# ducha-aiki/affnet

Measured on AMD Instinct MI355X. Metric: keypoints/sec (detect+AffNet+OriNet+HardNet) per image, 2000 kp @1024x768, higher is better.
Workload: dtype f32

## Files before the change

### affnet_amd/SparseImgRepresenter.py

```python
import ctypes as C

import torch
import torch.nn as nn

from . import _lib, engine
from ._lib import lib, check, ptr
from .architectures import _HipPatchNet
from .HandCraftedModules import AffineShapeEstimator, OrientationDetector, _HipHandCrafted
from .HardNet import HardTFeatNet
from .pytorch_sift import SIFTNet

_FOLLOW = (SIFTNet, HardTFeatNet)


class ScaleSpaceAffinePatchExtractor(nn.Module):
    def __init__(self, border=16, num_features=500, patch_size=32, mrSize=3.0, nlevels=3, num_Baum_iters=0,
                 init_sigma=1.6, th=None, RespNet=None, OriNet=None, AffNet=None, arith="fp32"):
        super(ScaleSpaceAffinePatchExtractor, self).__init__()
        self.arith = arith
        _lib.arith_code(arith)
        self.mrSize, self.PS, self.b = mrSize, patch_size, border
        self.num, self.nlevels = num_features, nlevels
        self.num_Baum_iters, self.init_sigma = num_Baum_iters, init_sigma
        self.th = th
        if th is not None:
            self.num = -1
        else:
            self.th = 0
        self.RespNet = RespNet
        if not 1 <= nlevels <= 6:
            raise NotImplementedError("nlevels must be 1..6 (levels per octave = nlevels + 2 <= 8)")
        self.OriNet = OriNet if OriNet is not None else OrientationDetector(patch_size=19)
        self.AffNet = AffNet if AffNet is not None else AffineShapeEstimator(patch_size=19)
        self.scale_pyr = self.sigmas = self.pix_dists = None
        self._ctx = None
        self._ctx_key = None
        self._fctx = self._fctx_key = self._pyr_ctx = None
        self.last_ids = None
        self.max_keep = 16384
        self.raw_div = 4
        self.lazy_shape_rows = -1
        self.shape_form = 1

        self.desc_form = 2

    def _context(self, x, allow_batch=False):
        engine.require_cuda(x, "image")
        if x.dim() != 4 or x.size(1) != 1 or x.size(0) < 1 or (x.size(0) != 1 and not allow_batch):
            raise ValueError("expected a (1,1,H,W) image; forward() is batch-size-1 like the reference "
                             "(HandCraftedModules.py:283-284) - use enqueue()/run_batch() for (B,1,H,W) batches")
        pre = int(1.5 * self.num) if self.num_Baum_iters > 0 else self.num
        key = (x.size(0), x.size(2), x.size(3), x.device, pre, self.num, float(self.th), self.mrSize, self.b, self.init_sigma,
               self.nlevels, self.max_keep, self.num_Baum_iters, self.raw_div, self.lazy_shape_rows)
        if self._ctx is not None and self._ctx_key == key and self._ctx.arith != _lib.arith_code(self.arith):
            self._ctx.set_arith(self.arith)
        if self._ctx is None or self._ctx_key != key:
            self._ctx = engine.Context(x.size(2), x.size(3), x.device, self.nlevels, self.init_sigma, self.b, self.mrSize,
                                       float(self.th), self.num, pre, self.max_keep, batch=x.size(0), baum_iters=self.num_Baum_iters, raw_div=self.raw_div,
                                       lazy_shape_rows=self.lazy_shape_rows, arith=self.arith)
            self._ctx_key = key
        if self._ctx.shape_form != int(self.shape_form):
            self._ctx.set_shape_form(self.shape_form)
        if self._ctx.desc_form != int(self.desc_form):
            self._ctx.set_desc_form(self.desc_form)
        return self._ctx

    def _publish_pyramid(self, ctx):
        self._pyr_ctx = ctx
        self.scale_pyr = ctx.pyramid_views()
        self.sigmas = [list(s) for s in ctx.plan.sigmas]
        self.pix_dists = [list(p) for p in ctx.plan.pix_dists]

    def _response_pyramid(self, ctx, img):
        dev = img.device
        st = engine.stream_of(dev)
        check(lib.affnet_pyramid_build(ctx.handle, ptr(img), st), ctx.handle, "affnet_pyramid_build")
        stride = lib.affnet_pyramid_image_stride(ctx.handle)
        base = lib.affnet_pyramid_level_offset(ctx.handle, 0, 0)
        resp = torch.zeros(ctx.batch * stride, dtype=torch.float32, device=dev)
        with torch.no_grad():
            for b in range(ctx.batch):
                pyr = ctx.pyramid_views(b)
                for o, (h, w) in enumerate(ctx.plan.sizes):
                    for l in range(ctx.plan.levels_per_octave):
                        off = b * stride + lib.affnet_pyramid_level_offset(ctx.handle, o, l) - base
                        r = self.RespNet(pyr[o][l], ctx.plan.sigmas[o][l])
                        resp[off:off + h * w].copy_(r.reshape(-1).to(dev, torch.float32))
        return resp

    @staticmethod
    def _native(slot):
        return slot is None or isinstance(slot, (_HipPatchNet, _HipHandCrafted))

    def enqueue(self, x, do_ori=False, desc=None, det_stream=None, input_ready=None):
        ctx = self._context(x, allow_batch=True)
        dev = x.device
        if not (self._native(self.AffNet) and self._native(self.OriNet)):
            raise NotImplementedError("the fused path needs the native AffNetFast / OriNetFast slots (foreign slots: forward())")
        img = x.contiguous().float()
        B, F = x.size(0), ctx.cap_final
        lafs = torch.empty(B, F, 2, 3, dtype=torch.float32, device=dev)
        resp = torch.empty(B, F, dtype=torch.float32, device=dev)
        ids = torch.empty(B, F, 3, dtype=torch.int32, device=dev)
        count = torch.zeros(B, dtype=torch.int32, device=dev)
        dsc = torch.empty(B, F, 128, dtype=torch.float32, device=dev) if desc is not None else None
        nets = self._nets(dev, do_ori, desc)
        follow = isinstance(desc, _FOLLOW)
        if isinstance(desc, HardTFeatNet):
            desc.check_usable()
        fused_dsc = None if follow else dsc
        if self.RespNet is not None:
            rmaps = self._response_pyramid(ctx, img)
            check(lib.affnet_detect_image_responses(ctx.handle, ptr(rmaps), engine.stream_of(dev)), ctx.handle, "affnet_detect_image_responses")
            rc = lib.affnet_describe_detected(ctx.handle, C.byref(nets), int(bool(do_ori)), ptr(lafs), ptr(resp), ptr(ids), ptr(fused_dsc),
                                              ptr(count), engine.stream_of(dev))
            check(rc, ctx.handle, "affnet_describe_detected")
        elif det_stream is None:
            rc = lib.affnet_extract_features(ctx.handle, C.byref(nets), ptr(img), int(bool(do_ori)), ptr(lafs), ptr(resp), ptr(ids),
                                             ptr(fused_dsc), ptr(count), engine.stream_of(dev))
            check(rc, ctx.handle, "affnet_extract_features")
        else:
            cur = torch.cuda.current_stream(dev)
            if input_ready is None:
                det_stream.wait_stream(cur)
            elif input_ready is not False:
                det_stream.wait_event(input_ready)
            if getattr(self, "_busy", None) is not None:
# ... 374 lines not shown
```

### affnet_amd/_lib.py

```python
import ctypes as C
import os

_HERE = os.path.dirname(os.path.abspath(__file__))
LIB_PATH = os.environ.get("AFFNET_HIP_LIB") or os.path.join(_HERE, "libaffnet_hip.so")
PROBES_LIB_PATH = os.path.join(_HERE, "libaffnet_hip_probes.so")

MAX_OCTAVES, MAX_LEVELS, MAX_TAPS = 16, 8, 37
NET_AFFNET, NET_ORINET, NET_HARDNET, NET_AFFNET_FULLCONV = 0, 1, 2, 3
ARITH_FP32_MFMA, ARITH_FP32_SPLIT3, ARITH_FP32_SPLIT2H = 0, 1, 2
ARITH_NAMES = {"fp32": ARITH_FP32_MFMA, "fp32_mfma": ARITH_FP32_MFMA, "fp32_split3": ARITH_FP32_SPLIT3, "split3": ARITH_FP32_SPLIT3,
               "fp32_split2h": ARITH_FP32_SPLIT2H, "split2h": ARITH_FP32_SPLIT2H}


def arith_code(arith):
    if arith is None:
        return ARITH_FP32_MFMA
    if isinstance(arith, str):
        if arith.lower() not in ARITH_NAMES:
            raise ValueError("arith must be one of %s" % sorted(ARITH_NAMES))
        return ARITH_NAMES[arith.lower()]
    if int(arith) not in (ARITH_FP32_MFMA, ARITH_FP32_SPLIT3, ARITH_FP32_SPLIT2H):
        raise ValueError("arith must be AFFNET_ARITH_FP32_MFMA (0), AFFNET_ARITH_FP32_SPLIT3 (1) or AFFNET_ARITH_FP32_SPLIT2H (2)")
    return int(arith)
SHAPE_FORM_DIRECT, SHAPE_FORM_WINOGRAD, SHAPE_FORM_POLYPHASE = 0, 1, 2
DESC_FORM_DIRECT, DESC_FORM_POLYPHASE, DESC_FORM_F43 = 0, 1, 2
OK, ERR_INVALID, ERR_HIP, ERR_CAPACITY, ERR_EMPTY = 0, -1, -2, -3, -4
VERIFY_AFFINE, VERIFY_HOMOGRAPHY, VERIFY_TILE, VERIFY_CHUNK = 0, 1, 128, 128
KNN_MAX_K = 8
IVF_MAX_PROBE = 8
VERIFY_FLAG_PAIR_RANGE = 8


class Config(C.Structure):
    _fields_ = [
        ("height", C.c_int32), ("width", C.c_int32), ("n_octaves", C.c_int32), ("levels_per_octave", C.c_int32),
        ("oct_h", C.c_int32 * MAX_OCTAVES), ("oct_w", C.c_int32 * MAX_OCTAVES),
        ("level_sigma", (C.c_float * MAX_LEVELS) * MAX_OCTAVES),
        ("level_sigma4", (C.c_float * MAX_LEVELS) * MAX_OCTAVES),
        ("level_sigma_px", (C.c_double * MAX_LEVELS) * MAX_OCTAVES),
        ("first_blur_taps", C.c_int32), ("first_blur", C.c_float * (MAX_TAPS * MAX_TAPS)),
        ("level_blur_taps", C.c_int32 * MAX_LEVELS),
        ("level_blur", (C.c_float * (MAX_TAPS * MAX_TAPS)) * MAX_LEVELS),
        ("level_blur0_taps", C.c_int32 * MAX_LEVELS),
        ("level_blur0", (C.c_float * (MAX_TAPS * MAX_TAPS)) * MAX_LEVELS),
        ("lazy_shape_rows", C.c_int32),
        ("onepass", C.c_int32),
        ("mr_size", C.c_float), ("threshold", C.c_float),
        ("num_features", C.c_int32), ("num_prefilter", C.c_int32),
        ("max_raw_per_octave_div", C.c_int32), ("max_keep", C.c_int32), ("batch", C.c_int32), ("baum_iters", C.c_int32),
        ("arith", C.c_int32),
    ]


class Nets(C.Structure):
    _fields_ = [("d_affnet", C.c_void_p), ("d_orinet", C.c_void_p), ("d_hardnet", C.c_void_p),
                ("h_orientation_window", C.c_void_p), ("h_baumberg_window", C.c_void_p)]


_P, _I, _SZ = C.c_void_p, C.c_int, C.c_size_t
SYMBOLS = {
    "affnet_config_fill": (_I, [C.POINTER(Config), _I, _I, _I, C.c_double, _I, C.c_double, C.c_double, _I, _I, _I, _I]),
    "affnet_ctx_create": (_I, [C.POINTER(_P), _I, C.POINTER(Config)]),
    "affnet_ctx_destroy": (None, [_P]),
    "affnet_last_error": (C.c_char_p, [_P]),
    "affnet_version": (C.c_char_p, []),
    "affnet_set_arith": (_I, [_P, _I]),
    "affnet_get_arith": (_I, [_P]),
    "affnet_set_shape_form": (_I, [_P, _I]),
    "affnet_get_shape_form": (_I, [_P]),
    "affnet_set_desc_form": (_I, [_P, _I]),
    "affnet_get_desc_form": (_I, [_P]),
    "affnet_workspace_bytes": (_SZ, [_P]),
    "affnet_bind_workspace": (_I, [_P, _P, _SZ]),
    "affnet_pyramid_level_offset": (C.c_int64, [_P, _I, _I]),
    "affnet_pyramid_image_stride": (C.c_int64, [_P]),
    "affnet_batch": (_I, [_P]),
    "affnet_capacity_prefilter": (_I, [_P]),
    "affnet_capacity_final": (_I, [_P]),
    "affnet_gauss_blur": (_I, [_P, _P, _P, _I, _I, C.POINTER(C.c_float), _I, _P]),
    "affnet_pyramid_build": (_I, [_P, _P, _P]),
    "affnet_hessian_response": (_I, [_P, _P, _P, _I, _I, C.c_float, _P]),
    "affnet_detect": (_I, [_P, _P, _P, _P, _P, _P]),
    "affnet_detect_responses": (_I, [_P, _P, _P, _P, _P, _P, _P]),
    "affnet_laf_grid_sample": (_I, [_P, _P, _I, _I, _P, _I, _I, _P, _P]),
    "affnet_pyr_grid_sample": (_I, [_P, _P, _P, _P, _I, _I, _P, _P]),
    "affnet_cnn32_packed_floats": (_SZ, [_I]),
    "affnet_cnn32_winograd_offset": (C.c_int64, [_I, _I]),
    "affnet_cnn32_pack_weights": (_I, [_I, C.POINTER(_P), C.POINTER(_P), C.POINTER(_P), _P, _P, _P, _P, _P]),
    "affnet_cnn32_forward": (_I, [_P, _I, _P, _P, _P, _I, _P, _P, _P]),
    "affnet_cnn32_forward_pyr": (_I, [_P, _I, _P, _P, _P, _P, _I, _P, _P, _P]),
    "affnet_local_norm": (_I, [_P, _P, _P, _I, _I, _P]),
    "affnet_fullconv_scratch_bytes": (_SZ, [_I, _I]),
    "affnet_fullconv_forward": (_I, [_P, _P, _P, _I, _I, _P, _P, _P]),
    "affnet_nms2d": (_I, [_P, _P, _P, _I, _I, C.c_float, _P]),
    "affnet_shape_filter_select": (_I, [_P, _P, _P, _P, _P, _P, _P, _P, _P, _P, _P]),
    "affnet_apply_rotation": (_I, [_P, _P, _P, _P, _I, _P]),
    "affnet_scale_lafs": (_I, [_P, _P, _P, _P, _I, _I, _I, _I, _P]),
    "affnet_lafs_to_ellipses": (_I, [_P, _P, _P, _I, _P, _P]),
    "affnet_ellipses_to_lafs": (_I, [_P, _P, _P, _I, _P, _P]),
    "affnet_level_select": (_I, [_P, _P, _P, _I, _I, _P, _P, _P]),
    "affnet_handcrafted_forward": (_I, [_P, _I, _P, _I, _P, _P, _P, _P]),
    "affnet_handcrafted_forward_pyr": (_I, [_P, _I, _P, _P, _P, _I, _P, _P, _P]),
    "affnet_sift_host_window": (_I, [_I, C.POINTER(C.c_float)]),
    "affnet_sift_forward": (_I, [_P, _P, _I, _P, C.c_float, _P, _P]),
    "affnet_sift_forward_pyr": (_I, [_P, _P, _P, _P, _I, _P, C.c_float, _P, _P]),
    "affnet_tfeat_packed_floats": (_SZ, []),
    "affnet_tfeat_pack_weights": (_I, [_P, _P, _P, _P, _P, _P, _P]),
    "affnet_tfeat_scratch_floats": (_SZ, [_I]),
    "affnet_tfeat_forward": (_I, [_P, _P, _P, _P, _I, _P, _P, _P]),
    "affnet_tfeat_forward_pyr": (_I, [_P, _P, _P, _P, _P, _I, _P, _P, _P]),
    "affnet_match_scratch_bytes": (_SZ, [_I, _I]),
    "affnet_distance_matrix": (_I, [_P, _P, _I, _P, _I, _I, _P, _P, _P]),
    "affnet_match_snn": (_I, [_P, _P, _I, _P, _I, _I, C.c_float, _P, _P, _P, _P, _P, _P, _P]),
    "affnet_reproject_lafs": (_I, [_P, _P, _I, C.POINTER(C.c_float), _P, _P]),
    "affnet_centre_nn": (_I, [_P, _P, _I, _P, _I, _P, _P, _P]),
    "affnet_verify_scratch_bytes": (_SZ, [_I]),
    "affnet_verify_score": (_I, [_P, _P, _I, _P, _I, _P, _P, _I, C.c_float, _P, _P, _P, _P]),
    "affnet_verify_matches": (_I, [_P, _P, _I, _P, _I, _P, _P, _I, C.c_float, _I, _I, _P, _P, _P, _P, _P, _P]),
    "affnet_match_many_scratch_bytes": (_SZ, [_I, _I, _I]),
    "affnet_match_snn_many": (_I, [_P, _P, _I, _P, _I, _I, _P, _I, _I, _I, C.c_float, _P, _P, _P, _P, _P, _P, _P]),
    "affnet_verify_many_scratch_bytes": (_SZ, [_I, _I]),
    "affnet_verify_matches_many": (_I, [_P, _P, _I, _P, _I, _P, _I, _P, _P, _I, C.c_float, _I, _I, _P, _P, _P, _P, _P, _P]),
    "affnet_knn_chunks": (_I, [_P, _I, _I]),
    "affnet_knn_scratch_bytes": (_SZ, [_I, _I, _I, _I]),
    "affnet_knn": (_I, [_P, _P, _I, _P, _I, _I, _I, _I, _I, _I, _P, _P, _P, _P]),
    "affnet_knn_vote": (_I, [_P, _P, _P, _I, _I, C.c_float, _P, _I, _I, _P, _P]),
    "affnet_quantize_desc": (_I, [_P, _P, _I, _I, C.c_float, _P, _P, _P]),
    "affnet_knn_q8_chunks": (_I, [_P, _I, _I]),
    "affnet_knn_q8_scratch_bytes": (_SZ, [_I, _I, _I, _I]),
    "affnet_knn_q8": (_I, [_P, _P, _P, _I, _P, _P, _I, _I, _I, _I, _I, _I, C.c_float, _P, _P, _P, _P, _P]),
    "affnet_ivf_sqnorm": (_I, [_P, _P, _I, _I, _P, _P]),
    "affnet_ivf_cell_means": (_I, [_P, _P, _I, _I, _P, _P, _I, _P, _P]),
    "affnet_ivf_scratch_bytes": (_SZ, [_I, _I, _I, _I]),
    "affnet_ivf_search": (_I, [_P, _P, _I, _P, _P, _P, _I, _P, _P, _I, _I, _I, _I, _I, _I, _P, _P, _P, _P, _P]),
    "affnet_ivf_q8_scratch_bytes": (_SZ, [_I, _I, _I, _I]),
    "affnet_ivf_search_q8": (_I, [_P, _P, _P, _P, _I, _P, _P, _P, _I, _P, _P, _I, _I, _I, _I, _I, _I, C.c_float, _P, _P, _P, _P, _P, _P]),
    "affnet_extract_features": (_I, [_P, C.POINTER(Nets), _P, _I, _P, _P, _P, _P, _P, _P]),
    "affnet_detect_image": (_I, [_P, _P, _P]),
    "affnet_detect_image_responses": (_I, [_P, _P, _P]),
    "affnet_detect_image_onepass": (_I, [_P, _P, _P, _P]),
    "affnet_detect_image_onepass_responses": (_I, [_P, _P, _P, _P]),
    "affnet_detected_list": (_I, [_P, _P, _P, _P, _P, _P]),
    "affnet_load_frames": (_I, [_P, _P, _I, _P, _P, _P, _I, _I, _P]),
    "affnet_describe_frames": (_I, [_P, C.POINTER(Nets), _P, _P, _P, _P, _I, _I, _P, _P, _P, _P, _P, _P]),
    "affnet_shape_iterate": (_I, [_P, _P, _P, _P, _P, _I, _P, _P]),
    "affnet_affmap_offset": (C.c_int64, [_P, _I]),
    "affnet_affmap_image_stride": (C.c_int64, [_P]),
    "affnet_describe_detected": (_I, [_P, C.POINTER(Nets), _I, _P, _P, _P, _P, _P, _P]),
    "affnet_graph_capture_extract": (_I, [_P, C.POINTER(Nets), _P, _I, _P, _P, _P, _P, _P, _P]),
    "affnet_graph_launch": (_I, [_P, _P]),
    "affnet_profile_enable": (_I, [_P, _I]),
    "affnet_profile_read": (_I, [_P, C.POINTER(C.c_double * 8), C.POINTER(C.c_int32)]),
    "affnet_read_counts": (_I, [_P, C.POINTER(C.c_int32 * 4), _P]),
    "affnet_counter_offset": (C.c_int64, [_P, _I]),
    "affnet_counter_stride": (C.c_int64, [_P]),
    "affnet_host_base_grid": (_I, [_I, C.POINTER(C.c_float)]),
}

DEBUG_SYMBOLS = {
    "affnet_cnn32_debug_timing": (_I, [_P, _P]),
    "affnet_cnn32_debug_layer": (_I, [_P, _I, _P, _P, _I, _P, _P]),
    "affnet_cnn32_debug_winograd_u": (_I, [_P, _I, _P, _I, _P, _P]),
    "affnet_selftest_mfma": (_I, [_P, _P, _P, _P]),
    "affnet_debug_split3_variant": (_I, [_P, _I]),
}

PROBE_SYMBOLS = {
    "affnet_cnn32_probe": (_I, [_P, _I, _I, _I, _I, _P, _P]),
    "affnet_split3_gemm": (_I, [_P, _P, _I, _I, _I, _I, _P, _P]),
    "affnet_split3_rate": (_I, [_I, _I, _I, _P, _P]),
    "affnet_debug_stream": (_I, [_P, _P, _SZ, _I, _I, _I, _P]),
    "affnet_probe_shape_offsets": (_I, [_P, C.POINTER(C.c_int64 * 3)]),
    "affnet_probe_affnet_wino_layer": (_I, [_P, _I, _P, _P, _I, _P, _P]),
    "affnet_probe_affnet_wino_partials": (_I, [_P, _P, _P, _I, _P, _P]),
    "affnet_probe_affnet_poly_layer": (_I, [_P, _I, _P, _P, _I, _P, _P]),
    "affnet_probe_affnet_poly_partials": (_I, [_P, _P, _P, _I, _P, _P]),
    "affnet_probe_trunk16_poly_u": (_I, [_P, _I, _P, _I, _P, _P]),
    "affnet_probe_hardnet_poly_layer": (_I, [_P, _P, _P, _I, _P, _P]),
    "affnet_probe_hardnet_poly_forward": (_I, [_P, _P, _P, _I, _P, _P, _P]),
    "affnet_probe_hardnet_poly_u": (_I, [_P, _P, _I, _P, _P]),
    "affnet_probe_hardnet_f43_layer": (_I, [_P, _P, _P, _I, _P, _P]),
    "affnet_probe_hardnet_f43_forward": (_I, [_P, _P, _P, _I, _P, _P, _P]),
    "affnet_probe_hardnet_f43_u": (_I, [_P, _P, _I, _P, _P]),
}


class AffnetHipError(RuntimeError):
    pass


class AffnetEmptyError(AffnetHipError):
    """AFFNET_ERR_EMPTY: no image of the call produced a detection (the reference raises in torch.cat([]),
    SparseImgRepresenter.py:100)."""


def _load():
    if not os.path.isfile(LIB_PATH):
        if os.path.basename(LIB_PATH) == os.path.basename(PROBES_LIB_PATH):
            raise ImportError("affnet_amd: %s is missing - the tools under tools/ need the probe build of the library: "
                              "AFFNET_PROBES=1 bash affnet_amd/csrc/build.sh" % LIB_PATH)
        raise ImportError(
            "affnet_amd: %s is missing - the HIP extension is the only implementation of this path "
            "(no CPU fallback). Build it: bash affnet_amd/csrc/build.sh" % LIB_PATH)
    lib = C.CDLL(LIB_PATH)
    for table in (SYMBOLS, DEBUG_SYMBOLS):
        for name, (res, args) in table.items():
            fn = getattr(lib, name)
            fn.restype, fn.argtypes = res, args
    for name, (res, args) in PROBE_SYMBOLS.items():
        if hasattr(lib, name):
            fn = getattr(lib, name)
            fn.restype, fn.argtypes = res, args
    return lib


lib = _load()


def check(rc, ctx=None, what=""):
    if rc != OK:
        msg = lib.affnet_last_error(ctx).decode() if ctx else ""
        if rc == ERR_EMPTY:
            raise AffnetEmptyError("%s: %s" % (what or "libaffnet_hip call", msg))
        raise AffnetHipError("%s failed (code %d): %s" % (what or "libaffnet_hip call", rc, msg))


def ptr(t):
    return None if t is None else C.c_void_p(t.data_ptr())


def current_stream(device):
    import torch
    return C.c_void_p(torch.cuda.current_stream(device).cuda_stream)
```

### affnet_amd/csrc/cnn32.hip

```cpp
#include "common.h"

static void aff_fill_pyr_src(const affnet_ctx* ctx, PyrSrc* s) {
    memset(s, 0, sizeof(*s));
    if (ctx->ws) aff_fill_pyr_table(ctx, &s->t);
    aff_base_grid(32, s->base);
}

static int cnn_check(affnet_ctx* ctx, const CnnCall& c, int* rows) {
    *rows = 0;
    if (c.kind < 0 || c.kind > 2) return aff_fail(ctx, AFFNET_ERR_INVALID, "cnn32: unknown net kind %d", c.kind);
    if (!c.packed || !c.out || c.n_max < 0 || (!c.patches && (!c.lafs || !c.ids))) return aff_fail(ctx, AFFNET_ERR_INVALID, "cnn32: null argument");
    if (!c.patches && !ctx->ws) return aff_fail(ctx, AFFNET_ERR_INVALID, "cnn32: sampling from the pyramid needs a bound workspace");
    if (c.dbg_layer < 0 && !c.scratch)
        return aff_fail(ctx, AFFNET_ERR_INVALID, "cnn32: d_scratch is required (HardNet n*(8192+512) floats, AffNet / OriNet n*144 floats)");
    if (c.dbg_layer >= 0 && ctx->arith != AFFNET_ARITH_FP32_MFMA)
        return aff_fail(ctx, AFFNET_ERR_INVALID, "cnn32: layer dumps exist for AFFNET_ARITH_FP32_MFMA only (context is in arithmetic mode %d)", ctx->arith);
    if (c.n_max == 0) return AFFNET_OK;
    if (c.kind == AFFNET_NET_HARDNET && c.n_max > 65535)
        return aff_fail(ctx, AFFNET_ERR_INVALID, "cnn32: n_max=%d (HardNet head: max 65535 rows per image)", c.n_max);
    const int row_count = c.row_count < 0 ? c.n_max - c.row_begin : c.row_count;
    if (c.row_begin < 0 || row_count < 0 || c.row_begin + row_count > c.n_max) return aff_fail(ctx, AFFNET_ERR_INVALID, "cnn32: bad row window");
    *rows = row_count;
    return AFFNET_OK;
}

TrunkKernel aff_trunk_kernel(int kind, int form, bool stamps) {
    typedef TrunkKernel (*Unit)(int, bool);
    static_assert(AFFNET_NET_AFFNET == 0 && AFFNET_NET_ORINET == 1 && AFFNET_NET_HARDNET == 2 && TRUNK_EXACT == 0 && TRUNK_WINO == 1 && TRUNK_SPLIT2 == 2 && TRUNK_SPLIT3 == 3 &&
                  TRUNK_WINO_F43 == 4 && TRUNK_WINO_POLY == 5 && TRUNK_FORMS == 6, "order of the table");
    static const Unit unit[3][TRUNK_FORMS] = {{aff_trunk_affnet, aff_trunk_affnet, aff_trunk_affnet, aff_trunk_affnet, nullptr, aff_trunk_affnet_poly},
                                              {aff_trunk_orinet, nullptr, aff_trunk_orinet, aff_trunk_orinet, nullptr, nullptr},
                                              {aff_trunk_hardnet, aff_trunk_hardnet_poly, aff_trunk_hardnet, aff_trunk_hardnet, aff_trunk_hardnet_f43, nullptr}};
    if (kind < 0 || kind > 2 || form < 0 || form >= TRUNK_FORMS || !unit[kind][form]) return nullptr;
    return unit[kind][form](form, stamps);
}

int aff_trunk_launch(affnet_ctx* ctx, const CnnCall& c, const NetLayout& L, dim3 grid, int wino, const int32_t* reeval, int shape_op) {
    int form = TRUNK_EXACT;
    if (ctx->arith != AFFNET_ARITH_FP32_MFMA) form = ctx->arith == AFFNET_ARITH_FP32_SPLIT2H ? TRUNK_SPLIT2 : TRUNK_SPLIT3;
    else if (c.kind == AFFNET_NET_AFFNET && wino) form = wino == 2 ? TRUNK_WINO_POLY : TRUNK_WINO;
    else if (c.kind == AFFNET_NET_HARDNET && c.desc_form != AFFNET_DESC_FORM_DIRECT) form = c.desc_form == AFFNET_DESC_FORM_F43 ? TRUNK_WINO_F43 : TRUNK_WINO;
    const bool stamps = ctx->dbg_time || c.dbg_layer >= 0;
    const TrunkKernel kernel = aff_trunk_kernel(c.kind, form, stamps);
    if (!kernel) return aff_fail(ctx, AFFNET_ERR_INVALID, "cnn32: no trunk kernel of net %d in form %d is built", c.kind, form);
    CnnArgs a;
    a.packed = c.packed; a.off = to_offsets(L, ctx->arith);
    a.reeval = reeval;
    const int rc = aff_derive_u(ctx, c.kind, form, c.packed, L, c.st, &a.wino_u);
    if (rc) return rc;
    a.patches = c.patches; a.lafs = c.lafs; a.ids = c.ids; a.count = c.count; a.n_max = c.n_max;
    a.out = (c.dbg_layer < 0) ? c.scratch : c.out;
    a.dbg_layer = c.dbg_layer; a.dbg_out = c.dbg_out; a.dbg_time = ctx->dbg_time;
    a.row_begin = c.row_begin; a.skip_cnt = c.skip_cnt; a.skip_n = c.skip_n;
    a.shape_cnt = (c.fuse && shape_op) ? c.fuse->cnt : nullptr; a.shape_op = shape_op;
    a.s3_alt = ctx->split3_variant;
    PyrSrc ps;
    aff_fill_pyr_src(ctx, &ps);
    hipLaunchKernelGGL(kernel, grid, dim3(512), 0, c.st, a, ps);
    AFF_LAUNCH_CHECK(ctx);
    return AFFNET_OK;
}

static int cnn_launch(affnet_ctx* ctx, const CnnCall& c) {
    int rows;
    int rc = cnn_check(ctx, c, &rows);
    if (rc || rows == 0) return rc;
    const NetLayout L = net_layout(c.kind);
    const int B = c.patches ? 1 : ctx->B;
    const bool form1 = c.wino_reeval && c.kind == AFFNET_NET_AFFNET && c.fuse && c.dbg_layer < 0 && ctx->arith == AFFNET_ARITH_FP32_MFMA;
    rc = aff_trunk_launch(ctx, c, L, dim3(rows, B), form1 ? c.wino_reeval : 0, nullptr, c.shape_op);
    if (rc) return rc;
    if (form1) {
        int32_t* flags = reinterpret_cast<int32_t*>(c.scratch + (size_t)B * c.n_max * HEAD_PART_AFF);
        rc = aff_margin_affnet(ctx, c, L, rows, B, flags);
        if (rc) return rc;
        rc = aff_trunk_launch(ctx, c, L, dim3(rows, B), 0, flags, 0);
        if (rc) return rc;
    }
    if (c.dbg_layer < 0 && c.kind != AFFNET_NET_HARDNET) {
        rc = c.kind == AFFNET_NET_AFFNET ? aff_finish_affnet(ctx, c, L, rows, B) : aff_finish_orinet(ctx, c, L, rows, B);
        if (rc) return rc;
    }
    if (c.mark_head) aff_prof_mark(ctx, 7, c.st);
    if (c.dbg_layer < 0 && c.kind == AFFNET_NET_HARDNET) return aff_hardnet_head(ctx, c, L, B);
    return AFFNET_OK;
}

extern "C" int affnet_cnn32_forward(affnet_ctx* ctx, int net_kind, const float* d_packed, const float* d_patches, const int32_t* d_count,
                                    int n_max, float* d_out, float* d_scratch, void* stream) {
    AFF_DEVICE(ctx);
    if (!ctx || !d_patches) return aff_fail(ctx, AFFNET_ERR_INVALID, "cnn32_forward: null argument");
    CnnCall c;
    c.kind = net_kind; c.packed = d_packed; c.patches = d_patches; c.count = d_count; c.n_max = n_max; c.out = d_out; c.scratch = d_scratch; c.st = (hipStream_t)stream;
    return cnn_launch(ctx, c);
}

extern "C" int affnet_cnn32_forward_pyr(affnet_ctx* ctx, int net_kind, const float* d_packed, const float* d_lafs, const int32_t* d_ids,
                                        const int32_t* d_count, int n_max, float* d_out, float* d_scratch, void* stream) {
    AFF_DEVICE(ctx);
    if (!ctx) return AFFNET_ERR_INVALID;
    CnnCall c;
    c.kind = net_kind; c.packed = d_packed; c.lafs = d_lafs; c.ids = d_ids; c.count = d_count; c.n_max = n_max; c.out = d_out; c.scratch = d_scratch; c.st = (hipStream_t)stream;
    return cnn_launch(ctx, c);
}

int aff_affnet_filter_rows(affnet_ctx* ctx, const float* packed, const float* resp, const float* lafs, const int32_t* ids, const int32_t* count,
                           float* out, float* scratch, int row_begin, int row_count, bool lazy, int shape_op, hipStream_t st) {
    ShapeFuse sf;
    sf.resp = resp; sf.lafs = lafs; sf.key = ctx->st_key; sf.good = ctx->st_good; sf.cnt = ctx->cnt;
    CnnCall c;
    c.kind = AFFNET_NET_AFFNET; c.packed = packed; c.lafs = lafs; c.ids = ids; c.count = count; c.n_max = ctx->cap_pre; c.out = out; c.scratch = scratch; c.st = st;
    c.row_begin = row_begin; c.row_count = row_count;
    c.skip_cnt = lazy ? ctx->cnt : nullptr; c.skip_n = ctx->cfg.num_features;
    c.fuse = &sf; c.shape_op = shape_op;
    c.wino_reeval = ctx->shape_form;
    return cnn_launch(ctx, c);
}

int aff_orinet_rotate(affnet_ctx* ctx, const float* packed, float* lafs, const int32_t* ids, const int32_t* count, int n_max, float* out, float* scratch,
                      hipStream_t st, const DenormSel* denorm) {
    CnnCall c;
    c.kind = AFFNET_NET_ORINET; c.packed = packed; c.lafs = lafs; c.ids = ids; c.count = count; c.n_max = n_max; c.out = out; c.scratch = scratch; c.st = st;
    c.rot_lafs = lafs; c.denorm = denorm;
    return cnn_launch(ctx, c);
// ... 52 lines not shown
```

### affnet_amd/csrc/cnn_mfma.h

```cpp
#pragma once
#include <math.h>
#include <stdlib.h>

#include <utility>

#include "common.h"
#include "weights_layout.h"

typedef float f32x4 __attribute__((ext_vector_type(4)));

typedef __attribute__((address_space(3))) const f32x4 LdsF4;
__device__ __forceinline__ unsigned lds_byte_addr(const float* p) {
    return (unsigned)(size_t)(__attribute__((address_space(3))) const float*)p;
}
__device__ __forceinline__ f32x4 lds_read4(unsigned byte_addr) { return *(LdsF4*)(size_t)byte_addr; }

typedef unsigned u32x4 __attribute__((ext_vector_type(4)));
__device__ __forceinline__ __amdgpu_buffer_rsrc_t weight_rsrc(const float* base, int n_floats) {
    return __builtin_amdgcn_make_buffer_rsrc(const_cast<float*>(base), 0, n_floats * 4, 0x00020000);
}
__device__ __forceinline__ f32x4 buf_read4(__amdgpu_buffer_rsrc_t r, int lane_byte_off, int uniform_byte_off) {
    return __builtin_bit_cast(f32x4, __builtin_amdgcn_raw_buffer_load_b128(r, lane_byte_off, uniform_byte_off, 0));
}

// ... 979 lines not shown
            for (int c = 0; c < 2; ++c) {
#pragma unroll
                for (int j = 0; j < 4; ++j)
#pragma unroll
                    for (int e = 0; e < 4; ++e) {
                        if (i == 0) t0[c][j][e] = acc[c][j][e];
                        else if (i == 1) { t0[c][j][e] = wadd(t0[c][j][e], acc[c][j][e]); t1[c][j][e] = acc[c][j][e]; }
                        else if (i == 2) { t0[c][j][e] = wadd(t0[c][j][e], acc[c][j][e]); t1[c][j][e] = wsub(t1[c][j][e], acc[c][j][e]); }
                        else t1[c][j][e] = wsub(t1[c][j][e], acc[c][j][e]);
                    }
                if (i == 3) {
#pragma unroll
                    for (int e = 0; e < 4; ++e) {
                        y[2 * u + c][0][e] = wadd(wadd(t0[c][0][e], t0[c][1][e]), t0[c][2][e]);
                        y[2 * u + c][1][e] = wsub(wsub(t0[c][1][e], t0[c][2][e]), t0[c][3][e]);
                        y[2 * u + c][2][e] = wadd(wadd(t1[c][0][e], t1[c][1][e]), t1[c][2][e]);
                        y[2 * u + c][3][e] = wsub(wsub(t1[c][1][e], t1[c][2][e]), t1[c][3][e]);
                    }
                }
            }
            __builtin_amdgcn_sched_barrier(0);
        }
    };
    {
        f32x4 da[4], db[4];
        wino_read_rows<LI>(window_addr(0), 0, da, db);
        wino_transform_row(0, da, db, Va);
    }
#pragma unroll
    for (int s = 0; s < NSTEP; s += 2) {
        step(s, Va, Vb);
        step(s + 1, Vb, Va);
    }
}

template <int NW, int CIN, int COUT, typename LI>
__device__ __forceinline__ void conv3x3_wino_mfma_shared_v(float* act, const float* __restrict__ Wu, f32x4 (&U)[16], f32x4 (&y)[1][4], int wave, int lane) {
    constexpr int NGRP = CIN / 16;
    static_assert(LI::H == 8 && COUT == 16 * NW && NGRP == NW, "one tile block, one channel block and one K group per wave");
    const int m = lane & 15, kq = lane >> 4;
    const __amdgpu_buffer_rsrc_t wrsrc = weight_rsrc(Wu, 16 * CIN * COUT);
    int ty, tx, cb;
    wino_tile<8, COUT, 1>(wave, 0, m, ty, tx, cb);
    const int u_lane = wino_u_lane<8, COUT, 1>(wave, 0, lane);
    f32x4 V[16];
    wino_window<LI>(lds_byte_addr(act) + ((wave * 4 + kq) * LI::PSG + (2 * ty * LI::WP + 2 * tx) * 4) * 4, V);
    __syncthreads();
    const unsigned v0 = lds_byte_addr(act) + lane * 16;
#pragma unroll
    for (int k = 0; k < 16; ++k) *reinterpret_cast<f32x4*>(&act[((wave * 16 + k) * 64 + lane) * 4]) = V[k];
    __syncthreads();
#pragma unroll
    for (int k = 0; k < 16; ++k) V[k] = lds_read4(v0 + k * 1024);
    f32x4 acc[16];
#pragma unroll
    for (int k = 0; k < 16; ++k) acc[k] = (f32x4){0.f, 0.f, 0.f, 0.f};
#pragma unroll 1
    for (int G = 0; G < NGRP; ++G) {
        const int Gn = G == NGRP - 1 ? G : G + 1;
        unsigned vb = v0 + Gn * 16 * 1024;
        asm("" : "+v"(vb));
        __builtin_amdgcn_sched_barrier(0);
#pragma unroll
        for (int k = 0; k < 16; k += 2) {
#pragma unroll
            for (int s4 = 0; s4 < 4; ++s4) {
                acc[k] = __builtin_amdgcn_mfma_f32_16x16x4f32(U[k][s4], V[k][s4], acc[k], 0, 0, 0);
                acc[k + 1] = __builtin_amdgcn_mfma_f32_16x16x4f32(U[k + 1][s4], V[k + 1][s4], acc[k + 1], 0, 0, 0);
            }
            U[k] = wino_load_u<CIN, COUT>(wrsrc, u_lane, k, Gn);
            U[k + 1] = wino_load_u<CIN, COUT>(wrsrc, u_lane, k + 1, Gn);
            V[k] = lds_read4(vb + k * 1024);
            V[k + 1] = lds_read4(vb + (k + 1) * 1024);
            __builtin_amdgcn_sched_barrier(0);
        }
    }
    wino_output(acc, y[0]);
}

struct F43L {
    static constexpr int V_FLOATS = 4 * F43_XI * 256;
    static constexpr int X = 0, X_FLOATS = 8 * 8 * 256;
};
__device__ __forceinline__ void f43_bt_lo(float d0, float d1, float d2, float d3, float d4, float& v0, float& v1, float& v2) {
    v0 = (4.0f * d0 - 5.0f * d2) + d4;
    const float a = d4 - 4.0f * d2, b = d3 - 4.0f * d1;
    v1 = a + b; v2 = a - b;
}
__device__ __forceinline__ void f43_bt_hi(float d1, float d2, float d3, float d4, float d5, float& v3, float& v4, float& v5) {
    const float c = d4 - d2, e = 2.0f * (d3 - d1);
    v3 = c + e; v4 = c - e;
    v5 = (4.0f * d1 - 5.0f * d3) + d5;
}
__device__ __forceinline__ void f43_at_axis(float m0, float m1, float m2, float m3, float m4, float m5, float& y0, float& y1, float& y2, float& y3) {
    const float p = m1 + m2, q = m1 - m2, r = m3 + m4, s = m3 - m4;
    y0 = (m0 + p) + r; y1 = q + 2.0f * s; y2 = p + 4.0f * r; y3 = q + (8.0f * s + m5);
}

template <typename LI, int HF>
__device__ __forceinline__ void f43_window_half(unsigned ab, f32x4 (&V)[18]) {
    f32x4 d[5][6];
#pragma unroll
    for (int r = 0; r < 5; ++r)
#pragma unroll
        for (int c = 0; c < 6; ++c) d[r][c] = lds_read4(ab + ((r + HF) * LI::WP + c) * 16);
#pragma unroll
    for (int e = 0; e < 4; ++e) {
        float t[3][6];
#pragma unroll
        for (int c = 0; c < 6; ++c) {
            if constexpr (HF == 0) f43_bt_lo(d[0][c][e], d[1][c][e], d[2][c][e], d[3][c][e], d[4][c][e], t[0][c], t[1][c], t[2][c]);
            else f43_bt_hi(d[0][c][e], d[1][c][e], d[2][c][e], d[3][c][e], d[4][c][e], t[0][c], t[1][c], t[2][c]);
        }
#pragma unroll
        for (int il = 0; il < 3; ++il) {
            float v[6];
            f43_bt_lo(t[il][0], t[il][1], t[il][2], t[il][3], t[il][4], v[0], v[1], v[2]);
            f43_bt_hi(t[il][1], t[il][2], t[il][3], t[il][4], t[il][5], v[3], v[4], v[5]);
#pragma unroll
            for (int j = 0; j < 6; ++j) V[6 * il + j][e] = v[j];
        }
    }
}

template <int CIN, int COUT>
__device__ __forceinline__ int f43_u_lane(int wave, int lane) {
    return ((lane >> 4) * COUT + (wave >> 1) * 16 + (lane & 15)) * 16 + (wave & 1) * (18 * CIN * COUT * 4);
}
template <int CIN, int COUT>
__device__ __forceinline__ void f43_prefetch_u(const float* __restrict__ Wu, f32x4 (&U)[18], int wave, int lane) {
    const __amdgpu_buffer_rsrc_t r = weight_rsrc(Wu, F43_XI * CIN * COUT);
    const int u_lane = f43_u_lane<CIN, COUT>(wave, lane);
#pragma unroll
    for (int k = 0; k < 18; ++k) U[k] = wino_load_u<CIN, COUT>(r, u_lane, k, 0);
}

template <int NW, int CIN, int COUT, typename LI>
__device__ __forceinline__ void conv3x3_f43_mfma_shared_v(float* act, const float* __restrict__ Wu, f32x4 (&U)[18], f32x4 (&t)[3][4], int wave, int lane) {
    constexpr int NGRP = CIN / 16;
    static_assert(NW == 8 && LI::H == 16 && COUT == 16 * (NW / 2) && NGRP == NW / 2, "one block of 16 4x4 tiles; a wave pair per channel block and per K group");
    const int m = lane & 15, kq = lane >> 4, p = wave >> 1, h = wave & 1;
    const __amdgpu_buffer_rsrc_t wrsrc = weight_rsrc(Wu, F43_XI * CIN * COUT);
    const int u_lane = f43_u_lane<CIN, COUT>(wave, lane);
    f32x4 V[18];
    {
        const unsigned ab = lds_byte_addr(act) + ((4 * p + kq) * LI::PSG + (4 * (m >> 2) * LI::WP + 4 * (m & 3)) * 4) * 4;
        if (h == 0) f43_window_half<LI, 0>(ab, V); else f43_window_half<LI, 1>(ab, V);
    }
    __syncthreads();
#pragma unroll
    for (int k = 0; k < 18; ++k) *reinterpret_cast<f32x4*>(&act[((p * F43_XI + 18 * h + k) * 64 + lane) * 4]) = V[k];
    __syncthreads();
    const unsigned v0 = lds_byte_addr(act) + (18 * h * 64 + lane) * 16;
#pragma unroll
    for (int k = 0; k < 18; ++k) V[k] = lds_read4(v0 + k * 1024);
    f32x4 acc[18];
#pragma unroll
    for (int k = 0; k < 18; ++k) acc[k] = (f32x4){0.f, 0.f, 0.f, 0.f};
#pragma unroll 1
    for (int G = 0; G < NGRP; ++G) {
        const int Gn = G == NGRP - 1 ? G : G + 1;
        unsigned vb = v0 + Gn * F43_XI * 1024;
        asm("" : "+v"(vb));
        __builtin_amdgcn_sched_barrier(0);
#pragma unroll
        for (int k = 0; k < 18; k += 2) {
#pragma unroll
            for (int s4 = 0; s4 < 4; ++s4) {
                acc[k] = __builtin_amdgcn_mfma_f32_16x16x4f32(U[k][s4], V[k][s4], acc[k], 0, 0, 0);
                acc[k + 1] = __builtin_amdgcn_mfma_f32_16x16x4f32(U[k + 1][s4], V[k + 1][s4], acc[k + 1], 0, 0, 0);
            }
            U[k] = wino_load_u<CIN, COUT>(wrsrc, u_lane, k, Gn);
            U[k + 1] = wino_load_u<CIN, COUT>(wrsrc, u_lane, k + 1, Gn);
            V[k] = lds_read4(vb + k * 1024);
            V[k + 1] = lds_read4(vb + (k + 1) * 1024);
            __builtin_amdgcn_sched_barrier(0);
        }
    }
#pragma unroll
    for (int il = 0; il < 3; ++il)
#pragma unroll
        for (int e = 0; e < 4; ++e) {
            float yc[4];
            f43_at_axis(acc[6 * il][e], acc[6 * il + 1][e], acc[6 * il + 2][e], acc[6 * il + 3][e], acc[6 * il + 4][e], acc[6 * il + 5][e], yc[0], yc[1], yc[2], yc[3]);
#pragma unroll
            for (int c = 0; c < 4; ++c) t[il][c][e] = yc[c];
        }
}

__device__ __forceinline__ void f43_combine(float* lds, const f32x4 (&t)[3][4], f32x4 (&y)[8], int wave, int lane) {
    const int h = wave & 1;
    float* xw = lds + F43L::X + (wave * 8 * 64 + lane) * 4;
    const float* xr = lds + F43L::X + ((wave ^ 1) * 8 * 64 + lane) * 4;
    f32x4 k0[4], k1[4];
    if (h == 0) {
#pragma unroll
        for (int c = 0; c < 4; ++c) {
            const f32x4 p = t[1][c] + t[2][c], q = t[1][c] - t[2][c];
            k0[c] = t[0][c] + p; k1[c] = q;
            *reinterpret_cast<f32x4*>(&xw[c * 256]) = p;
            *reinterpret_cast<f32x4*>(&xw[(4 + c) * 256]) = q;
        }
    } else {
#pragma unroll
        for (int c = 0; c < 4; ++c) {
            const f32x4 r = t[0][c] + t[1][c], s = t[0][c] - t[1][c];
            k0[c] = 4.0f * r; k1[c] = 8.0f * s + t[2][c];
            *reinterpret_cast<f32x4*>(&xw[c * 256]) = r;
            *reinterpret_cast<f32x4*>(&xw[(4 + c) * 256]) = 2.0f * s;
        }
    }
    __syncthreads();
#pragma unroll
    for (int c = 0; c < 4; ++c) {
        const f32x4 o0 = *reinterpret_cast<const f32x4*>(&xr[c * 256]), o1 = *reinterpret_cast<const f32x4*>(&xr[(4 + c) * 256]);
        y[c] = k0[c] + o0;
        y[4 + c] = k1[c] + o1;
    }
}

template <typename LO>
__device__ __forceinline__ void f43_store_lds(float* act, f32x4 bias, const f32x4 (&y)[8], int wave, int lane) {
    const int m = lane & 15, oy = 4 * (m >> 2) + 2 * (wave & 1), ox = 4 * (m & 3);
#pragma unroll
    for (int k = 0; k < 8; ++k) {
        const f32x4 v = bias_relu(y[k], bias);
        *reinterpret_cast<f32x4*>(&act[((wave >> 1) * 4 + (lane >> 4)) * LO::PSG + ((oy + (k >> 2) + 1) * LO::WP + ox + (k & 3) + 1) * 4]) = v;
    }
}

template <int NW, int CIN, int COUT, int H, int NB>
__device__ __forceinline__ void wino_prefetch_u_row(const float* __restrict__ Wu, f32x4 (&U)[4], int wave, int lane) {
    const __amdgpu_buffer_rsrc_t r = weight_rsrc(Wu, 16 * CIN * COUT);
    const int u_lane = wino_u_lane<H, COUT, NB>(wave, 0, lane);
#pragma unroll
    for (int k = 0; k < 4; ++k) U[k] = wino_load_u<CIN, COUT>(r, u_lane, k, 0);
}

template <int NW, int CIN, int COUT, typename LI, int NB>
__device__ __forceinline__ void conv3x3_wino_mfma_rows(const float* act, const float* __restrict__ Wu, f32x4 (&U)[4], f32x4 (&y)[NB][4], int wave, int lane) {
    constexpr int H = LI::H, HT = H / 2, NGRP = CIN / 16, NSTEP = NB * 4 * NGRP;
    static_assert(H % 2 == 0 && (HT * HT) % 16 == 0 && COUT % 16 == 0 && CIN % 16 == 0, "Winograd tiling");
    static_assert((HT * HT / 16) * (COUT / 16) == NW * NB, "the waves' passes must tile the layer exactly");
    const int m = lane & 15, kq = lane >> 4;
    const __amdgpu_buffer_rsrc_t wrsrc = weight_rsrc(Wu, 16 * CIN * COUT);
    f32x4 t0[4], t1[4], acc[4];
#pragma unroll
    for (int s = 0; s < NSTEP; ++s) {
        const int q = s / (4 * NGRP), i = (s / NGRP) % 4, G = s % NGRP;
        const int sn = s + 1 < NSTEP ? s + 1 : s;
        const int qn = sn / (4 * NGRP), in = (sn / NGRP) % 4, Gn = sn % NGRP;
        int ty, tx, cb;
        wino_tile<H, COUT, NB>(wave, q, m, ty, tx, cb);
        const int u_next = wino_u_lane<H, COUT, NB>(wave, qn, lane);
        unsigned ab = lds_byte_addr(act) + (((4 * G + kq) * LI::PSG + (2 * ty * LI::WP + 2 * tx) * 4) * 4);
        asm("" : "+v"(ab));
        f32x4 da[4], db[4], V[4];
        wino_read_rows<LI>(ab, i, da, db);
        wino_transform_row(i, da, db, V);
        if (G == 0) {
#pragma unroll
            for (int k = 0; k < 4; ++k) acc[k] = (f32x4){0.f, 0.f, 0.f, 0.f};
        }
        __builtin_amdgcn_sched_barrier(0);
#pragma unroll
        for (int k = 0; k < 4; k += 2) {
#pragma unroll
            for (int s4 = 0; s4 < 4; ++s4) {
                acc[k] = __builtin_amdgcn_mfma_f32_16x16x4f32(U[k][s4], V[k][s4], acc[k], 0, 0, 0);
                acc[k + 1] = __builtin_amdgcn_mfma_f32_16x16x4f32(U[k + 1][s4], V[k + 1][s4], acc[k + 1], 0, 0, 0);
            }
            U[k] = wino_load_u<CIN, COUT>(wrsrc, u_next, 4 * in + k, Gn);
            U[k + 1] = wino_load_u<CIN, COUT>(wrsrc, u_next, 4 * in + k + 1, Gn);
            __builtin_amdgcn_sched_barrier(0);
        }
        if (G == NGRP - 1) {
#pragma unroll
            for (int j = 0; j < 4; ++j)
#pragma unroll
                for (int e = 0; e < 4; ++e) {
                    if (i == 0) t0[j][e] = acc[j][e];
                    else if (i == 1) { t0[j][e] = wadd(t0[j][e], acc[j][e]); t1[j][e] = acc[j][e]; }
                    else if (i == 2) { t0[j][e] = wadd(t0[j][e], acc[j][e]); t1[j][e] = wsub(t1[j][e], acc[j][e]); }
                    else t1[j][e] = wsub(t1[j][e], acc[j][e]);
                }
            if (i == 3) {
#pragma unroll
                for (int e = 0; e < 4; ++e) {
                    y[q][0][e] = wadd(wadd(t0[0][e], t0[1][e]), t0[2][e]);
                    y[q][1][e] = wsub(wsub(t0[1][e], t0[2][e]), t0[3][e]);
                    y[q][2][e] = wadd(wadd(t1[0][e], t1[1][e]), t1[2][e]);
                    y[q][3][e] = wsub(wsub(t1[1][e], t1[2][e]), t1[3][e]);
                }
            }
        }
    }
}

struct Wino5 {
    static constexpr int X = 16 * LayC4::PSG, X_FLOATS = 8 * 4 * 256;
    static constexpr int HEAD = 0;
    static constexpr int U_HALF = 8 * 4 * 16 * 64 * 4;
};
__device__ __forceinline__ void wino5_prefetch_u(const float* __restrict__ Wu, f32x4 (&U)[4], int wave, int lane) {
    const __amdgpu_buffer_rsrc_t r = weight_rsrc(Wu, 16 * 64 * 64);
    const int u_lane = ((lane >> 4) * 64 + (wave >> 1) * 16 + (lane & 15)) * 16 + (wave & 1) * Wino5::U_HALF;
#pragma unroll
    for (int k = 0; k < 4; ++k) U[k] = wino_load_u<64, 64>(r, u_lane, k, 0);
}

template <int NW, typename LI>
// ... 385 lines not shown
```

### affnet_amd/csrc/cnn_trunk.h

```cpp
#pragma once
#include <math.h>

#include <type_traits>

#include "common.h"

#include "cnn_mfma.h"

template <int TM>
__device__ __forceinline__ void head_partials(const float* __restrict__ hw, const f32x4 (&bias)[1], const f32x4 (&acc)[TM][1],
                                              float* __restrict__ part, int wave, int lane) {
    constexpr int MT = 4, MG = MT / TM;
    const int mg = wave % MG, ng = wave / MG;
    const int n = lane & 15, g = lane >> 4;
    const int c4 = ng * 16 + 4 * g;
    f32x4 v[TM];
#pragma unroll
    for (int i = 0; i < TM; ++i) v[i] = bias_relu(acc[i][0], bias[0]);
    const __amdgpu_buffer_rsrc_t r = weight_rsrc(hw, 3 * 4096);
    f32x4 w[3][TM];
#pragma unroll
    for (int o = 0; o < 3; ++o)
#pragma unroll
        for (int i = 0; i < TM; ++i) w[o][i] = buf_read4(r, (n * 64 + c4) * 4, (o * 4096 + (mg * TM + i) * 16 * 64) * 4);
// ... 62 lines not shown
    }
}
template <int TM>
__device__ __forceinline__ void ori_head_pbase(const OriHeadLane& L, int (&pbase)[TM]) {
#pragma unroll
    for (int i = 0; i < TM; ++i) {
        const int p = (L.mg * TM + i) * 16 + L.n;
        pbase[i] = ((p >> 3) * 10 + (p & 7)) * ORI_HP + L.c4;
    }
}
template <int TM>
__device__ __forceinline__ void ori_head_reduce(const f32x4 (&w)[2][TM], const int (&pbase)[TM], float* __restrict__ part, const float* act, int wave, int lane) {
    __syncthreads();
#pragma unroll
    for (int q = 0; q < 9; ++q) {
        float s0 = 0.f, s1 = 0.f;
#pragma unroll
        for (int i = 0; i < TM; ++i) {
            const f32x4 av = *reinterpret_cast<const f32x4*>(&act[pbase[i] + ((q / 3) * 10 + q % 3) * ORI_HP]);
#pragma unroll
            for (int j = 0; j < 4; ++j) { s0 = fmaf(av[j], w[0][i][j], s0); s1 = fmaf(av[j], w[1][i][j], s1); }
        }
        s0 = wave_sum(s0);
        s1 = wave_sum(s1);
        if (lane == 0) { part[wave * 18 + q] = s0; part[wave * 18 + 9 + q] = s1; }
    }
}
template <int TM, int NTHR>
__device__ __forceinline__ void head_partials_ori_lds(const float* __restrict__ hw, const f32x4 (&bias)[1], const f32x4 (&acc)[TM][1],
                                                      float* __restrict__ part, float* act, int wave, int lane, int tid) {
    constexpr int MT = 4, MG = MT / TM;
    const int mg = wave % MG, ng = wave / MG;
    const int n = lane & 15, g = lane >> 4;
    const int c4 = ng * 16 + 4 * g;
    f32x4 v[TM];
#pragma unroll
    for (int i = 0; i < TM; ++i) v[i] = bias_relu(acc[i][0], bias[0]);
    const __amdgpu_buffer_rsrc_t r = weight_rsrc(hw, 2 * 4096);
    f32x4 w[2][TM];
#pragma unroll
    for (int o = 0; o < 2; ++o)
#pragma unroll
        for (int i = 0; i < TM; ++i) w[o][i] = buf_read4(r, (n * 64 + c4) * 4, (o * 4096 + (mg * TM + i) * 16 * 64) * 4);
    __syncthreads();
    ori_head_zero_halo<NTHR>(act, tid);
    int pbase[TM];
#pragma unroll
    for (int i = 0; i < TM; ++i) {
        const int p = (mg * TM + i) * 16 + n;
        pbase[i] = ((p >> 3) * 10 + (p & 7)) * ORI_HP + c4;
        *reinterpret_cast<f32x4*>(&act[pbase[i] + 11 * ORI_HP]) = v[i];
    }
    ori_head_reduce<TM>(w, pbase, part, act, wave, lane);
}

#define CNN_STAMP(k)                                                                                     \
    do {                                                                                                 \
        if (STAMPS && a.dbg_time && lane == 0) a.dbg_time[((size_t)pidx * NW + wave) * 32 + (k)] = __builtin_readcyclecounter(); \
    } while (0)

template <int CB>
struct TrunkLds {
    static constexpr int ACT = (CB / 4) * LayC0::PSG;
    static constexpr int PATCH = WP32 * WP32;
    static constexpr int RED = 256;
    static constexpr int TOTAL = ACT + PATCH + RED;
};

template <int KIND, int NW>
struct TrunkShape {
    static constexpr int CB = (KIND == AFFNET_NET_HARDNET) ? 32 : 16;
    static constexpr int NTHR = NW * 64;
    static constexpr int T1M = (CB == 16) ? 8 : 64 / NW, T1N = CB / 16;
    static constexpr int T2M = (CB == 16) ? 4 : 64 / NW, T2N = 1;
    static constexpr int T4M = (CB == 16) ? 2 : 32 / NW, T4N = 1;
    static constexpr int AREG = (NW == 8 && CB == 32) ? 128 : 48;
    static constexpr int G2 = pick_groups(CB, T2M, T2N, 32, AREG), G3 = pick_groups(2 * CB, T2M, T2N, 32, AREG);
    static constexpr int G4 = pick_groups(2 * CB, T4M, T4N, 32, AREG), G5 = pick_groups(4 * CB, T4M, T4N, 32, AREG);
};

template <int KIND, int S3>
struct TrunkTraits {
    static_assert(S3 == TRUNK_EXACT || S3 == TRUNK_SPLIT2 || S3 == TRUNK_SPLIT3 || (S3 == TRUNK_WINO && KIND != AFFNET_NET_ORINET) ||
                  (S3 == TRUNK_WINO_F43 && KIND == AFFNET_NET_HARDNET) || (S3 == TRUNK_WINO_POLY && KIND == AFFNET_NET_AFFNET), "no such trunk form of this net (common.h: TRUNK_*)");
    static constexpr bool EXACT = S3 != TRUNK_SPLIT2 && S3 != TRUNK_SPLIT3;
    static constexpr bool WINO13 = (S3 == TRUNK_EXACT && KIND == AFFNET_NET_ORINET) || ((S3 == TRUNK_WINO || S3 == TRUNK_WINO_POLY) && KIND == AFFNET_NET_AFFNET);
    static constexpr bool POLY16 = (S3 == TRUNK_EXACT && KIND == AFFNET_NET_ORINET) || (S3 == TRUNK_WINO_POLY && KIND == AFFNET_NET_AFFNET);
    static constexpr bool POLY = (S3 == TRUNK_WINO || S3 == TRUNK_WINO_F43) && KIND == AFFNET_NET_HARDNET, F43_3 = S3 == TRUNK_WINO_F43 && KIND == AFFNET_NET_HARDNET;
};

template <int C, typename L, int NTHR>
__device__ __forceinline__ void dump_planes(const float* act, float* dst) {
    constexpr int H = L::H;
    for (int i = threadIdx.x; i < C * H * H; i += NTHR) {
        const int c = i / (H * H), r = i - c * H * H, y = r / H, x = r - y * H;
        dst[i] = act[L::at(c, y, x)];
    }
}

template <int CB>
struct SplitLays {
    typedef LayQ<16, 32, 34, CB, 0, 3> LQH;
    typedef LayQ<16, 32, 34, CB, 16, 3> LQH2;
    using LR0 = LayR<32, 32, 34, CB, 0>;
    using LR0H = LayR<16, 32, 34, CB, 0, 34>;
    using LR1 = LayR<32, 32, 34, CB, 16>;
    using LR1H = LayR<16, 32, 34, CB, 16, 34>;
    static_assert(LR0::BYTES <= TrunkLds<CB>::ACT * 4 && LR1::BYTES <= TrunkLds<CB>::ACT * 4 && LR0H::GS == LR0::GS && LR1H::GS == LR1::GS, "whole-patch split layouts");
    static_assert(LQH::BYTES <= TrunkLds<CB>::ACT * 4 && LQH2::BYTES <= TrunkLds<CB>::ACT * 4, "pre-split layouts must fit the activation buffer");
};

template <int KIND, int NW, bool STAMPS, int S3 = 0>
__global__ __launch_bounds__(NW * 64, (KIND == AFFNET_NET_HARDNET) ? NW / 4 : 4) void cnn32_trunk_kernel(CnnArgs a, PyrSrc ps) {
    using F = TrunkTraits<KIND, S3>;
    constexpr bool EXACT = F::EXACT, WINO13 = F::WINO13, POLY16 = F::POLY16, POLY = F::POLY, F43_3 = F::F43_3;
    using S = TrunkShape<KIND, NW>;
    constexpr int CB = S::CB, NTHR = S::NTHR;
    static_assert((CB / 4) * LayC1::PSG <= TrunkLds<CB>::ACT && (CB / 2) * LayC3::PSG <= TrunkLds<CB>::ACT, "LDS layout");
    __shared__ __attribute__((aligned(16))) float lds[TrunkLds<CB>::TOTAL];
    float* act = lds;
    float* patch = lds + TrunkLds<CB>::ACT;
    float* red = patch + TrunkLds<CB>::PATCH;
    const int n = a.count ? min(a.count[blockIdx.y], a.n_max) : a.n_max;
    const int prow = blockIdx.x + a.row_begin;
    if (KIND == AFFNET_NET_AFFNET && a.shape_cnt && blockIdx.x == 0 && threadIdx.x == 0) {
        int32_t* c = a.shape_cnt + (size_t)blockIdx.y * CNT_TOTAL;
        if (a.shape_op == 1) { c[CNT_SURVIVED] = 0; c[CNT_SURVIVED1] = 0; c[CNT_AFF_EVAL] = 0; c[CNT_AFF_REEVAL] = 0; }
        else if (a.shape_op == 2) c[CNT_SURVIVED1] = c[CNT_SURVIVED];
    }
    if (prow >= n || lazy_skip(a.skip_cnt, a.skip_n, blockIdx.y, CNT_SURVIVED)) return;
    const size_t pidx = (size_t)blockIdx.y * a.n_max + prow;
    if (KIND == AFFNET_NET_AFFNET && a.reeval && a.reeval[pidx] == 0) return;
    const int tid = threadIdx.x, wave = tid >> 6, lane = tid & 63;
    if (KIND == AFFNET_NET_HARDNET) __builtin_amdgcn_s_setprio(3);
    CNN_STAMP(0);
    if (STAMPS && a.dbg_time && lane == 0) {
        a.dbg_time[((size_t)pidx * NW + wave) * 32 + 14] = __builtin_amdgcn_s_getreg((31 << 11) | 4);
        a.dbg_time[((size_t)pidx * NW + wave) * 32 + 15] = __builtin_amdgcn_s_getreg((31 << 11) | 20);
    }
    float w0[3][S::T1N];
    f32x4 bias0[S::T1N];
    conv0_load_w<NW, CB, S::T1M, S::T1N>(a.packed + a.off.w[0], a.packed + a.off.b[0], w0, bias0, wave, lane);
    f32x4 b1[1][S::T1N];
    f32x4 Ur[4];
    if constexpr (S3 == TRUNK_EXACT && KIND == AFFNET_NET_AFFNET) prefetch_b0<NW, CB, 32, S::T1M, S::T1N, 1>(a.packed + a.off.w[1], b1, wave, lane);
    if constexpr (WINO13) wino_prefetch_u_row<NW, CB, CB, 32, Wino16::NB1>(a.wino_u, Ur, wave, lane);

    constexpr int PPT = 1024 / NTHR;
    constexpr int RPT = 32 / PPT;
    float v[PPT];
    if (a.patches) {
        const float* src = a.patches + pidx * 1024;
#pragma unroll
        for (int q = 0; q < PPT; ++q) v[q] = src[tid + q * NTHR];
    } else {
        int o = a.ids[3 * pidx], l = a.ids[3 * pidx + 1];
        o = o < 0 ? 0 : (o >= ps.t.n_octaves ? ps.t.n_octaves - 1 : o);
        l = l < 0 ? 0 : (l >= ps.t.n_levels ? ps.t.n_levels - 1 : l);
        const float* img = ps.t.lvl[o][l] + blockIdx.y * ps.t.img_stride;
        const int h = ps.t.h[o], w = ps.t.w[o];
        const float* L = a.lafs + 6 * pidx;
        const float m = (float)(h < w ? h : w);
        const float t00 = L[0] * m, t01 = L[1] * m, t02 = L[2] * (float)w;
        const float t10 = L[3] * m, t11 = L[4] * m, t12 = L[5] * (float)h;
#pragma unroll
        for (int q = 0; q < PPT; ++q)
            v[q] = aff_sample_bilinear(img, h, w, t00, t01, t02, t10, t11, t12, ps.base[tid & 31], ps.base[(tid >> 5) + q * RPT]);
    }
    CNN_STAMP(16);
    if (tid < 4 * 33) {
        const int e = tid;
        const int y = e < 34 ? 0 : (e < 68 ? 33 : 1 + ((e - 68) >> 1)), x = e < 34 ? e : (e < 68 ? e - 34 : ((e - 68) & 1) * 33);
        patch[y * WP32 + x] = 0.0f;
    }
    if constexpr (EXACT) zero_halo<LayC0, NTHR>(act, CB);
    else if constexpr (S3 == TRUNK_SPLIT2) zero_halo_q<typename SplitLays<CB>::LR0, NTHR>(act);
    else zero_halo_q<typename SplitLays<CB>::LQH, NTHR>(act);
    float sum = 0.f;
#pragma unroll
    for (int q = 0; q < PPT; ++q) sum += v[q];
    const float mean = block_sum<NW>(sum, red) * (1.0f / 1024.0f);
    CNN_STAMP(17);
    float sq = 0.f;
#pragma unroll
    for (int q = 0; q < PPT; ++q) { v[q] -= mean; sq += v[q] * v[q]; }
    const float var = block_sum<NW>(sq, red + NW) * (1.0f / 1023.0f);
    const float sd = sqrtf(var) + 1e-7f;
    CNN_STAMP(18);
#pragma unroll
    for (int q = 0; q < PPT; ++q) patch[((tid >> 5) + q * RPT + 1) * WP32 + (tid & 31) + 1] = v[q] / sd;
    __syncthreads();
    CNN_STAMP(1);

    if constexpr (EXACT && KIND == AFFNET_NET_HARDNET) {
        constexpr int T1M = S::T1M, T1N = S::T1N, T2M = S::T2M, T2N = S::T2N, T4M = S::T4M, T4N = S::T4N;
        constexpr int NB1 = (16 * 16 / 16) * (CB / 16) / NW, NB3 = (8 * 8 / 16) * (2 * CB / 16) / NW, NB5 = (4 * 4 / 16) * (4 * CB / 16) / NW;
        constexpr int NBP2 = (8 * 8 / 16) * (2 * CB / 16) / NW, NBP4 = (4 * 4 / 16) * (4 * CB / 16) / NW;

        f32x4 Up[2][4];
        f32x4 Uw[16];
        f32x4 Uf[18];
        {
            f32x4 acc[T1M][T1N];
            conv0_mfma<NW, CB, T1M, T1N>(patch, w0, bias0, acc, wave, lane);
            CNN_STAMP(19);
            store_tiles_lds<CB, LayC0, T1M, T1N, false>(act, bias0, acc, wave, lane);
            CNN_STAMP(20);
            wino_prefetch_u_pair<NW, CB, CB, 32, NB1>(a.packed + a.off.w_wino[0], Up, wave, lane);
            __syncthreads();
        }
        if (STAMPS && a.dbg_layer == 0) { dump_planes<CB, LayC0, NTHR>(act, a.dbg_out); return; }
        CNN_STAMP(2);

        f32x4 b2[S::G2][T2N];
        f32x4 bias2[T2N];
        f32x4 P2a[2][3], P2b[2][3];
        {
            f32x4 y[NB1][4], bw[NB1];
            __builtin_amdgcn_s_setprio(0);
            conv3x3_wino_mfma_pair_rows<NW, CB, CB, LayC0, NB1>(act, a.packed + a.off.w_wino[0], Up, y, wave, lane);
            __builtin_amdgcn_s_setprio(3);
            CNN_STAMP(3);
            if constexpr (POLY) poly_prefetch_u<NW, CB, 2 * CB, 16, NBP2, 2>(a.wino_u + Poly32::offset(2), P2a, P2b, wave, lane);
            else {
                prefetch_b0<NW, 2 * CB, 16, T2M, T2N, S::G2>(a.packed + a.off.w[2], b2, wave, lane);
                prefetch_bias<NW, 16, T2M, T2N>(a.packed + a.off.b[2], bias2, wave, lane);
            }
            wino_bias<NW, 32, CB, NB1>(a.packed + a.off.b[1], bw, wave, lane);
            __syncthreads();
            CNN_STAMP(21);
            zero_halo<LayC1, NTHR>(act, CB);
            wino_store_lds<CB, LayC1, NB1>(act, bw, y, wave, lane);
            CNN_STAMP(22);
            __syncthreads();
            CNN_STAMP(4);
        }
        if (STAMPS && a.dbg_layer == 1) { dump_planes<CB, LayC1, NTHR>(act, a.dbg_out); return; }

        if constexpr (POLY) {
            f32x4 y[NBP2][4], bw[NBP2];
            __builtin_amdgcn_s_setprio(0);
            conv3x3_poly_mfma_rows<NW, CB, 2 * CB, LayC1, NBP2, 2>(act, a.wino_u + Poly32::offset(2), P2a, P2b, y, wave, lane);
            __builtin_amdgcn_s_setprio(3);
            CNN_STAMP(5);
            if constexpr (F43_3) f43_prefetch_u<2 * CB, 2 * CB>(a.wino_u + F43::BASE + F43::offset(3), Uf, wave, lane);
            else wino_prefetch_u_pair<NW, 2 * CB, 2 * CB, 16, NB3>(a.packed + a.off.w_wino[1], Up, wave, lane);
            wino_bias<NW, 16, 2 * CB, NBP2>(a.packed + a.off.b[2], bw, wave, lane);
            __syncthreads();
            zero_halo<LayC2, NTHR>(act, 2 * CB);
            wino_store_lds<2 * CB, LayC2, NBP2>(act, bw, y, wave, lane);
            __syncthreads();
            CNN_STAMP(6);
        } else {
            f32x4 acc[T2M][T2N];
            __builtin_amdgcn_s_setprio(0);
            conv3x3_mfma<NW, CB, 2 * CB, LayC1, 2, T2M, T2N, S::G2>(act, a.packed + a.off.w[2], b2, acc, wave, lane);
            __builtin_amdgcn_s_setprio(3);
            CNN_STAMP(5);
            wino_prefetch_u_pair<NW, 2 * CB, 2 * CB, 16, NB3>(a.packed + a.off.w_wino[1], Up, wave, lane);
            __syncthreads();
            zero_halo<LayC2, NTHR>(act, 2 * CB);
            store_tiles_lds<2 * CB, LayC2, T2M, T2N>(act, bias2, acc, wave, lane);
            __syncthreads();
            CNN_STAMP(6);
        }
        if (STAMPS && a.dbg_layer == 2) { dump_planes<2 * CB, LayC2, NTHR>(act, a.dbg_out); return; }

        f32x4 b4[S::G4][T4N];
        f32x4 bias4[T4N];
        f32x4 P4a[1][3], P4b[1][3];
        if constexpr (F43_3) {
            static_assert(F43L::V_FLOATS <= TrunkLds<CB>::ACT && F43L::X + F43L::X_FLOATS <= F43L::V_FLOATS, "conv3: V of the layer fits the activation buffer");
            f32x4 tf[3][4], y[8];
            __builtin_amdgcn_s_setprio(0);
            conv3x3_f43_mfma_shared_v<NW, 2 * CB, 2 * CB, LayC2>(act, a.wino_u + F43::BASE + F43::offset(3), Uf, tf, wave, lane);
            __builtin_amdgcn_s_setprio(3);
            CNN_STAMP(23);
            poly_prefetch_u<NW, 2 * CB, 4 * CB, 8, NBP4, 1>(a.wino_u + Poly32::offset(4), P4a, P4b, wave, lane);
            const f32x4 bf = *reinterpret_cast<const f32x4*>(&a.packed[a.off.b[3] + (wave >> 1) * 16 + 4 * (lane >> 4)]);
            __syncthreads();
            f43_combine(act, tf, y, wave, lane);
            CNN_STAMP(7);
            __syncthreads();
            zero_halo<LayC3, NTHR>(act, 2 * CB);
            f43_store_lds<LayC3>(act, bf, y, wave, lane);
            __syncthreads();
            CNN_STAMP(8);
        } else {
            f32x4 y[NB3][4], bw[NB3];
            __builtin_amdgcn_s_setprio(0);
            conv3x3_wino_mfma_pair_rows<NW, 2 * CB, 2 * CB, LayC2, NB3>(act, a.packed + a.off.w_wino[1], Up, y, wave, lane);
            __builtin_amdgcn_s_setprio(3);
            CNN_STAMP(7);
            if constexpr (POLY) poly_prefetch_u<NW, 2 * CB, 4 * CB, 8, NBP4, 1>(a.wino_u + Poly32::offset(4), P4a, P4b, wave, lane);
            else {
                prefetch_b0<NW, 4 * CB, 8, T4M, T4N, S::G4>(a.packed + a.off.w[4], b4, wave, lane);
                prefetch_bias<NW, 8, T4M, T4N>(a.packed + a.off.b[4], bias4, wave, lane);
            }
            wino_bias<NW, 16, 2 * CB, NB3>(a.packed + a.off.b[3], bw, wave, lane);
            __syncthreads();
// ... 524 lines not shown
```

### affnet_amd/csrc/common.h

```cpp
#pragma once
#include <hip/hip_runtime.h>
#include <stdint.h>
#include <stdio.h>
#include <string.h>

#include <string>
#include <type_traits>
#include <vector>

#include "../../include/affnet_hip.h"
#include "../../include/affnet_hip_debug.h"
#include "weights_layout.h"

#define AFF_WAVE 64

enum {
    CNT_RAW0 = 0,
    CNT_CAND = AFFNET_MAX_OCTAVES,
    CNT_OVERFLOW,
    CNT_SEL,
    CNT_EQ_TAKEN,
    CNT_SEL_MODE,
    CNT_SEL_THRESH,
    CNT_SEL_NEED_EQ,
    CNT_DET,
    CNT_SHAPED,
    CNT_SURVIVED,
    CNT_CAND2,
    CNT_AFF_EVAL,
    CNT_SURVIVED1,
    CNT_SEL_EQ_TOTAL,
    CNT_SEL_TIE_LO, CNT_SEL_TIE_HI,
    CNT_AFF_REEVAL,
    CNT_POS0 = AFFNET_MAX_OCTAVES + 24,
    CNT_HYP0 = AFFNET_MAX_OCTAVES + 24 + (AFFNET_MAX_LEVELS - 2) * AFFNET_MAX_OCTAVES,
    CNT_TOTAL = AFFNET_MAX_OCTAVES + 24 + (AFFNET_MAX_LEVELS - 2) * AFFNET_MAX_OCTAVES + 8 * AFFNET_MAX_OCTAVES
};

#define OVF_FRAMES_COUNT 16
#define OVF_FRAMES_NONFINITE 32

#define SEL_HIST_BINS 2048

struct RawMax {
    int32_t pix;
    int32_t lvl;
    float val;
    float s, y, x;
    float prev[2];
};

struct OctaveGeom {
    int32_t h, w;
    int64_t pyr_off;
    int64_t map_off;
    int64_t raw_off;
    int32_t raw_cap;
};

struct affnet_ctx {
    int device = 0;
    affnet_config cfg;
    int B = 1;
    size_t pyr_stride = 0;
    size_t map_stride = 0;
    size_t raw_stride = 0;
    std::string err;
    OctaveGeom oct[AFFNET_MAX_OCTAVES];
    size_t off_pyr = 0, off_map = 0, off_raw = 0, off_cnt = 0, off_hist = 0, off_cand = 0, off_sel = 0, off_stage = 0;
    size_t off_affmap = 0, off_dense = 0, off_cand2 = 0, off_lvltab = 0;
    size_t aff_stride = 0;
    size_t aff_off[AFFNET_MAX_OCTAVES] = {0};
    size_t dense_stride = 0;
    float* affmap = nullptr; float* dense = nullptr;
    float* cand2_resp = nullptr; float* cand2_syx = nullptr; int32_t* cand2_ids = nullptr;
    int32_t* lvltab = nullptr;
    size_t ws_bytes = 0;
    size_t pyr_floats = 0, map_bytes = 0, raw_total = 0, cand_cap = 0;
    int cap_pre = 0, cap_final = 0;
    char* ws = nullptr;
    float* pyr = nullptr;
    uint8_t* omap = nullptr;
    RawMax* raw = nullptr;
    int32_t* cnt = nullptr;
    uint32_t* sel_hist = nullptr;
    float* cand_resp = nullptr; float* cand_syx = nullptr; int32_t* cand_ids = nullptr;
    float* sel_resp = nullptr; float* sel_syx = nullptr; int32_t* sel_ids = nullptr;
    float* st_det_resp = nullptr; float* st_det_lafs = nullptr; int32_t* st_det_ids = nullptr;
    int32_t* st_det_count = nullptr;
    float* st_A = nullptr; float* st_key = nullptr; int32_t* st_good = nullptr;
    float* st_A2 = nullptr; float* st_lafs_iter = nullptr;
    float* st_R = nullptr; float* st_lafs_norm = nullptr; int32_t* st_lvl_ids = nullptr;
    float* st_hard_scratch = nullptr;
    float* st_lafs_shaped = nullptr;
    int32_t* st_rank = nullptr;
    bool prof_on = false;
    std::vector<hipEvent_t> prof_ev;
    int prof_calls = 0;
    unsigned long long* dbg_time = nullptr;
    int shape_form = AFFNET_SHAPE_FORM_WINOGRAD;
    int arith = AFFNET_ARITH_FP32_MFMA;
    int split3_variant = 0;
    hipGraph_t graph = nullptr;
    hipGraphExec_t graph_exec = nullptr;
    float* derived_u = nullptr;
    int desc_form = AFFNET_DESC_FORM_F43;
    ~affnet_ctx() {
        if (derived_u) (void)hipFree(derived_u);
        if (graph_exec) (void)hipGraphExecDestroy(graph_exec);
        if (graph) (void)hipGraphDestroy(graph);
        for (auto& e : prof_ev) (void)hipEventDestroy(e);
    }
};

struct AffDeviceGuard {
    int prev = -1;
    bool switched = false;
    explicit AffDeviceGuard(const affnet_ctx* ctx) {
        if (!ctx) return;
        if (hipGetDevice(&prev) != hipSuccess) { (void)hipGetLastError(); prev = -1; return; }
        if (prev != ctx->device) switched = hipSetDevice(ctx->device) == hipSuccess;
    }
    ~AffDeviceGuard() {
        if (switched) (void)hipSetDevice(prev);
    }
    AffDeviceGuard(const AffDeviceGuard&) = delete;
    AffDeviceGuard& operator=(const AffDeviceGuard&) = delete;
};
#define AFF_DEVICE(ctx) AffDeviceGuard aff_device_guard_(ctx)

#define PROF_RING 256
#define PROF_EVENTS (AFFNET_PROFILE_STAGES + 2)

#define AFF_HIP(ctx, expr)                                                                         \
    do {                                                                                           \
        hipError_t e_ = (expr);                                                                    \
        if (e_ != hipSuccess)                                                                      \
            return aff_fail(ctx, AFFNET_ERR_HIP, "%s failed: %s (%s:%d)", #expr, hipGetErrorString(e_), \
                            __FILE__, __LINE__);                                                   \
    } while (0)

#define AFF_LAUNCH_CHECK(ctx)                                                                      \
    do {                                                                                           \
        hipError_t e_ = hipGetLastError();                                                         \
        if (e_ != hipSuccess)                                                                      \
            return aff_fail(ctx, AFFNET_ERR_HIP, "kernel launch failed: %s (%s:%d)",                \
                            hipGetErrorString(e_), __FILE__, __LINE__);                            \
    } while (0)

struct AffZeroSegs {
    unsigned char* p[8];
    size_t bytes[8];
    int n = 0;
    bool overflow = false;
    void add(void* ptr, size_t nbytes) {
        if (!ptr || !nbytes) return;
        if (n >= 8) { overflow = true; return; }
        p[n] = (unsigned char*)ptr; bytes[n] = nbytes; ++n;
    }
};

static inline size_t aff_align(size_t x, size_t a = 256) { return (x + a - 1) / a * a; }
static inline int aff_cdiv(int a, int b) { return (a + b - 1) / b; }

struct AffPairRow { int row1, n1, row2, n2; };
__device__ __forceinline__ bool aff_pair_row(const int32_t* __restrict__ pairs, int p, int rows1, int rows2, int n1_max, int n2_max, AffPairRow& r) {
    r.row1 = pairs[4 * (size_t)p]; r.n1 = pairs[4 * (size_t)p + 1]; r.row2 = pairs[4 * (size_t)p + 2]; r.n2 = pairs[4 * (size_t)p + 3];
    return r.row1 >= 0 && r.n1 >= 0 && r.row2 >= 0 && r.n2 >= 0 && (long long)r.row1 + r.n1 <= rows1 && (long long)r.row2 + r.n2 <= rows2 &&
           r.n1 <= n1_max && r.n2 <= n2_max;
}

struct PyrTable {
    const float* lvl[AFFNET_MAX_OCTAVES][AFFNET_MAX_LEVELS];
    int h[AFFNET_MAX_OCTAVES], w[AFFNET_MAX_OCTAVES];
    int n_octaves, n_levels;
    size_t img_stride;
};

struct LevelTable { double sig[AFFNET_MAX_OCTAVES * AFFNET_MAX_LEVELS]; int n_oct, n_lvl; };
struct DenormSel {
    float* out_px; int32_t* ids; float* lafs_norm;
    float c_a, c_x, c_y, ps, ca, cx, cy;
    LevelTable lt;
};


#define HEAD_PART_AFF 32
#define HEAD_PART_ORI 144
#define HEAD_KSPLIT 4
#define HEAD_KC 128
#define HEAD_AS (HEAD_KC + 4)

struct PyrSrc {
    PyrTable t;
    float base[32];
};

struct CnnArgs {
    const float* packed;
    NetOffsets off;
    const float* wino_u;
    const int32_t* reeval;
    const float* patches;
    const float* lafs;
    const int32_t* ids;
    const int32_t* count;
    int n_max;
    float* out;
    int dbg_layer;
    int s3_alt;
    float* dbg_out;
    unsigned long long* dbg_time;
    int row_begin;
    const int32_t* skip_cnt;
    int skip_n;
    int32_t* shape_cnt;
    int shape_op;
};

constexpr int TRUNK_EXACT = 0;
constexpr int TRUNK_WINO = 1;
constexpr int TRUNK_SPLIT2 = 2;
constexpr int TRUNK_SPLIT3 = 3;
constexpr int TRUNK_WINO_F43 = 4;
constexpr int TRUNK_WINO_POLY = 5;
constexpr int TRUNK_FORMS = 6;

__device__ __forceinline__ bool lazy_skip(const int32_t* skip_cnt, int skip_n, int image, int which = CNT_SURVIVED1) {
    if (!skip_cnt) return false;
    const int32_t* c = skip_cnt + (size_t)image * CNT_TOTAL;
    return c[CNT_SEL_MODE] == 1 && c[which] >= skip_n;
}

struct ShapeFuse {
    const float* resp; const float* lafs; float* key; int32_t* good; int32_t* cnt;
};

struct CnnCall {
    int kind = -1;
    const float* packed = nullptr;
    const float* patches = nullptr;
    const float* lafs = nullptr; const int32_t* ids = nullptr;
    const int32_t* count = nullptr; int n_max = 0;
    float* out = nullptr; float* scratch = nullptr;
    hipStream_t st = nullptr;
    int dbg_layer = -1; float* dbg_out = nullptr;
    bool mark_head = false;
    int row_begin = 0, row_count = -1;
    const int32_t* skip_cnt = nullptr; int skip_n = 0;
    const ShapeFuse* fuse = nullptr; int shape_op = 0;
    int desc_form = AFFNET_DESC_FORM_DIRECT;
    int wino_reeval = 0;
    float* rot_lafs = nullptr; const DenormSel* denorm = nullptr;
};

typedef void (*TrunkKernel)(CnnArgs, PyrSrc);

int aff_fail(affnet_ctx* ctx, int code, const char* fmt, ...);
int aff_zero_async(affnet_ctx* ctx, void* dst, size_t bytes, hipStream_t st);
int aff_zero_multi_async(affnet_ctx* ctx, const AffZeroSegs& z, hipStream_t st);
int aff_copy_async(affnet_ctx* ctx, void* dst, const void* src, size_t bytes, hipStream_t st);
int aff_copy2d_async(affnet_ctx* ctx, void* dst, size_t dpitch, const void* src, size_t spitch, size_t width_bytes, size_t rows, hipStream_t st);
void aff_base_grid(int ps, float* base);

void aff_prof_mark(affnet_ctx* ctx, int idx, hipStream_t st);

int aff_detect_impl(affnet_ctx* ctx, const float* d_responses, float* d_resp, float* d_lafs, int32_t* d_ids, int32_t* d_count, void* stream);
int aff_detect_onepass_impl(affnet_ctx* ctx, const float* d_packed_fullconv, const float* d_responses, hipStream_t st);

int aff_fullconv_launch(affnet_ctx* ctx, const float* packed, const float* img, size_t img_stride, int h, int w, float* out, size_t out_stride,
                        float* scratch, size_t scratch_stride, int B, hipStream_t st);

int aff_handcrafted_launch(affnet_ctx* ctx, int kind, const float* patches, const float* lafs, const int32_t* ids, const int32_t* count,
                           int n_max, const float* h_weights, float* out, float* out_angle, hipStream_t st);

void aff_fill_pyr_table(const affnet_ctx* ctx, PyrTable* t);
int aff_shape_select(affnet_ctx* ctx, const float* d_resp_in, const float* d_lafs_in, const int32_t* d_ids_in, const float* d_A,
                     const int32_t* d_count_in, float* d_resp_out, float* d_lafs_out, int32_t* d_ids_out, int32_t* d_count_out, hipStream_t st);
int aff_shape_iterate(affnet_ctx* ctx, const float* A, float* base, const float* lafs, const int32_t* count, int mode, float* lafs_out,
                      hipStream_t st);
void aff_denorm_sel_fill(affnet_ctx* ctx, int ps, float* d_lafs_px, int32_t* d_ids, float* d_lafs_norm, DenormSel* ds);
int aff_denorm_level_select(affnet_ctx* ctx, const float* d_lafs_norm_in, float* d_lafs_px, const int32_t* d_count, int n_max, int ps, int32_t* d_ids,
                            float* d_lafs_norm, hipStream_t st);

int aff_affnet_filter_rows(affnet_ctx* ctx, const float* packed, const float* resp, const float* lafs, const int32_t* ids, const int32_t* count,
                           float* out, float* scratch, int row_begin, int row_count, bool lazy, int shape_op, hipStream_t st);
int aff_orinet_rotate(affnet_ctx* ctx, const float* packed, float* lafs, const int32_t* ids, const int32_t* count, int n_max, float* out, float* scratch,
                      hipStream_t st, const DenormSel* denorm);
int aff_hardnet_forward_pyr_marked(affnet_ctx* ctx, const float* packed, const float* lafs, const int32_t* ids, const int32_t* count,
                                   int n_max, float* out, float* scratch, hipStream_t st);

int aff_hardnet_poly_patches(affnet_ctx* ctx, const float* packed, const float* patches, int n, float* out, float* scratch, int dbg_layer, hipStream_t st,
                             int form = AFFNET_DESC_FORM_POLYPHASE);
TrunkKernel aff_trunk_kernel(int kind, int form, bool stamps);
int aff_trunk_launch(affnet_ctx* ctx, const CnnCall& c, const NetLayout& L, dim3 grid, int wino, const int32_t* reeval, int shape_op);

TrunkKernel aff_trunk_affnet(int form, bool stamps), aff_trunk_affnet_poly(int form, bool stamps), aff_trunk_orinet(int form, bool stamps);
TrunkKernel aff_trunk_hardnet(int form, bool stamps), aff_trunk_hardnet_poly(int form, bool stamps), aff_trunk_hardnet_f43(int form, bool stamps);
int aff_derived_u_ensure(affnet_ctx* ctx);
int aff_derive_u(affnet_ctx* ctx, int kind, int form, const float* packed, const NetLayout& L, hipStream_t st, const float** region);

int aff_finish_affnet(affnet_ctx* ctx, const CnnCall& c, const NetLayout& L, int rows, int B);
int aff_margin_affnet(affnet_ctx* ctx, const CnnCall& c, const NetLayout& L, int rows, int B, int32_t* flags);
int aff_finish_orinet(affnet_ctx* ctx, const CnnCall& c, const NetLayout& L, int rows, int B);
int aff_hardnet_head(affnet_ctx* ctx, const CnnCall& c, const NetLayout& L, int B);

void aff_sqnorm_launch(hipStream_t st, const float* x, int n, int dim, float* out);
void aff_knn_merge_launch(hipStream_t st, const float* part_d, const int32_t* part_i, int n1, int n_lists, int k, float* out_d, int32_t* out_i);
void aff_knn_q8_merge_launch(hipStream_t st, const int32_t* part_d, const int32_t* part_i, int n1, int n_lists, int k, float scale, int32_t* out_d2,
                             float* out_f, int32_t* out_i);

struct AffSkip { int lo, hi; };
static inline AffSkip aff_skip_range(int skip_row, int skip_n, int n2) {
    const long long lo64 = skip_row < 0 ? 0 : skip_row, hi64 = (long long)skip_row + skip_n;
    return {(int)(lo64 < n2 ? lo64 : n2), (int)(hi64 < 0 ? 0 : (hi64 < n2 ? hi64 : n2))};
}

static inline int aff_topk_cap(int k) { return k == 1 ? 1 : (k == 2 ? 2 : (k <= 4 ? 4 : 8)); }
template <typename F>
static inline void aff_topk_dispatch(int k, F f) {
    switch (aff_topk_cap(k)) {
        case 1: f(std::integral_constant<int, 1>()); break;
        case 2: f(std::integral_constant<int, 2>()); break;
        case 4: f(std::integral_constant<int, 4>()); break;
        default: f(std::integral_constant<int, 8>()); break;
    }
}

static inline int aff_chunk_choice(const affnet_ctx* ctx, long long row_blocks, long long units, int workgroups_per_cu, int min_units, int max_chunks) {
    int cus = 256;
    if (ctx) {
        int v = 0;
        if (hipDeviceGetAttribute(&v, hipDeviceAttributeMultiprocessorCount, ctx->device) == hipSuccess && v > 0) cus = v;
        else (void)hipGetLastError();
    }
    const long long want = ((long long)workgroups_per_cu * cus + row_blocks - 1) / row_blocks, most = units / min_units;
    long long nc = want < most ? want : most;
    if (nc > max_chunks) nc = max_chunks;
    return nc < 1 ? 1 : (int)nc;
}

struct AffTile {
    int x0, y0, tw, th;
};

__device__ __forceinline__ AffTile aff_tile_box(float t00, float t01, float t02, float t10, float t11, float t12, int ps, int cap) {
    const float um = (float)(ps - 1) / (float)ps;
    const float hx = (fabsf(t00) + fabsf(t01)) * um, hy = (fabsf(t10) + fabsf(t11)) * um;
    const float cx = t02 - 0.5f, cy = t12 - 0.5f;
    AffTile t;
    t.tw = 0; t.th = 0; t.x0 = 0; t.y0 = 0;
    if (!(hx < 4096.0f && hy < 4096.0f && fabsf(cx) < 1.0e6f && fabsf(cy) < 1.0e6f)) return t;
    const int x0 = (int)floorf(cx - hx) - 1, x1 = (int)floorf(cx + hx) + 2;
    const int y0 = (int)floorf(cy - hy) - 1, y1 = (int)floorf(cy + hy) + 2;
    const int tw = x1 - x0 + 1, th = y1 - y0 + 1;
    if (tw * th > cap || tw * th > 2 * ps * ps) return t;
    t.x0 = x0; t.y0 = y0; t.tw = tw; t.th = th;
    return t;
}

template <int NTHR>
__device__ __forceinline__ void aff_tile_load(float* tile, const AffTile t, const float* __restrict__ img, int h, int w, int tid) {
    const int n = t.tw * t.th;
    for (int i = tid; i < n; i += NTHR) {
        const int ty = i / t.tw, tx = i - ty * t.tw;
        const int gy = t.y0 + ty, gx = t.x0 + tx;
        tile[i] = (gy >= 0 && gy < h && gx >= 0 && gx < w) ? img[(size_t)gy * w + gx] : 0.0f;
    }
}

__device__ __forceinline__ float aff_sample_bilinear(const float* __restrict__ img, int h, int w,
                                                     float t00, float t01, float t02, float t10,
                                                     float t11, float t12, float u, float v) {
    float gx = fmaf(1.0f, t02, fmaf(v, t01, u * t00));
    float gy = fmaf(1.0f, t12, fmaf(v, t11, u * t10));
    const float fw = (float)w, fh = (float)h;
    gx = 2.0f * gx / fw - 1.0f;
    gy = 2.0f * gy / fh - 1.0f;
    const float ix = fmaf(gx + 1.0f, fw * 0.5f, -0.5f);
    const float iy = fmaf(gy + 1.0f, fh * 0.5f, -0.5f);
    const float x0f = floorf(ix), y0f = floorf(iy);
// ... 46 lines not shown
```

### affnet_amd/csrc/context.hip

```cpp
#include <stdarg.h>

#include "common.h"

int aff_fail(affnet_ctx* ctx, int code, const char* fmt, ...) {
    char buf[1024];
    va_list ap;
    va_start(ap, fmt);
    vsnprintf(buf, sizeof(buf), fmt, ap);
    va_end(ap);
    if (ctx) ctx->err = buf;
    return code;
}

__global__ __launch_bounds__(256) void aff_zero_kernel(unsigned char* __restrict__ p, size_t bytes) {
    const size_t head = ((16 - ((size_t)p & 15)) & 15) < bytes ? ((16 - ((size_t)p & 15)) & 15) : bytes;
    const size_t n16 = (bytes - head) / 16, tail0 = head + n16 * 16;
    uint4* q = reinterpret_cast<uint4*>(p + head);
    for (size_t i = (size_t)blockIdx.x * 256 + threadIdx.x; i < n16; i += (size_t)gridDim.x * 256) q[i] = make_uint4(0u, 0u, 0u, 0u);
    if (blockIdx.x == 0) {
        for (size_t i = threadIdx.x; i < head; i += 256) p[i] = 0;
        for (size_t i = tail0 + threadIdx.x; i < bytes; i += 256) p[i] = 0;
    }
}

// ... 120 lines not shown
        g.h = c.oct_h[o]; g.w = c.oct_w[o];
        g.pyr_off = (int64_t)pyr; pyr += (size_t)c.levels_per_octave * g.h * g.w;
        g.map_off = (int64_t)mapb; mapb += aff_align((size_t)g.h * g.w, 16);
        int cap = (int)((size_t)g.h * g.w / div); if (cap < 256) cap = 256;
        g.raw_off = (int64_t)raw; g.raw_cap = cap; raw += cap;
    }
    ctx->B = c.batch > 0 ? c.batch : 1;
    const size_t B = (size_t)ctx->B;
    ctx->pyr_floats = pyr; ctx->map_bytes = mapb; ctx->raw_total = raw; ctx->cand_cap = raw;
    ctx->pyr_stride = aff_align(pyr * sizeof(float)) / sizeof(float);
    ctx->map_stride = aff_align(mapb);
    ctx->raw_stride = raw;
    const int keep = c.max_keep > 0 ? c.max_keep : 65536;
    ctx->cap_pre = c.num_prefilter > 0 ? c.num_prefilter : keep;
    ctx->cap_final = c.num_features > 0 ? c.num_features : ctx->cap_pre;
    if (ctx->cap_final > ctx->cap_pre) ctx->cap_final = ctx->cap_pre;
    size_t off = 0;
    ctx->off_pyr = off; off += B * ctx->pyr_stride * sizeof(float);
    ctx->off_map = off; off += B * ctx->map_stride;
    ctx->off_raw = off; off += aff_align(B * raw * sizeof(RawMax));
    ctx->off_cnt = off; off += aff_align(B * CNT_TOTAL * sizeof(int32_t));
    ctx->off_hist = off; off += aff_align(B * SEL_HIST_BINS * sizeof(uint32_t));
    ctx->off_cand = off; off += aff_align(B * ctx->cand_cap * 7 * sizeof(float));
    ctx->off_sel = off; off += aff_align(B * (size_t)ctx->cap_pre * 7 * sizeof(float));
    ctx->off_stage = off;
    const size_t P = B * (size_t)ctx->cap_pre, F = B * (size_t)ctx->cap_final;
    off += aff_align(P * 10 * sizeof(float));
    off += aff_align(P * 4 * sizeof(float));
    off += aff_align(P * 10 * sizeof(float));
    off += aff_align(P * 2 * sizeof(float));
    off += aff_align(P * sizeof(int32_t));
    off += aff_align(B * sizeof(int32_t));
    off += aff_align(F * 6 * sizeof(float));
    off += aff_align(F * 4 * sizeof(float));
    off += aff_align(F * 9 * sizeof(float));
    {
        const size_t hard = F * (8192 + 4 * 128), aff = P * 144;
        off += aff_align((hard > aff ? hard : aff) * sizeof(float));
    }
    if (c.onepass) {
        if (c.num_prefilter != c.num_features) { *out = ctx; return aff_fail(ctx, AFFNET_ERR_INVALID, "onepass: num_prefilter must equal num_features"); }
        size_t aff = 0;
        for (int o = 0; o < c.n_octaves; ++o) {
            if (c.oct_h[o] < 34 || c.oct_w[o] < 34) {
                *out = ctx;
                return aff_fail(ctx, AFFNET_ERR_INVALID, "onepass: octave %d is %dx%d, LocalNorm2d(33) needs >= 34 px in this library (17 in the reference: use "
                                "border >= 15 like its scripts, so that the pyramid stops earlier)", o, c.oct_w[o], c.oct_h[o]);
            }
            ctx->aff_off[o] = aff; aff += aff_align((size_t)4 * c.oct_h[o] * c.oct_w[o] * sizeof(float)) / sizeof(float);
        }
        ctx->aff_stride = aff;
        ctx->dense_stride = affnet_fullconv_scratch_bytes(c.oct_h[0], c.oct_w[0]) / sizeof(float);
        ctx->off_affmap = off; off += aff_align(B * aff * sizeof(float));
        ctx->off_dense = off; off += aff_align(B * ctx->dense_stride * sizeof(float));
        ctx->off_cand2 = off; off += aff_align(B * ctx->cand_cap * 7 * sizeof(float));
        ctx->off_lvltab = off; off += aff_align(B * (size_t)AFFNET_MAX_OCTAVES * AFFNET_MAX_LEVELS * 4 * sizeof(int32_t));
    }
    ctx->ws_bytes = off;
    *out = ctx;
    return AFFNET_OK;
}

extern "C" void affnet_ctx_destroy(affnet_ctx* ctx) { delete ctx; }

extern "C" int affnet_set_arith(affnet_ctx* ctx, int arith) {
    if (!ctx) return AFFNET_ERR_INVALID;
    if (arith < AFFNET_ARITH_FP32_MFMA || arith > AFFNET_ARITH_FP32_SPLIT2H) return aff_fail(ctx, AFFNET_ERR_INVALID, "arith=%d (AFFNET_ARITH_*)", arith);
    ctx->arith = arith;
    ctx->cfg.arith = arith;
    return AFFNET_OK;
}
extern "C" int affnet_get_arith(const affnet_ctx* ctx) { return ctx ? ctx->arith : AFFNET_ERR_INVALID; }

extern "C" int affnet_set_shape_form(affnet_ctx* ctx, int form) {
    if (!ctx) return AFFNET_ERR_INVALID;
    if (form != AFFNET_SHAPE_FORM_DIRECT && form != AFFNET_SHAPE_FORM_WINOGRAD && form != AFFNET_SHAPE_FORM_POLYPHASE) return aff_fail(ctx, AFFNET_ERR_INVALID, "shape form=%d (AFFNET_SHAPE_FORM_*)", form);
    ctx->shape_form = form;
    return AFFNET_OK;
}
extern "C" int affnet_get_shape_form(const affnet_ctx* ctx) { return ctx ? ctx->shape_form : AFFNET_ERR_INVALID; }

extern "C" int affnet_set_desc_form(affnet_ctx* ctx, int form) {
    if (!ctx) return AFFNET_ERR_INVALID;
    if (form != AFFNET_DESC_FORM_DIRECT && form != AFFNET_DESC_FORM_POLYPHASE && form != AFFNET_DESC_FORM_F43) return aff_fail(ctx, AFFNET_ERR_INVALID, "descriptor form=%d (AFFNET_DESC_FORM_*)", form);
    ctx->desc_form = form;
    return AFFNET_OK;
}
extern "C" int affnet_get_desc_form(const affnet_ctx* ctx) { return ctx ? ctx->desc_form : AFFNET_ERR_INVALID; }

extern "C" size_t affnet_workspace_bytes(const affnet_ctx* ctx) { return ctx ? ctx->ws_bytes : 0; }

extern "C" int affnet_capacity_prefilter(const affnet_ctx* ctx) { return ctx ? ctx->cap_pre : 0; }
extern "C" int affnet_capacity_final(const affnet_ctx* ctx) { return ctx ? ctx->cap_final : 0; }

extern "C" int64_t affnet_pyramid_level_offset(const affnet_ctx* ctx, int octave, int level) {
    if (!ctx || octave < 0 || octave >= ctx->cfg.n_octaves || level < 0 || level >= ctx->cfg.levels_per_octave) return -1;
    const OctaveGeom& g = ctx->oct[octave];
    return (int64_t)(ctx->off_pyr / sizeof(float)) + g.pyr_off + (int64_t)level * g.h * g.w;
}

extern "C" int64_t affnet_pyramid_image_stride(const affnet_ctx* ctx) { return ctx ? (int64_t)ctx->pyr_stride : 0; }

extern "C" int64_t affnet_counter_offset(const affnet_ctx* ctx, int which) {
    if (!ctx || ctx->ws_bytes == 0 || which < 0 || which > 4) return -1;
    const int idx = which == 0 ? CNT_OVERFLOW : (which == 1 ? CNT_DET : (which == 2 ? CNT_SHAPED : (which == 3 ? CNT_AFF_EVAL : CNT_AFF_REEVAL)));
    return (int64_t)(ctx->off_cnt / sizeof(int32_t)) + idx;
}
extern "C" int64_t affnet_counter_stride(const affnet_ctx* ctx) { return ctx ? (int64_t)CNT_TOTAL : 0; }

extern "C" int64_t affnet_affmap_offset(const affnet_ctx* ctx, int octave) {
    if (!ctx || !ctx->cfg.onepass || octave < 0 || octave >= ctx->cfg.n_octaves) return -1;
    return (int64_t)(ctx->off_affmap / sizeof(float)) + (int64_t)ctx->aff_off[octave];
}
extern "C" int64_t affnet_affmap_image_stride(const affnet_ctx* ctx) { return (ctx && ctx->cfg.onepass) ? (int64_t)ctx->aff_stride : 0; }
extern "C" int affnet_batch(const affnet_ctx* ctx) { return ctx ? ctx->B : 0; }

extern "C" int affnet_bind_workspace(affnet_ctx* ctx, void* d_workspace, size_t bytes) {
    if (!ctx) return AFFNET_ERR_INVALID;
    if (!d_workspace || bytes < ctx->ws_bytes)
        return aff_fail(ctx, AFFNET_ERR_INVALID, "workspace too small: %zu < %zu", bytes, ctx->ws_bytes);
    if (((uintptr_t)d_workspace & 255) != 0) return aff_fail(ctx, AFFNET_ERR_INVALID, "workspace must be 256-byte aligned");
    {
        hipPointerAttribute_t at;
        if (hipPointerGetAttributes(&at, d_workspace) == hipSuccess) {
            if (at.type == hipMemoryTypeDevice && at.device != ctx->device)
                return aff_fail(ctx, AFFNET_ERR_INVALID, "workspace belongs to device %d, the context to device %d", at.device, ctx->device);
        } else {
            (void)hipGetLastError();
        }
    }
    char* b = (char*)d_workspace;
    ctx->ws = b;
    ctx->pyr = (float*)(b + ctx->off_pyr);
    ctx->omap = (uint8_t*)(b + ctx->off_map);
    ctx->raw = (RawMax*)(b + ctx->off_raw);
    ctx->cnt = (int32_t*)(b + ctx->off_cnt);
    ctx->sel_hist = (uint32_t*)(b + ctx->off_hist);
    const size_t B = (size_t)ctx->B;
    float* cand = (float*)(b + ctx->off_cand);
    const size_t CC = B * ctx->cand_cap;
    ctx->cand_resp = cand; ctx->cand_syx = cand + CC; ctx->cand_ids = (int32_t*)(cand + 4 * CC);
    float* sel = (float*)(b + ctx->off_sel);
    const size_t P = B * (size_t)ctx->cap_pre, F = B * (size_t)ctx->cap_final;
    ctx->sel_resp = sel; ctx->sel_syx = sel + P; ctx->sel_ids = (int32_t*)(sel + 4 * P);
    char* s = b + ctx->off_stage;
    ctx->st_det_resp = (float*)s; ctx->st_det_lafs = (float*)s + P; ctx->st_det_ids = (int32_t*)((float*)s + 7 * P);
    s += aff_align(P * 10 * sizeof(float));
    ctx->st_A = (float*)s; s += aff_align(P * 4 * sizeof(float));
    ctx->st_A2 = (float*)s; ctx->st_lafs_iter = (float*)s + 4 * P; s += aff_align(P * 10 * sizeof(float));
    ctx->st_key = (float*)s; ctx->st_good = (int32_t*)((float*)s + P); s += aff_align(P * 2 * sizeof(float));
    ctx->st_rank = (int32_t*)s; s += aff_align(P * sizeof(int32_t));
    ctx->st_det_count = (int32_t*)s; s += aff_align(B * sizeof(int32_t));
    ctx->st_lafs_shaped = (float*)s; s += aff_align(F * 6 * sizeof(float));
    ctx->st_R = (float*)s; s += aff_align(F * 4 * sizeof(float));
    ctx->st_lafs_norm = (float*)s; ctx->st_lvl_ids = (int32_t*)((float*)s + 6 * F); s += aff_align(F * 9 * sizeof(float));
    ctx->st_hard_scratch = (float*)s;
    if (ctx->cfg.onepass) {
        ctx->affmap = (float*)(b + ctx->off_affmap);
        ctx->dense = (float*)(b + ctx->off_dense);
        float* c2 = (float*)(b + ctx->off_cand2);
        ctx->cand2_resp = c2; ctx->cand2_syx = c2 + CC; ctx->cand2_ids = (int32_t*)(c2 + 4 * CC);
        ctx->lvltab = (int32_t*)(b + ctx->off_lvltab);
    }
    return AFFNET_OK;
}

extern "C" int affnet_read_counts(affnet_ctx* ctx, int32_t out[4], void* stream) {
// ... 24 lines not shown
```

### affnet_amd/csrc/debug.hip

```cpp
#include "common.h"

#include "../../include/affnet_hip_probes.h"

template <typename T>
__global__ __launch_bounds__(256) void stream_read_kernel(const T* __restrict__ src, float* __restrict__ dst, size_t n_items) {
    float acc = 0.f;
    for (size_t i = (size_t)blockIdx.x * 256 + threadIdx.x; i < n_items; i += (size_t)gridDim.x * 256) {
        const T v = src[i];
        const float* f = reinterpret_cast<const float*>(&v);
#pragma unroll
        for (int k = 0; k < (int)(sizeof(T) / 4); ++k) acc += f[k];
    }
    if (acc == 123.456f) dst[blockIdx.x] = acc;
    if (threadIdx.x == 0 && blockIdx.x == 0) dst[0] = acc;
}

template <typename T>
__global__ __launch_bounds__(256) void stream_write_kernel(T* __restrict__ dst, size_t n_items) {
    T v;
    float* f = reinterpret_cast<float*>(&v);
#pragma unroll
    for (int k = 0; k < (int)(sizeof(T) / 4); ++k) f[k] = (float)(threadIdx.x + k);
    for (size_t i = (size_t)blockIdx.x * 256 + threadIdx.x; i < n_items; i += (size_t)gridDim.x * 256) dst[i] = v;
}
// ... 51 lines not shown
    if (ctx->arith != AFFNET_ARITH_FP32_MFMA) return aff_fail(ctx, AFFNET_ERR_INVALID, "probe_affnet_wino: AFFNET_ARITH_FP32_MFMA only");
    CnnCall c;
    c.kind = AFFNET_NET_AFFNET; c.packed = d_packed; c.patches = d_patches; c.n_max = n; c.st = st;
    c.out = d_out; c.scratch = d_out;
    c.dbg_layer = layer; c.dbg_out = d_out;
    return aff_trunk_launch(ctx, c, net_layout(AFFNET_NET_AFFNET), dim3(n, 1), poly ? 2 : 1, nullptr, 0);
}

extern "C" int affnet_probe_affnet_wino_layer(affnet_ctx* ctx, int net_kind, const float* d_packed, const float* d_patch, int layer, float* d_out, void* stream) {
    AFF_DEVICE(ctx);
    if (!ctx || !d_packed || !d_patch || !d_out || net_kind != AFFNET_NET_AFFNET || layer < 0 || layer > 5)
        return aff_fail(ctx, AFFNET_ERR_INVALID, "probe_affnet_wino_layer: AffNet, layer 0 .. 5");
    return probe_affnet_wino(ctx, d_packed, d_patch, 1, d_out, layer, (hipStream_t)stream);
}

extern "C" int affnet_probe_affnet_wino_partials(affnet_ctx* ctx, const float* d_packed, const float* d_patches, int n, float* d_partials, void* stream) {
    AFF_DEVICE(ctx);
    if (!ctx || !d_packed || !d_patches || !d_partials || n < 1 || n > 65535) return aff_fail(ctx, AFFNET_ERR_INVALID, "probe_affnet_wino_partials: bad argument");
    return probe_affnet_wino(ctx, d_packed, d_patches, n, d_partials, -1, (hipStream_t)stream);
}

extern "C" int affnet_probe_affnet_poly_layer(affnet_ctx* ctx, int net_kind, const float* d_packed, const float* d_patch, int layer, float* d_out, void* stream) {
    AFF_DEVICE(ctx);
    if (!ctx || !d_packed || !d_patch || !d_out || net_kind != AFFNET_NET_AFFNET || layer < 0 || layer > 5)
        return aff_fail(ctx, AFFNET_ERR_INVALID, "probe_affnet_poly_layer: AffNet, layer 0 .. 5");
    return probe_affnet_wino(ctx, d_packed, d_patch, 1, d_out, layer, (hipStream_t)stream, true);
}

extern "C" int affnet_probe_affnet_poly_partials(affnet_ctx* ctx, const float* d_packed, const float* d_patches, int n, float* d_partials, void* stream) {
    AFF_DEVICE(ctx);
    if (!ctx || !d_packed || !d_patches || !d_partials || n < 1 || n > 65535) return aff_fail(ctx, AFFNET_ERR_INVALID, "probe_affnet_poly_partials: bad argument");
    return probe_affnet_wino(ctx, d_packed, d_patches, n, d_partials, -1, (hipStream_t)stream, true);
}

static int probe_derived_u(affnet_ctx* ctx, int kind, int form, const float* d_packed, int offset, int floats, float* d_out, void* stream) {
    const float* u;
    const int rc = aff_derive_u(ctx, kind, form, d_packed, net_layout(kind), (hipStream_t)stream, &u);
    if (rc) return rc;
    return aff_copy_async(ctx, d_out, u + offset, (size_t)floats * sizeof(float), (hipStream_t)stream);
}

extern "C" int affnet_probe_trunk16_poly_u(affnet_ctx* ctx, int net_kind, const float* d_packed, int layer, float* d_out, void* stream) {
    AFF_DEVICE(ctx);
    if (!ctx || !d_packed || !d_out || (net_kind != AFFNET_NET_AFFNET && net_kind != AFFNET_NET_ORINET) || (layer != 2 && layer != 4))
        return aff_fail(ctx, AFFNET_ERR_INVALID, "probe_trunk16_poly_u: AffNet / OriNet, layer 2 or 4");
    return probe_derived_u(ctx, net_kind, net_kind == AFFNET_NET_AFFNET ? TRUNK_WINO_POLY : TRUNK_EXACT, d_packed, Wino16::offset(layer), Wino16::floats(layer), d_out, stream);
}

extern "C" int affnet_probe_hardnet_poly_layer(affnet_ctx* ctx, const float* d_packed, const float* d_patch, int layer, float* d_out, void* stream) {
    AFF_DEVICE(ctx);
    if (!ctx || !d_packed || !d_patch || !d_out || layer < 0 || layer > 5) return aff_fail(ctx, AFFNET_ERR_INVALID, "probe_hardnet_poly_layer: layer 0 .. 5");
    return aff_hardnet_poly_patches(ctx, d_packed, d_patch, 1, d_out, nullptr, layer, (hipStream_t)stream);
}

extern "C" int affnet_probe_hardnet_poly_forward(affnet_ctx* ctx, const float* d_packed, const float* d_patches, int n, float* d_out, float* d_scratch, void* stream) {
    AFF_DEVICE(ctx);
    if (!ctx || !d_packed || !d_patches || !d_out || !d_scratch || n < 1 || n > 65535) return aff_fail(ctx, AFFNET_ERR_INVALID, "probe_hardnet_poly_forward: bad argument");
    return aff_hardnet_poly_patches(ctx, d_packed, d_patches, n, d_out, d_scratch, -1, (hipStream_t)stream);
}

extern "C" int affnet_probe_hardnet_poly_u(affnet_ctx* ctx, const float* d_packed, int layer, float* d_out, void* stream) {
    AFF_DEVICE(ctx);
    if (!ctx || !d_packed || !d_out || (layer != 2 && layer != 4)) return aff_fail(ctx, AFFNET_ERR_INVALID, "probe_hardnet_poly_u: layer 2 or 4");
    return probe_derived_u(ctx, AFFNET_NET_HARDNET, TRUNK_WINO, d_packed, Poly32::offset(layer), Poly32::floats(layer), d_out, stream);
}

extern "C" int affnet_probe_hardnet_f43_layer(affnet_ctx* ctx, const float* d_packed, const float* d_patch, int layer, float* d_out, void* stream) {
    AFF_DEVICE(ctx);
    if (!ctx || !d_packed || !d_patch || !d_out || layer < 0 || layer > 5) return aff_fail(ctx, AFFNET_ERR_INVALID, "probe_hardnet_f43_layer: layer 0 .. 5");
    return aff_hardnet_poly_patches(ctx, d_packed, d_patch, 1, d_out, nullptr, layer, (hipStream_t)stream, AFFNET_DESC_FORM_F43);
}

extern "C" int affnet_probe_hardnet_f43_forward(affnet_ctx* ctx, const float* d_packed, const float* d_patches, int n, float* d_out, float* d_scratch, void* stream) {
    AFF_DEVICE(ctx);
    if (!ctx || !d_packed || !d_patches || !d_out || !d_scratch || n < 1 || n > 65535) return aff_fail(ctx, AFFNET_ERR_INVALID, "probe_hardnet_f43_forward: bad argument");
    return aff_hardnet_poly_patches(ctx, d_packed, d_patches, n, d_out, d_scratch, -1, (hipStream_t)stream, AFFNET_DESC_FORM_F43);
}

extern "C" int affnet_probe_hardnet_f43_u(affnet_ctx* ctx, const float* d_packed, int layer, float* d_out, void* stream) {
    AFF_DEVICE(ctx);
    if (!ctx || !d_packed || !d_out || (layer != 1 && layer != 3)) return aff_fail(ctx, AFFNET_ERR_INVALID, "probe_hardnet_f43_u: layer 1 or 3");
    return probe_derived_u(ctx, AFFNET_NET_HARDNET, TRUNK_WINO_F43, d_packed, F43::BASE + F43::offset(layer), F43::floats(layer), d_out, stream);
}
```

### affnet_amd/csrc/derive_u.hip

```cpp
#include "common.h"

__global__ __launch_bounds__(256) void derive_u_kernel(const float* __restrict__ packed, NetOffsets off, DerivedTable t, float* __restrict__ U) {
    derive_u_pair(t, blockIdx.x * 256 + threadIdx.x, packed, off.w, U);
}

int aff_derived_u_ensure(affnet_ctx* ctx) {
    if (ctx->derived_u) return AFFNET_OK;
    AFF_HIP(ctx, hipMalloc((void**)&ctx->derived_u, (size_t)DerivedU::FLOATS * sizeof(float)));
    return AFFNET_OK;
}

static DerivedTable table_of(int kind, int form) {
    if (kind == AFFNET_NET_HARDNET) return form == TRUNK_WINO ? derived_hardnet_poly() : (form == TRUNK_WINO_F43 ? derived_hardnet_form2() : DerivedTable{});
    const bool wino = kind == AFFNET_NET_ORINET ? form == TRUNK_EXACT : (form == TRUNK_WINO || form == TRUNK_WINO_POLY);
    return wino ? derived_trunk16() : DerivedTable{};
}

int aff_derive_u(affnet_ctx* ctx, int kind, int form, const float* packed, const NetLayout& L, hipStream_t st, const float** region) {
    *region = nullptr;
    const DerivedTable t = table_of(kind, form);
    if (t.n == 0) return AFFNET_OK;
    const int rc = aff_derived_u_ensure(ctx);
    if (rc) return rc;
    float* dst = ctx->derived_u + DerivedU::region(kind);
    hipLaunchKernelGGL(derive_u_kernel, dim3(t.pairs / 256), dim3(256), 0, st, packed, to_offsets(L), t, dst);
    AFF_LAUNCH_CHECK(ctx);
    *region = dst;
    return AFFNET_OK;
}
```

### affnet_amd/csrc/pack_check.cpp

```cpp
#include <math.h>
#include <stdio.h>
#include <string.h>

#include <initializer_list>
#include <memory>

#include "../../include/affnet_hip.h"
#include "weights_layout.h"

#define CHECK(cond) do { if (!(cond)) { fprintf(stderr, "pack_check: line %d: %s\n", __LINE__, #cond); return 1; } } while (0)

struct State {
    std::unique_ptr<float[]> conv[6], mean[6], var[6], head_w, head_b, hbm, hbv, out;
    const float *conv_p[6], *mean_p[6], *var_p[6];
    size_t conv_n[6], total;
};

static uint32_t lcg = 12345u;
static float rnd() { lcg = lcg * 1664525u + 1013904223u; return (float)(lcg >> 8) / (float)(1 << 24) - 0.5f; }
static std::unique_ptr<float[]> filled(size_t n, float scale, float offset) {
    std::unique_ptr<float[]> p(new float[n]);
    for (size_t i = 0; i < n; ++i) p[i] = rnd() * scale + offset;
    return p;
}

static void make_state(int kind, State& s) {
    const int cb = kind == AFFNET_NET_HARDNET ? 32 : 16, ch[7] = {1, cb, cb, 2 * cb, 2 * cb, 4 * cb, 4 * cb};
    for (int i = 0; i < 6; ++i) {
        s.conv_n[i] = (size_t)ch[i + 1] * ch[i] * 9;
        s.conv[i] = filled(s.conv_n[i], 0.2f, 0.f); s.mean[i] = filled(ch[i + 1], 1.f, 0.f); s.var[i] = filled(ch[i + 1], 1.f, 1.f);
        s.conv_p[i] = s.conv[i].get(); s.mean_p[i] = s.mean[i].get(); s.var_p[i] = s.var[i].get();
    }
    const int no = kind == AFFNET_NET_ORINET ? 2 : 3;
    if (kind == AFFNET_NET_HARDNET) { s.head_w = filled((size_t)128 * 128 * 64, 0.02f, 0.f); s.hbm = filled(128, 1.f, 0.f); s.hbv = filled(128, 1.f, 1.f); }
    else { s.head_w = filled((size_t)no * 64 * 64, 0.1f, 0.f); s.head_b = filled(no, 1.f, 0.f); }
    s.total = affnet_cnn32_packed_floats(kind);
    s.out.reset(new float[s.total]);
}

static int pack(int kind, State& s) {
    return affnet_cnn32_pack_weights(kind, s.conv_p, s.mean_p, s.var_p, s.head_w.get(), s.head_b.get(), s.hbm.get(), s.hbv.get(), s.out.get());
}

static int check_kind(int kind) {
    State s;
    make_state(kind, s);
    CHECK(s.total > 0 && pack(kind, s) == AFFNET_OK);
    size_t nonfinite = 0;
    for (size_t i = 0; i < s.total; ++i) nonfinite += !isfinite(s.out[i]);
    CHECK(nonfinite == 0);
    int64_t want = -1;
    for (int layer = -1; layer <= 6; ++layer) {
        const bool has = kind == AFFNET_NET_HARDNET && (layer == 1 || layer == 3 || layer == 5);
        const int64_t got = affnet_cnn32_winograd_offset(kind, layer);
        if (!has) { CHECK(got == -1); continue; }
        if (want < 0) want = (int64_t)s.total - 16 * (32 * 32 + 64 * 64 + 128 * 128);
        CHECK(got == want);
        want += 16 * (layer == 1 ? 32 * 32 : layer == 3 ? 64 * 64 : 128 * 128);
    }
    CHECK(affnet_cnn32_winograd_offset(-1, 1) == -1 && affnet_cnn32_winograd_offset(4, 1) == -1 && affnet_cnn32_packed_floats(-1) == 0 && affnet_cnn32_packed_floats(4) == 0);
    float* const o = s.out.get();
    const float *hw = s.head_w.get(), *hb = s.head_b.get(), *m = s.hbm.get(), *v = s.hbv.get();
    CHECK(affnet_cnn32_pack_weights(kind, nullptr, s.mean_p, s.var_p, hw, hb, m, v, o) == AFFNET_ERR_INVALID);
    CHECK(affnet_cnn32_pack_weights(kind, s.conv_p, nullptr, s.var_p, hw, hb, m, v, o) == AFFNET_ERR_INVALID);
    CHECK(affnet_cnn32_pack_weights(kind, s.conv_p, s.mean_p, nullptr, hw, hb, m, v, o) == AFFNET_ERR_INVALID);
    CHECK(affnet_cnn32_pack_weights(kind, s.conv_p, s.mean_p, s.var_p, nullptr, hb, m, v, o) == AFFNET_ERR_INVALID);
    CHECK(affnet_cnn32_pack_weights(kind, s.conv_p, s.mean_p, s.var_p, hw, hb, m, v, nullptr) == AFFNET_ERR_INVALID);
    CHECK(affnet_cnn32_pack_weights(-1, s.conv_p, s.mean_p, s.var_p, hw, hb, m, v, o) == AFFNET_ERR_INVALID);
    CHECK(affnet_cnn32_pack_weights(4, s.conv_p, s.mean_p, s.var_p, hw, hb, m, v, o) == AFFNET_ERR_INVALID);
    if (kind == AFFNET_NET_HARDNET) {
        CHECK(affnet_cnn32_pack_weights(kind, s.conv_p, s.mean_p, s.var_p, hw, hb, nullptr, v, o) == AFFNET_ERR_INVALID);
        CHECK(affnet_cnn32_pack_weights(kind, s.conv_p, s.mean_p, s.var_p, hw, hb, m, nullptr, o) == AFFNET_ERR_INVALID);
    } else {
        CHECK(affnet_cnn32_pack_weights(kind, s.conv_p, s.mean_p, s.var_p, hw, nullptr, m, v, o) == AFFNET_ERR_INVALID);
    }
    int edges = 0;
    const float saved = s.conv[3][7], saved_var = s.var[2][1];
    for (const float x : {INFINITY, NAN}) { s.conv[3][7] = x; CHECK(pack(kind, s) == AFFNET_OK); ++edges; }
    s.conv[3][7] = saved;
    s.var[2][1] = 0.f; CHECK(pack(kind, s) == AFFNET_OK); ++edges;
    s.var[2][1] = saved_var;
    for (const float scale : {0.f, 1e-30f, 1e30f}) {
        for (int i = 0; i < 6; ++i)
            for (size_t j = 0; j < s.conv_n[i]; ++j) s.conv[i][j] = scale * ((j & 1) ? -1.f : 1.f);
        CHECK(pack(kind, s) == AFFNET_OK); ++edges;
    }
    printf("kind %d: %zu floats packed, %d edge cases and the rejected arguments as documented\n", kind, s.total, edges);
    return 0;
}

static_assert(Wino16::offset(1) == 0 && Wino16::offset(3) == 4096 && Wino16::offset(5) == 20480 && Wino16::offset(2) == 86016 && Wino16::offset(4) == 98816 && Wino16::FLOATS == 150016 && Wino16::PAIRS == 7936, "Wino16");
static_assert(Poly32::offset(2) == 0 && Poly32::offset(4) == 51200 && Poly32::FLOATS == 256000 && Poly32::PAIRS == 10240, "Poly32");
static_assert(F43::BASE == 256000 && F43::offset(1) == 0 && F43::offset(3) == 36864 && F43::FLOATS == 184320 && F43::PAIRS == 5120, "F43");

static int check_derived(const char* name, int kind, const DerivedTable& t, int want_sections, size_t want_floats) {
    const NetLayout L = net_layout(kind); const NetOffsets off = to_offsets(L);
    CHECK(L.total == affnet_cnn32_packed_floats(kind) && t.n == want_sections && t.n <= DERIVED_MAX && (size_t)t.floats == want_floats && t.pairs % 256 == 0);
    const std::unique_ptr<float[]> blob = filled(L.total, 0.2f, 0.f), U(new float[want_floats]), want(new float[want_floats]);
    const std::unique_ptr<unsigned char[]> owned(new unsigned char[want_floats]());
    const float sentinel = -12345.f;
    for (size_t i = 0; i < want_floats; ++i) U[i] = sentinel;
    size_t pairs = 0, floats = 0;
    for (int i = 0; i < t.n; ++i) {
        const DerivedSection& s = t.s[i];
        const int xi = s.family == DERIVED_WINO ? 16 : s.family == DERIVED_POLY ? 25 : 36;
        CHECK(s.layer >= 1 && s.layer <= 5 && s.cin == L.cin[s.layer] && s.cout == L.cout[s.layer] && (size_t)s.pair0 == pairs && s.family >= 0 && s.family <= DERIVED_F43);
        for (int c = 0; c < s.cin; ++c)
            for (int n = 0; n < s.cout; ++n, ++pairs) {
                float g[9], u[36];
                for (int tap = 0; tap < 9; ++tap) g[tap] = blob[L.w_off[s.layer] + w_tap_index(tap, c, n, s.cin, s.cout)];
                if (s.family == DERIVED_WINO) wino_weight_transform(g, u);
                else if (s.family == DERIVED_POLY) poly_weight_transform(g, u);
                else f43_weight_transform(g, u);
                const size_t e = s.pair0 + w_tap_index(0, c, n, s.cin, s.cout);
                CHECK(e < (size_t)t.pairs);
                for (int p = 0; p < xi; ++p, ++floats) {
                    const size_t d = s.dst + w_tap_index(p, c, n, s.cin, s.cout);
                    CHECK(d < want_floats && !owned[d] && U[d] == sentinel);
                    owned[d] = 1; want[d] = u[p];
                }
                derive_u_pair(t, (int)e, blob.get(), off.w, U.get());
            }
    }
    for (int e = t.pairs; e < t.pairs + 256; ++e) derive_u_pair(t, e, blob.get(), off.w, U.get());
    CHECK(pairs == (size_t)t.pairs && floats == want_floats && memcmp(U.get(), want.get(), want_floats * sizeof(float)) == 0);
    printf("derived %s: %d sections, %d pairs, %zu floats: every float written once, by its own pair, with its transform\n", name, t.n, t.pairs, want_floats);
    return 0;
}

static int check_regions() {
    const size_t t16 = derived_trunk16().floats, poly = derived_hardnet_poly().floats, f43 = derived_hardnet_f43().floats;
    CHECK(DerivedU::AFFNET == 0 && DerivedU::ORINET == t16 && DerivedU::HARDNET == 2 * t16 && DerivedU::HARDNET_F43 == 2 * t16 + poly && DerivedU::FLOATS == 2 * t16 + poly + f43);
    CHECK(DerivedU::region(AFFNET_NET_AFFNET) == DerivedU::AFFNET && DerivedU::region(AFFNET_NET_ORINET) == DerivedU::ORINET && DerivedU::region(AFFNET_NET_HARDNET) == DerivedU::HARDNET);
    CHECK(derived_hardnet_form2().floats == poly + f43);
    return 0;
}

int main() {
    for (int kind = 0; kind <= AFFNET_NET_AFFNET_FULLCONV; ++kind)
        if (check_kind(kind)) return 1;
    if (check_derived("AffNet", AFFNET_NET_AFFNET, derived_trunk16(), 5, 150016) || check_derived("OriNet", AFFNET_NET_ORINET, derived_trunk16(), 5, 150016) ||
        check_derived("HardNet polyphase", AFFNET_NET_HARDNET, derived_hardnet_poly(), 2, 256000) || check_derived("HardNet F(4x4, 3x3)", AFFNET_NET_HARDNET, derived_hardnet_f43(), 2, 184320) ||
        check_derived("HardNet form 2", AFFNET_NET_HARDNET, derived_hardnet_form2(), 4, 256000 + 184320) || check_regions())
        return 1;
    return 0;
}
```

### affnet_amd/csrc/weights_layout.h

```cpp
#pragma once
#include <stddef.h>
#include <stdint.h>

#include "../../include/affnet_hip.h"

#ifdef __HIPCC__
#define AFF_HOST_DEVICE __host__ __device__
#else
#define AFF_HOST_DEVICE
#endif

#define HEAD_K 8192
#define H2_TAIL 4
#define S3_LAYER_MASK 0x3E

constexpr size_t w_tap_index(int p, int c, int n, int cin, int cout) {
    return ((((size_t)p * (cin / 16) + c / 16) * 4 + (c / 4) % 4) * cout + n) * 4 + c % 4;
}

constexpr size_t w_split_index(int tap, int c, int term, int n, int cin, int cout, int terms) {
    const int step = cin == 16 ? tap / 2 : tap * (cin / 32) + c / 32;
    const int kq = cin == 16 ? (tap % 2) * 2 + c / 8 : (c % 32) / 8;
    return ((((size_t)step * terms + term) * 4 + kq) * cout + n) * 8 + c % 8;
}
// ... 62 lines not shown
};

static inline NetOffsets to_offsets(const NetLayout& L, int arith = AFFNET_ARITH_FP32_SPLIT3) {
    NetOffsets o;
    const bool h2 = arith == AFFNET_ARITH_FP32_SPLIT2H;
    for (int i = 0; i < 6; ++i) { o.w[i] = (int)L.w_off[i]; o.b[i] = (int)L.b_off[i]; }
    o.head_w = (int)L.head_w; o.head_b = (int)L.head_b;
    for (int i = 0; i < 6; ++i) o.w_s3[i] = (int)(h2 ? L.w_h2[i] : L.w_s3[i]);
    o.head_s3 = (int)(h2 ? L.head_h2 : L.head_s3);
    for (int i = 0; i < 3; ++i) o.w_wino[i] = (int)L.w_wino[2 * i + 1];
    return o;
}

#define TFEAT_K1 52
#define TFEAT_HEAD_K 4096
constexpr size_t tfeat_c1_index(int k, int n) { return (size_t)k * 32 + n; }
constexpr size_t tfeat_c2_index(int p, int c, int n) { return w_tap_index(p, c, n, 32, 64); }
constexpr size_t tfeat_head_index(int pixel, int c, int n) { return w_tap_index(0, pixel * 64 + c, n, TFEAT_HEAD_K, 128); }

struct TfeatLayout {
    size_t c1_w, c1_b, c2_w, c2_b, head_w, head_b, total;
};

static inline TfeatLayout tfeat_layout() {
    TfeatLayout L;
    size_t off = 0;
    L.c1_w = off; off += (size_t)TFEAT_K1 * 32;
    L.c1_b = off; off += 32;
    L.c2_w = off; off += (size_t)36 * 32 * 64;
    L.c2_b = off; off += 64;
    L.head_w = off; off += (size_t)TFEAT_HEAD_K * 128;
    L.head_b = off; off += 128;
    L.total = off;
    return L;
}

AFF_HOST_DEVICE inline void wino_g_axis(float g0, float g1, float g2, float* o, int stride) {
    const float s = g0 + g2;
    o[0] = g0; o[stride] = 0.5f * (s + g1); o[2 * stride] = 0.5f * (s - g1); o[3 * stride] = g2;
}
AFF_HOST_DEVICE inline void wino_weight_transform(const float g[9], float U[16]) {
    float t[12];
#pragma unroll
    for (int ky = 0; ky < 3; ++ky) wino_g_axis(g[3 * ky], g[3 * ky + 1], g[3 * ky + 2], t + 4 * ky, 1);
#pragma unroll
    for (int j = 0; j < 4; ++j) wino_g_axis(t[j], t[4 + j], t[8 + j], U + j, 4);
}

#define POLY_XI 25
AFF_HOST_DEVICE inline void poly_weight_transform(const float g[9], float U[POLY_XI]) {
    float t[3][3];
#pragma unroll
    for (int ky = 0; ky < 3; ++ky) { t[ky][0] = g[3 * ky]; t[ky][1] = g[3 * ky] + g[3 * ky + 2]; t[ky][2] = g[3 * ky + 2]; }
#pragma unroll
    for (int j = 0; j < 3; ++j) {
        const float s = t[0][j] + t[2][j];
        U[j] = t[0][j]; U[3 + j] = s; U[6 + j] = t[2][j];
        U[15 + j] = t[1][j]; U[18 + j] = t[1][j];
    }
    const float se = g[1] + g[7];
#pragma unroll
    for (int j = 0; j < 2; ++j) {
        U[9 + j] = g[1]; U[11 + j] = se; U[13 + j] = g[7];
        U[21 + j] = g[4]; U[23 + j] = g[4];
    }
}

#define F43_XI 36
AFF_HOST_DEVICE inline void f43_g_axis(float g0, float g1, float g2, float* o, int stride) {
    const float c6 = 1.0f / 6.0f, c12 = 1.0f / 12.0f, c24 = 1.0f / 24.0f;
    const float s = g0 + g2;
    const float p = c24 * g0 + c6 * g2, q = c12 * g1;
    o[0] = 0.25f * g0; o[stride] = -c6 * (s + g1); o[2 * stride] = -c6 * (s - g1);
    o[3 * stride] = p + q; o[4 * stride] = p - q; o[5 * stride] = g2;
}
AFF_HOST_DEVICE inline void f43_weight_transform(const float g[9], float U[F43_XI]) {
    float t[18];
#pragma unroll
    for (int ky = 0; ky < 3; ++ky) f43_g_axis(g[3 * ky], g[3 * ky + 1], g[3 * ky + 2], t + 6 * ky, 1);
#pragma unroll
    for (int j = 0; j < 6; ++j) f43_g_axis(t[j], t[6 + j], t[12 + j], U + j, 6);
}

enum { DERIVED_WINO = 0, DERIVED_POLY = 1, DERIVED_F43 = 2 };
constexpr int derived_xi(int family) { return family == DERIVED_WINO ? 16 : (family == DERIVED_POLY ? POLY_XI : F43_XI); }
struct DerivedSection {
    int layer, cin, cout;
    int family;
    int pair0;
    int dst;
};
constexpr int derived_floats(const DerivedSection& s) { return derived_xi(s.family) * s.cin * s.cout; }
#define DERIVED_MAX 5
struct DerivedTable {
    int n, pairs, floats;
    DerivedSection s[DERIVED_MAX];
};
constexpr DerivedTable derived_add(DerivedTable t, int cb, int layer, int family) {
    const DerivedSection s = {layer, cb << ((layer - 1) / 2), cb << (layer / 2), family, t.pairs, t.floats};
    t.s[t.n++] = s; t.pairs += s.cin * s.cout; t.floats += derived_floats(s);
    return t;
}
constexpr DerivedTable derived_trunk16() {
    return derived_add(derived_add(derived_add(derived_add(derived_add(DerivedTable{}, 16, 1, DERIVED_WINO), 16, 3, DERIVED_WINO), 16, 5, DERIVED_WINO), 16, 2, DERIVED_POLY), 16, 4, DERIVED_POLY);
}
constexpr DerivedTable derived_hardnet_poly() { return derived_add(derived_add(DerivedTable{}, 32, 2, DERIVED_POLY), 32, 4, DERIVED_POLY); }
constexpr DerivedTable derived_hardnet_f43() { return derived_add(derived_add(DerivedTable{}, 32, 1, DERIVED_F43), 32, 3, DERIVED_F43); }
constexpr DerivedTable derived_hardnet_form2() { return derived_add(derived_add(derived_hardnet_poly(), 32, 1, DERIVED_F43), 32, 3, DERIVED_F43); }
constexpr DerivedSection derived_layer(const DerivedTable& t, int layer) {
    for (int i = 0; i < t.n; ++i)
        if (t.s[i].layer == layer) return t.s[i];
    return DerivedSection{-1, 0, 0, 0, 0, 0};
}
constexpr DerivedSection derived_section(const DerivedTable& t, int e) {
    DerivedSection s = t.s[0];
    for (int i = 1; i < DERIVED_MAX; ++i)
        if (i < t.n && e >= t.s[i].pair0) s = t.s[i];
    return s;
}
constexpr bool derived_by_workgroups(const DerivedTable& t, int i = 0) {
    return i == t.n || (t.s[i].pair0 % 256 == 0 && t.s[i].cin * t.s[i].cout % 256 == 0 && derived_by_workgroups(t, i + 1));
}
static_assert(derived_by_workgroups(derived_trunk16()) && derived_by_workgroups(derived_hardnet_poly()) && derived_by_workgroups(derived_hardnet_f43()) &&
              derived_by_workgroups(derived_hardnet_form2()), "a 256-thread workgroup of derive_u_kernel stays within one section");

template <DerivedTable (*T)()>
struct DerivedView {
    static constexpr int FLOATS = T().floats, PAIRS = T().pairs;
    static constexpr int offset(int layer) { return derived_layer(T(), layer).dst; }
    static constexpr int floats(int layer) { return derived_floats(derived_layer(T(), layer)); }
};
struct Wino16 : DerivedView<derived_trunk16> { static constexpr int NB1 = 2, NB3 = 1; };
typedef DerivedView<derived_hardnet_poly> Poly32;
struct F43 : DerivedView<derived_hardnet_f43> { static constexpr int BASE = Poly32::FLOATS; };
static_assert(derived_hardnet_form2().s[2].dst == F43::BASE + F43::offset(1) && derived_hardnet_form2().s[3].dst == F43::BASE + F43::offset(3) &&
              derived_hardnet_form2().floats == F43::BASE + F43::FLOATS, "form 2's table = Poly32 with F43 at F43::BASE");

struct DerivedU {
    static constexpr int AFFNET = 0, ORINET = AFFNET + Wino16::FLOATS;
    static constexpr int HARDNET = ORINET + Wino16::FLOATS;
    static constexpr int HARDNET_F43 = HARDNET + F43::BASE;
    static constexpr int FLOATS = HARDNET_F43 + F43::FLOATS;
    static constexpr int region(int kind) { return kind == AFFNET_NET_AFFNET ? AFFNET : (kind == AFFNET_NET_ORINET ? ORINET : HARDNET); }
};
static_assert(DerivedU::AFFNET == 0 && DerivedU::ORINET - DerivedU::AFFNET == derived_trunk16().floats && DerivedU::HARDNET - DerivedU::ORINET == derived_trunk16().floats &&
              DerivedU::FLOATS - DerivedU::HARDNET == derived_hardnet_form2().floats && DerivedU::FLOATS == 2 * Wino16::FLOATS + Poly32::FLOATS + F43::FLOATS,
              "the regions are disjoint, in this order, and fill the buffer");
static_assert(DerivedU::ORINET % 64 == 0 && DerivedU::HARDNET % 64 == 0 && DerivedU::HARDNET_F43 % 64 == 0, "every region starts on a 256-byte boundary, as an allocation of its own would");
static_assert(w_tap_index(7, 21, 13, 32, 64) == 7 * 32 * 64 + w_tap_index(0, 21, 13, 32, 64) && w_tap_index(35, 63, 63, 64, 64) == 35 * 64 * 64 + w_tap_index(0, 63, 63, 64, 64),
              "a position is a plane of cin * cout floats");
AFF_HOST_DEVICE inline void derive_u_pair(const DerivedTable& t, int e, const float* packed, const int (&w_off)[6], float* U) {
    if (e >= t.pairs) return;
    const DerivedSection s = derived_section(t, e & ~255);
    const int plane = s.cin * s.cout;
    const float* src = packed + w_off[s.layer] + (e - s.pair0);
    float* dst = U + s.dst + (e - s.pair0);
    float g[9];
#pragma unroll
    for (int tap = 0; tap < 9; ++tap) g[tap] = src[(size_t)tap * plane];
    float u[F43_XI];
    if (s.family == DERIVED_WINO) wino_weight_transform(g, u);
    else if (s.family == DERIVED_POLY) poly_weight_transform(g, u);
    else f43_weight_transform(g, u);
#pragma unroll
    for (int xi = 0; xi < F43_XI; ++xi)
        if (xi < derived_xi(s.family)) dst[(size_t)xi * plane] = u[xi];
}
```

### affnet_amd/engine.py

```python
import ctypes as C

import numpy as np
import torch

from . import _lib
from ._lib import lib, check, ptr
from .host_plan import PyramidPlan

_UTILITY = {}


def require_cuda(t, what="tensor"):
    if not (isinstance(t, torch.Tensor) and t.is_cuda):
        raise RuntimeError("affnet_amd: %s must live on the MI355X (tensor.cuda()); this implementation has no CPU path" % what)


def utility_ctx(device, arith=0):
    idx = device.index if device.index is not None else torch.cuda.current_device()
    key = (idx, _lib.arith_code(arith))
    if key not in _UTILITY:
        h = C.c_void_p()
        check(lib.affnet_ctx_create(C.byref(h), idx, None), None, "affnet_ctx_create(utility)")
        check(lib.affnet_set_arith(h, key[1]), h, "affnet_set_arith")
        _UTILITY[key] = h
    h = _UTILITY[key]
    if lib.affnet_get_arith(h) != key[1]:
        check(lib.affnet_set_arith(h, key[1]), h, "affnet_set_arith")
    return h


def stream_of(device):
    return C.c_void_p(torch.cuda.current_stream(device).cuda_stream)


class Context(object):

    def __init__(self, height, width, device, n_levels, init_sigma, border, mr_size, threshold,
                 num_features, num_prefilter, max_keep=16384, batch=1, baum_iters=0, raw_div=4, onepass=False, lazy_shape_rows=-1, arith=0):
        self.plan = PyramidPlan(height, width, n_levels, init_sigma, border)
        self.batch = int(batch)
        self.onepass = bool(onepass)
        self.cfg = self.plan.fill_config(mr_size, threshold, num_features, num_prefilter, max_keep, raw_div=raw_div, batch=self.batch, baum_iters=baum_iters,
                                         onepass=onepass, lazy_shape_rows=lazy_shape_rows, arith=arith)
        self.arith = _lib.arith_code(arith)
        self.shape_form = _lib.SHAPE_FORM_WINOGRAD
        self.desc_form = _lib.DESC_FORM_F43
        self.device = device
        self.handle = C.c_void_p()
        idx = device.index if device.index is not None else torch.cuda.current_device()
        rc = lib.affnet_ctx_create(C.byref(self.handle), idx, C.byref(self.cfg))
        check(rc, self.handle, "affnet_ctx_create")
        nbytes = lib.affnet_workspace_bytes(self.handle)
        self.workspace = torch.empty(nbytes, dtype=torch.uint8, device=device)
        check(lib.affnet_bind_workspace(self.handle, ptr(self.workspace), nbytes), self.handle, "affnet_bind_workspace")
        self.cap_pre = lib.affnet_capacity_prefilter(self.handle)
        self.cap_final = lib.affnet_capacity_final(self.handle)
        self._ws_f32 = self.workspace.view(torch.float32)

    def set_arith(self, arith):
        self.arith = _lib.arith_code(arith)
        check(lib.affnet_set_arith(self.handle, self.arith), self.handle, "affnet_set_arith")

    def set_shape_form(self, form):
        check(lib.affnet_set_shape_form(self.handle, int(form)), self.handle, "affnet_set_shape_form")
        self.shape_form = int(form)

    def set_desc_form(self, form):
        check(lib.affnet_set_desc_form(self.handle, int(form)), self.handle, "affnet_set_desc_form")
        self.desc_form = int(form)

    def pyramid_views(self, image=0):
        pyr = []
        base = image * lib.affnet_pyramid_image_stride(self.handle)
        for o, (h, w) in enumerate(self.plan.sizes):
            levels = []
            for l in range(self.plan.levels_per_octave):
                off = base + lib.affnet_pyramid_level_offset(self.handle, o, l)
                levels.append(self._ws_f32[off:off + h * w].view(1, 1, h, w))
            pyr.append(levels)
        return pyr

    def affmap_views(self, image=0):
        base = image * lib.affnet_affmap_image_stride(self.handle)
        out = []
        for o, (h, w) in enumerate(self.plan.sizes):
            off = base + lib.affnet_affmap_offset(self.handle, o)
            out.append(self._ws_f32[off:off + 4 * h * w].view(1, 4, h, w))
        return out

    def counter_view(self, which=0):
        off, stride = lib.affnet_counter_offset(self.handle, which), lib.affnet_counter_stride(self.handle)
        return self.workspace.view(torch.int32)[off:off + stride * self.batch:stride]

    def read_counts(self, allow_empty=False):
        out = (C.c_int32 * 4)()
        rc = lib.affnet_read_counts(self.handle, C.byref(out), stream_of(self.device))
        if not (allow_empty and rc == _lib.ERR_EMPTY):
            check(rc, self.handle, "affnet_read_counts")
        return list(out)

    def __del__(self):
        try:
            if self.handle:
                lib.affnet_ctx_destroy(self.handle)
                self.handle = None
        except Exception:
            pass


def pack_state_dict(kind, sd, winograd=False):
    conv_idx, bn_idx = (0, 3, 6, 9, 12, 15), (1, 4, 7, 10, 13, 16)

    def f32(name):
        return sd[name].detach().to("cpu", torch.float32).contiguous()

    keep = []
    convs = [f32("features.%d.weight" % i) for i in conv_idx]
    means = [f32("features.%d.running_mean" % i) for i in bn_idx]
    vars_ = [f32("features.%d.running_var" % i) for i in bn_idx]
    head_w = f32("features.19.weight")
    head_b = f32("features.19.bias") if "features.19.bias" in sd else None
    if kind == _lib.NET_AFFNET_FULLCONV and head_b is None:
        raise ValueError("AffNetFastFullConv: features.19.bias missing from the state dict")
    hbm = f32("features.20.running_mean") if kind == _lib.NET_HARDNET else None
    hbv = f32("features.20.running_var") if kind == _lib.NET_HARDNET else None
    keep += convs + means + vars_ + [head_w, head_b, hbm, hbv]
    arr = lambda ts: (C.c_void_p * 6)(*[t.data_ptr() for t in ts])
    n = lib.affnet_cnn32_packed_floats(kind)
    out = torch.empty(n, dtype=torch.float32)
# ... 77 lines not shown
```

### include/affnet_hip.h

```cpp
#ifndef AFFNET_HIP_H
#define AFFNET_HIP_H

#include <stddef.h>
#include <stdint.h>

#ifdef __cplusplus
extern "C" {
#endif

#define AFFNET_OK 0
#define AFFNET_ERR_INVALID (-1)
#define AFFNET_ERR_HIP (-2)
#define AFFNET_ERR_CAPACITY (-3)
#define AFFNET_ERR_EMPTY (-4)

#define AFFNET_MAX_OCTAVES 16
#define AFFNET_MAX_LEVELS 8
#define AFFNET_MAX_TAPS 37

#define AFFNET_NET_AFFNET 0
#define AFFNET_NET_ORINET 1
#define AFFNET_NET_HARDNET 2
#define AFFNET_NET_AFFNET_FULLCONV 3

#define AFFNET_ARITH_FP32_MFMA 0
#define AFFNET_ARITH_FP32_SPLIT3 1
#define AFFNET_ARITH_FP32_SPLIT2H 2

typedef struct affnet_ctx affnet_ctx;

typedef struct affnet_config {
    int32_t height, width;
    int32_t n_octaves;
    int32_t levels_per_octave;
    int32_t oct_h[AFFNET_MAX_OCTAVES];
    int32_t oct_w[AFFNET_MAX_OCTAVES];
    float level_sigma[AFFNET_MAX_OCTAVES][AFFNET_MAX_LEVELS];
    float level_sigma4[AFFNET_MAX_OCTAVES][AFFNET_MAX_LEVELS];
    double level_sigma_px[AFFNET_MAX_OCTAVES][AFFNET_MAX_LEVELS];
    int32_t first_blur_taps;
    float first_blur[AFFNET_MAX_TAPS * AFFNET_MAX_TAPS];
    int32_t level_blur_taps[AFFNET_MAX_LEVELS];
    float level_blur[AFFNET_MAX_LEVELS][AFFNET_MAX_TAPS * AFFNET_MAX_TAPS];
    int32_t level_blur0_taps[AFFNET_MAX_LEVELS];
    float level_blur0[AFFNET_MAX_LEVELS][AFFNET_MAX_TAPS * AFFNET_MAX_TAPS];
    int32_t lazy_shape_rows;
    int32_t onepass;
    float mr_size;
    float threshold;
    int32_t num_features;
    int32_t num_prefilter;
    int32_t max_raw_per_octave_div;
    int32_t max_keep;
    int32_t batch;
    int32_t baum_iters;
    int32_t arith;
} affnet_config;

int affnet_config_fill(affnet_config* cfg, int height, int width, int n_levels, double init_sigma, int border, double mr_size,
                       double threshold, int num_features, int num_prefilter, int batch, int baum_iters);


int affnet_ctx_create(affnet_ctx** out, int device, const affnet_config* cfg);
void affnet_ctx_destroy(affnet_ctx* ctx);
const char* affnet_last_error(const affnet_ctx* ctx);
const char* affnet_version(void);
int affnet_set_arith(affnet_ctx* ctx, int arith);
int affnet_get_arith(const affnet_ctx* ctx);

#define AFFNET_SHAPE_FORM_DIRECT 0
#define AFFNET_SHAPE_FORM_WINOGRAD 1
#define AFFNET_SHAPE_FORM_POLYPHASE 2
int affnet_set_shape_form(affnet_ctx* ctx, int form);
int affnet_get_shape_form(const affnet_ctx* ctx);

#define AFFNET_DESC_FORM_DIRECT 0
#define AFFNET_DESC_FORM_POLYPHASE 1
#define AFFNET_DESC_FORM_F43 2
int affnet_set_desc_form(affnet_ctx* ctx, int form);
int affnet_get_desc_form(const affnet_ctx* ctx);

size_t affnet_workspace_bytes(const affnet_ctx* ctx);
int affnet_bind_workspace(affnet_ctx* ctx, void* d_workspace, size_t bytes);
int64_t affnet_pyramid_level_offset(const affnet_ctx* ctx, int octave, int level);
int64_t affnet_pyramid_image_stride(const affnet_ctx* ctx);
int affnet_batch(const affnet_ctx* ctx);
int affnet_capacity_prefilter(const affnet_ctx* ctx);
int affnet_capacity_final(const affnet_ctx* ctx);


int affnet_gauss_blur(affnet_ctx* ctx, const float* d_in, float* d_out, int h, int w,
                      const float* h_taps, int k, void* stream);

int affnet_pyramid_build(affnet_ctx* ctx, const float* d_img, void* stream);

int affnet_hessian_response(affnet_ctx* ctx, const float* d_in, float* d_out, int h, int w,
                            float sigma4, void* stream);

int affnet_detect(affnet_ctx* ctx, float* d_resp, float* d_lafs, int32_t* d_ids,
                  int32_t* d_count, void* stream);

int affnet_detect_responses(affnet_ctx* ctx, const float* d_responses, float* d_resp, float* d_lafs, int32_t* d_ids,
                            int32_t* d_count, void* stream);

int affnet_laf_grid_sample(affnet_ctx* ctx, const float* d_img, int h, int w,
                           const float* d_lafs, int n, int ps, float* d_out, void* stream);

int affnet_pyr_grid_sample(affnet_ctx* ctx, const float* d_lafs, const int32_t* d_ids,
                           const int32_t* d_count, int n_max, int ps, float* d_out, void* stream);


size_t affnet_cnn32_packed_floats(int net_kind);
int64_t affnet_cnn32_winograd_offset(int net_kind, int layer);
int affnet_cnn32_pack_weights(int net_kind, const float* const* conv_w, const float* const* bn_mean,
                              const float* const* bn_var, const float* head_w, const float* head_b,
                              const float* head_bn_mean, const float* head_bn_var, float* h_out);

int affnet_cnn32_forward(affnet_ctx* ctx, int net_kind, const float* d_packed, const float* d_patches,
                         const int32_t* d_count, int n_max, float* d_out, float* d_scratch, void* stream);

int affnet_cnn32_forward_pyr(affnet_ctx* ctx, int net_kind, const float* d_packed, const float* d_lafs,
                             const int32_t* d_ids, const int32_t* d_count, int n_max, float* d_out,
                             float* d_scratch, void* stream);


int affnet_local_norm(affnet_ctx* ctx, const float* d_in, float* d_out, int h, int w, void* stream);

size_t affnet_fullconv_scratch_bytes(int h, int w);

int affnet_fullconv_forward(affnet_ctx* ctx, const float* d_packed, const float* d_img, int h, int w, float* d_out, float* d_scratch,
                            void* stream);

int affnet_nms2d(affnet_ctx* ctx, const float* d_in, float* d_out, int h, int w, float threshold, void* stream);


#define AFFNET_HC_ORIENTATION 0
#define AFFNET_HC_BAUMBERG 1

int affnet_handcrafted_forward(affnet_ctx* ctx, int kind, const float* d_patches, int n, const float* h_weights, float* d_out,
                               float* d_angles, void* stream);
int affnet_handcrafted_forward_pyr(affnet_ctx* ctx, int kind, const float* d_lafs, const int32_t* d_ids, const int32_t* d_count,
                                   int n_max, const float* h_weights, float* d_out, void* stream);


int affnet_sift_host_window(int patch_size, float* h_out);
int affnet_sift_forward(affnet_ctx* ctx, const float* d_patches, int n, const float* d_window, float clipval, float* d_desc, void* stream);
int affnet_sift_forward_pyr(affnet_ctx* ctx, const float* d_lafs_norm, const int32_t* d_ids, const int32_t* d_count, int n_max,
                            const float* d_window, float clipval, float* d_desc, void* stream);


size_t affnet_tfeat_packed_floats(void);
int affnet_tfeat_pack_weights(const float* conv1_w, const float* conv1_b, const float* conv2_w, const float* conv2_b, const float* cls_w,
                              const float* cls_b, float* h_out);
size_t affnet_tfeat_scratch_floats(int rows);
int affnet_tfeat_forward(affnet_ctx* ctx, const float* d_packed, const float* d_patches, const int32_t* d_count, int n_max, float* d_desc,
                         float* d_scratch, void* stream);
int affnet_tfeat_forward_pyr(affnet_ctx* ctx, const float* d_packed, const float* d_lafs_norm, const int32_t* d_ids, const int32_t* d_count,
                             int n_max, float* d_desc, float* d_scratch, void* stream);


int affnet_shape_filter_select(affnet_ctx* ctx, const float* d_resp_in, const float* d_lafs_in,
// ... 166 lines not shown
```

### include/affnet_hip_probes.h

```cpp
#ifndef AFFNET_HIP_PROBES_H
#define AFFNET_HIP_PROBES_H

#include "affnet_hip.h"

#ifdef __cplusplus
extern "C" {
#endif

int affnet_cnn32_probe(const float* d_packed, int layer, int probe, int reps, int n_blocks, float* d_out, void* stream);

int affnet_debug_stream(const void* d_src, void* d_dst, size_t n_bytes, int width, int mode, int halo, void* stream);

int affnet_split3_gemm(const float* d_A, const float* d_Bt, int M, int N, int K, int mode, float* d_C, void* stream);
int affnet_split3_rate(int reps, int terms, int n_blocks, float* d_out, void* stream);

int affnet_probe_shape_offsets(const affnet_ctx* ctx, int64_t out[3]);

int affnet_probe_affnet_wino_layer(affnet_ctx* ctx, int net_kind, const float* d_packed, const float* d_patch, int layer, float* d_out, void* stream);

int affnet_probe_affnet_wino_partials(affnet_ctx* ctx, const float* d_packed, const float* d_patches, int n, float* d_partials, void* stream);

int affnet_probe_affnet_poly_layer(affnet_ctx* ctx, int net_kind, const float* d_packed, const float* d_patch, int layer, float* d_out, void* stream);
int affnet_probe_affnet_poly_partials(affnet_ctx* ctx, const float* d_packed, const float* d_patches, int n, float* d_partials, void* stream);
int affnet_probe_trunk16_poly_u(affnet_ctx* ctx, int net_kind, const float* d_packed, int layer, float* d_out, void* stream);

int affnet_probe_hardnet_poly_layer(affnet_ctx* ctx, const float* d_packed, const float* d_patch, int layer, float* d_out, void* stream);
int affnet_probe_hardnet_poly_forward(affnet_ctx* ctx, const float* d_packed, const float* d_patches, int n, float* d_out, float* d_scratch, void* stream);
int affnet_probe_hardnet_poly_u(affnet_ctx* ctx, const float* d_packed, int layer, float* d_out, void* stream);

int affnet_probe_hardnet_f43_layer(affnet_ctx* ctx, const float* d_packed, const float* d_patch, int layer, float* d_out, void* stream);
int affnet_probe_hardnet_f43_forward(affnet_ctx* ctx, const float* d_packed, const float* d_patches, int n, float* d_out, float* d_scratch, void* stream);
int affnet_probe_hardnet_f43_u(affnet_ctx* ctx, const float* d_packed, int layer, float* d_out, void* stream);

#ifdef __cplusplus
}
#endif
#endif
```

Before: 1.678 million.

## Add F(2x4,3x3) Winograd form for HardNet conv1 and make it default

Adds a new descriptor form that runs HardNet's first 32->32 3x3 conv (layer 1) as a mixed Winograd F(2x4,3x3): an F(4,3) transform along x and an F(2,3) transform along y. Each wave covers 16 tiles of 2x4 against both channel blocks. Transformed weights are derived into a new region of the U buffer, and the other layers keep the F43/polyphase paths. The default desc_form becomes this new form. The aim is fewer MFMA operations and less LDS traffic than the previous conv1 path, at the cost of a new LDS layout, more register pressure and a hand-tuned instruction schedule.

```diff
diff --git a/affnet_amd/SparseImgRepresenter.py b/affnet_amd/SparseImgRepresenter.py
--- a/affnet_amd/SparseImgRepresenter.py
+++ b/affnet_amd/SparseImgRepresenter.py
@@ -42,7 +42,7 @@
         self.lazy_shape_rows = -1
         self.shape_form = 1
 
-        self.desc_form = 2
+        self.desc_form = 3
 
     def _context(self, x, allow_batch=False):
         engine.require_cuda(x, "image")
diff --git a/affnet_amd/_lib.py b/affnet_amd/_lib.py
--- a/affnet_amd/_lib.py
+++ b/affnet_amd/_lib.py
@@ -23,7 +23,7 @@
         raise ValueError("arith must be AFFNET_ARITH_FP32_MFMA (0), AFFNET_ARITH_FP32_SPLIT3 (1) or AFFNET_ARITH_FP32_SPLIT2H (2)")
     return int(arith)
 SHAPE_FORM_DIRECT, SHAPE_FORM_WINOGRAD, SHAPE_FORM_POLYPHASE = 0, 1, 2
-DESC_FORM_DIRECT, DESC_FORM_POLYPHASE, DESC_FORM_F43 = 0, 1, 2
+DESC_FORM_DIRECT, DESC_FORM_POLYPHASE, DESC_FORM_F43, DESC_FORM_F24 = 0, 1, 2, 3
 OK, ERR_INVALID, ERR_HIP, ERR_CAPACITY, ERR_EMPTY = 0, -1, -2, -3, -4
 VERIFY_AFFINE, VERIFY_HOMOGRAPHY, VERIFY_TILE, VERIFY_CHUNK = 0, 1, 128, 128
 KNN_MAX_K = 8
@@ -182,6 +182,9 @@
     "affnet_probe_hardnet_f43_layer": (_I, [_P, _P, _P, _I, _P, _P]),
     "affnet_probe_hardnet_f43_forward": (_I, [_P, _P, _P, _I, _P, _P, _P]),
     "affnet_probe_hardnet_f43_u": (_I, [_P, _P, _I, _P, _P]),
+    "affnet_probe_hardnet_f24_layer": (_I, [_P, _P, _P, _I, _P, _P]),
+    "affnet_probe_hardnet_f24_forward": (_I, [_P, _P, _P, _I, _P, _P, _P]),
+    "affnet_probe_hardnet_f24_u": (_I, [_P, _P, _I, _P, _P]),
 }
 
 
diff --git a/affnet_amd/csrc/cnn32.hip b/affnet_amd/csrc/cnn32.hip
--- a/affnet_amd/csrc/cnn32.hip
+++ b/affnet_amd/csrc/cnn32.hip
@@ -27,10 +27,10 @@
 TrunkKernel aff_trunk_kernel(int kind, int form, bool stamps) {
     typedef TrunkKernel (*Unit)(int, bool);
     static_assert(AFFNET_NET_AFFNET == 0 && AFFNET_NET_ORINET == 1 && AFFNET_NET_HARDNET == 2 && TRUNK_EXACT == 0 && TRUNK_WINO == 1 && TRUNK_SPLIT2 == 2 && TRUNK_SPLIT3 == 3 &&
-                  TRUNK_WINO_F43 == 4 && TRUNK_WINO_POLY == 5 && TRUNK_FORMS == 6, "order of the table");
-    static const Unit unit[3][TRUNK_FORMS] = {{aff_trunk_affnet, aff_trunk_affnet, aff_trunk_affnet, aff_trunk_affnet, nullptr, aff_trunk_affnet_poly},
-                                              {aff_trunk_orinet, nullptr, aff_trunk_orinet, aff_trunk_orinet, nullptr, nullptr},
-                                              {aff_trunk_hardnet, aff_trunk_hardnet_poly, aff_trunk_hardnet, aff_trunk_hardnet, aff_trunk_hardnet_f43, nullptr}};
+                  TRUNK_WINO_F43 == 4 && TRUNK_WINO_POLY == 5 && TRUNK_WINO_F24 == 6 && TRUNK_FORMS == 7, "order of the table");
+    static const Unit unit[3][TRUNK_FORMS] = {{aff_trunk_affnet, aff_trunk_affnet, aff_trunk_affnet, aff_trunk_affnet, nullptr, aff_trunk_affnet_poly, nullptr},
+                                              {aff_trunk_orinet, nullptr, aff_trunk_orinet, aff_trunk_orinet, nullptr, nullptr, nullptr},
+                                              {aff_trunk_hardnet, aff_trunk_hardnet_poly, aff_trunk_hardnet, aff_trunk_hardnet, aff_trunk_hardnet_f43, nullptr, aff_trunk_hardnet_f24}};
     if (kind < 0 || kind > 2 || form < 0 || form >= TRUNK_FORMS || !unit[kind][form]) return nullptr;
     return unit[kind][form](form, stamps);
 }
@@ -39,7 +39,7 @@
     int form = TRUNK_EXACT;
     if (ctx->arith != AFFNET_ARITH_FP32_MFMA) form = ctx->arith == AFFNET_ARITH_FP32_SPLIT2H ? TRUNK_SPLIT2 : TRUNK_SPLIT3;
     else if (c.kind == AFFNET_NET_AFFNET && wino) form = wino == 2 ? TRUNK_WINO_POLY : TRUNK_WINO;
-    else if (c.kind == AFFNET_NET_HARDNET && c.desc_form != AFFNET_DESC_FORM_DIRECT) form = c.desc_form == AFFNET_DESC_FORM_F43 ? TRUNK_WINO_F43 : TRUNK_WINO;
+    else if (c.kind == AFFNET_NET_HARDNET && c.desc_form != AFFNET_DESC_FORM_DIRECT) form = c.desc_form == AFFNET_DESC_FORM_F24 ? TRUNK_WINO_F24 : (c.desc_form == AFFNET_DESC_FORM_F43 ? TRUNK_WINO_F43 : TRUNK_WINO);
     const bool stamps = ctx->dbg_time || c.dbg_layer >= 0;
     const TrunkKernel kernel = aff_trunk_kernel(c.kind, form, stamps);
     if (!kernel) return aff_fail(ctx, AFFNET_ERR_INVALID, "cnn32: no trunk kernel of net %d in form %d is built", c.kind, form);
diff --git a/affnet_amd/csrc/cnn_mfma.h b/affnet_amd/csrc/cnn_mfma.h
--- a/affnet_amd/csrc/cnn_mfma.h
+++ b/affnet_amd/csrc/cnn_mfma.h
@@ -1085,18 +1085,21 @@
     static constexpr int V_FLOATS = 4 * F43_XI * 256;
     static constexpr int X = 0, X_FLOATS = 8 * 8 * 256;
 };
-__device__ __forceinline__ void f43_bt_lo(float d0, float d1, float d2, float d3, float d4, float& v0, float& v1, float& v2) {
+template <typename T>
+__device__ __forceinline__ void f43_bt_lo(T d0, T d1, T d2, T d3, T d4, T& v0, T& v1, T& v2) {
     v0 = (4.0f * d0 - 5.0f * d2) + d4;
-    const float a = d4 - 4.0f * d2, b = d3 - 4.0f * d1;
+    const T a = d4 - 4.0f * d2, b = d3 - 4.0f * d1;
     v1 = a + b; v2 = a - b;
 }
-__device__ __forceinline__ void f43_bt_hi(float d1, float d2, float d3, float d4, float d5, float& v3, float& v4, float& v5) {
-    const float c = d4 - d2, e = 2.0f * (d3 - d1);
+template <typename T>
+__device__ __forceinline__ void f43_bt_hi(T d1, T d2, T d3, T d4, T d5, T& v3, T& v4, T& v5) {
+    const T c = d4 - d2, e = 2.0f * (d3 - d1);
     v3 = c + e; v4 = c - e;
     v5 = (4.0f * d1 - 5.0f * d3) + d5;
 }
-__device__ __forceinline__ void f43_at_axis(float m0, float m1, float m2, float m3, float m4, float m5, float& y0, float& y1, float& y2, float& y3) {
-    const float p = m1 + m2, q = m1 - m2, r = m3 + m4, s = m3 - m4;
+template <typename T>
+__device__ __forceinline__ void f43_at_axis(T m0, T m1, T m2, T m3, T m4, T m5, T& y0, T& y1, T& y2, T& y3) {
+    const T p = m1 + m2, q = m1 - m2, r = m3 + m4, s = m3 - m4;
     y0 = (m0 + p) + r; y1 = q + 2.0f * s; y2 = p + 4.0f * r; y3 = q + (8.0f * s + m5);
 }
 
@@ -1230,6 +1233,143 @@
         const f32x4 v = bias_relu(y[k], bias);
         *reinterpret_cast<f32x4*>(&act[((wave >> 1) * 4 + (lane >> 4)) * LO::PSG + ((oy + (k >> 2) + 1) * LO::WP + ox + (k & 3) + 1) * 4]) = v;
     }
+}
+
+typedef Lay<32, 34, 4628> LayC0F;
+
+__device__ __forceinline__ void f24_tile(int wave, int m, int& ty, int& tx) { ty = 2 * wave + (m >> 3); tx = m & 7; }
+
+template <int CIN, int COUT>
+__device__ __forceinline__ void f24_prefetch_u(const float* __restrict__ Wu, f32x4 (&U)[2][3], int lane) {
+    const __amdgpu_buffer_rsrc_t r = weight_rsrc(Wu, F24_XI * CIN * COUT);
+    const int u_lane = ((lane >> 4) * COUT + (lane & 15)) * 16;
+#pragma unroll
+    for (int k = 0; k < 3; ++k)
+#pragma unroll
+        for (int c = 0; c < 2; ++c) U[c][k] = wino_load_u<CIN, COUT>(r, u_lane, k, 0, c);
+}
+
+template <typename LI>
+__device__ __forceinline__ void f24_read_rows(unsigned ab, int i, f32x4 (&da)[6], f32x4 (&db)[6]) {
+    const int ra = wino_row_a(i), rb = wino_row_b(i);
+#pragma unroll
+    for (int c = 0; c < 6; ++c) { da[c] = lds_read4(ab + (ra * LI::WP + c) * 16); db[c] = lds_read4(ab + (rb * LI::WP + c) * 16); }
+}
+
+__device__ __forceinline__ void f24_transform_row(int i, const f32x4 (&da)[6], const f32x4 (&db)[6], f32x4 (&V)[6]) {
+    f32x4 t[6];
+#pragma unroll
+    for (int c = 0; c < 6; ++c)
+#pragma unroll
+        for (int e = 0; e < 4; ++e) t[c][e] = i == 1 ? wadd(da[c][e], db[c][e]) : wsub(da[c][e], db[c][e]);
+#pragma unroll
+    for (int e = 0; e < 4; ++e) {
+        float v[6];
+        f43_bt_lo(t[0][e], t[1][e], t[2][e], t[3][e], t[4][e], v[0], v[1], v[2]);
+        f43_bt_hi(t[1][e], t[2][e], t[3][e], t[4][e], t[5][e], v[3], v[4], v[5]);
+#pragma unroll
+        for (int j = 0; j < 6; ++j) { asm("" : "+v"(v[j])); V[j][e] = v[j]; }
+    }
+}
+
+template <int NW, int CIN, int COUT, typename LI>
+__device__ __forceinline__ void conv3x3_f24_mfma_pair_rows(const float* act, const float* __restrict__ Wu, f32x4 (&U)[2][3], f32x4 (&y)[2][2][4], int wave, int lane) {
+    constexpr int NGRP = CIN / 16, NSTEP = 4 * NGRP;
+    static_assert(LI::H == 32 && NW == 8 && COUT == 32 && CIN % 16 == 0 && NSTEP % 2 == 0, "8 blocks of 16 tiles of 2 x 4, one per wave, against two channel blocks");
+    const int m = lane & 15, kq = lane >> 4;
+    const __amdgpu_buffer_rsrc_t wrsrc = weight_rsrc(Wu, F24_XI * CIN * COUT);
+    const int u_lane = (kq * COUT + m) * 16;
+    int ty, tx;
+    f24_tile(wave, m, ty, tx);
+    const unsigned a0 = lds_byte_addr(act) + (kq * LI::PSG + (2 * ty * LI::WP + 4 * tx) * 4) * 4;
+    f32x4 acc[2][6], Va[6], Vb[6];
+    auto window_addr = [&](int G) {
+        unsigned ab = a0 + 4 * G * LI::PSG * 4;
+        asm("" : "+v"(ab));
+        return ab;
+    };
+    auto step = [&](int s, const f32x4 (&V)[6], f32x4 (&Vn)[6]) {
+        const int i = s / NGRP, G = s % NGRP;
+        const bool more = s + 1 < NSTEP;
+        const int sn = more ? s + 1 : s;
+        const int in = sn / NGRP, Gn = sn % NGRP;
+        unsigned abn = 0;
+        if (more) abn = window_addr(Gn);
+        if (G == 0) {
+#pragma unroll
+            for (int c = 0; c < 2; ++c)
+#pragma unroll
+                for (int k = 0; k < 6; ++k) acc[c][k] = (f32x4){0.f, 0.f, 0.f, 0.f};
+        }
+        __builtin_amdgcn_sched_barrier(0);
+        f32x4 da[6], db[6];
+        if (more) f24_read_rows<LI>(abn, in, da, db);
+#pragma unroll
+        for (int k = 0; k < 6; ++k) {
+#pragma unroll
+            for (int s4 = 0; s4 < 4; ++s4) {
+                acc[0][k] = __builtin_amdgcn_mfma_f32_16x16x4f32(U[0][k % 3][s4], V[k][s4], acc[0][k], 0, 0, 0);
+                acc[1][k] = __builtin_amdgcn_mfma_f32_16x16x4f32(U[1][k % 3][s4], V[k][s4], acc[1][k], 0, 0, 0);
+            }
+            U[0][k % 3] = k < 3 ? wino_load_u<CIN, COUT>(wrsrc, u_lane, 6 * i + k + 3, G, 0) : wino_load_u<CIN, COUT>(wrsrc, u_lane, 6 * in + k - 3, Gn, 0);
+            U[1][k % 3] = k < 3 ? wino_load_u<CIN, COUT>(wrsrc, u_lane, 6 * i + k + 3, G, 1) : wino_load_u<CIN, COUT>(wrsrc, u_lane, 6 * in + k - 3, Gn, 1);
+        }
+        if (more) {
+            f24_transform_row(in, da, db, Vn);
+#pragma unroll
+            for (int l = 0; l < 48; ++l) {
+                __builtin_amdgcn_sched_group_barrier(0x008, 1, 0);
+                if (l < 12) __builtin_amdgcn_sched_group_barrier(0x100, 1, 0);
+                if (l >= 8 && (l < 16 || (l & 1))) __builtin_amdgcn_sched_group_barrier(0x002, 3, 0);
+                else if (l >= 8) __builtin_amdgcn_sched_group_barrier(0x002, 2, 0);
+                if (l % 8 == 7) __builtin_amdgcn_sched_group_barrier(0x020, 2, 0);
+            }
+        }
+        __builtin_amdgcn_sched_barrier(0);
+        if (G == NGRP - 1) {
+#pragma unroll
+            for (int c = 0; c < 2; ++c) {
+                f32x4 yc[4];
+                f43_at_axis(acc[c][0], acc[c][1], acc[c][2], acc[c][3], acc[c][4], acc[c][5], yc[0], yc[1], yc[2], yc[3]);
+#pragma unroll
+                for (int col = 0; col < 4; ++col) {
+                    if (i == 0) y[c][0][col] = yc[col];
+                    else if (i == 1) { y[c][0][col] = y[c][0][col] + yc[col]; y[c][1][col] = yc[col]; }
+                    else if (i == 2) { y[c][0][col] = y[c][0][col] + yc[col]; y[c][1][col] = y[c][1][col] - yc[col]; }
+                    else y[c][1][col] = y[c][1][col] - yc[col];
+                    if (i < 3) asm volatile("" : "+v"(y[c][0][col]));
+                    if (i > 0) asm volatile("" : "+v"(y[c][1][col]));
+                }
+            }
+            __builtin_amdgcn_sched_barrier(0);
+        }
+    };
+    {
+        f32x4 da[6], db[6];
+        f24_read_rows<LI>(window_addr(0), 0, da, db);
+        f24_transform_row(0, da, db, Va);
+    }
+#pragma unroll
+    for (int s = 0; s < NSTEP; s += 2) {
+        step(s, Va, Vb);
+        step(s + 1, Vb, Va);
+    }
+}
+
+template <typename LO>
+__device__ __forceinline__ void f24_store_lds(float* act, const f32x4 (&bias)[2], const f32x4 (&y)[2][2][4], int wave, int lane) {
+    const int g = lane >> 4;
+    int ty, tx;
+    f24_tile(wave, lane & 15, ty, tx);
+#pragma unroll
+    for (int c = 0; c < 2; ++c)
+#pragma unroll
+        for (int r = 0; r < 2; ++r)
+#pragma unroll
+            for (int col = 0; col < 4; ++col) {
+                const f32x4 v = bias_relu(y[c][r][col], bias[c]);
+                *reinterpret_cast<f32x4*>(&act[(c * 4 + g) * LO::PSG + ((2 * ty + r + 1) * LO::WP + 4 * tx + col + 1) * 4]) = v;
+            }
 }
 
 template <int NW, int CIN, int COUT, int H, int NB>
diff --git a/affnet_amd/csrc/cnn_trunk.h b/affnet_amd/csrc/cnn_trunk.h
--- a/affnet_amd/csrc/cnn_trunk.h
+++ b/affnet_amd/csrc/cnn_trunk.h
@@ -168,11 +168,12 @@
 template <int KIND, int S3>
 struct TrunkTraits {
     static_assert(S3 == TRUNK_EXACT || S3 == TRUNK_SPLIT2 || S3 == TRUNK_SPLIT3 || (S3 == TRUNK_WINO && KIND != AFFNET_NET_ORINET) ||
-                  (S3 == TRUNK_WINO_F43 && KIND == AFFNET_NET_HARDNET) || (S3 == TRUNK_WINO_POLY && KIND == AFFNET_NET_AFFNET), "no such trunk form of this net (common.h: TRUNK_*)");
+                  ((S3 == TRUNK_WINO_F43 || S3 == TRUNK_WINO_F24) && KIND == AFFNET_NET_HARDNET) || (S3 == TRUNK_WINO_POLY && KIND == AFFNET_NET_AFFNET), "no such trunk form of this net (common.h: TRUNK_*)");
     static constexpr bool EXACT = S3 != TRUNK_SPLIT2 && S3 != TRUNK_SPLIT3;
     static constexpr bool WINO13 = (S3 == TRUNK_EXACT && KIND == AFFNET_NET_ORINET) || ((S3 == TRUNK_WINO || S3 == TRUNK_WINO_POLY) && KIND == AFFNET_NET_AFFNET);
     static constexpr bool POLY16 = (S3 == TRUNK_EXACT && KIND == AFFNET_NET_ORINET) || (S3 == TRUNK_WINO_POLY && KIND == AFFNET_NET_AFFNET);
-    static constexpr bool POLY = (S3 == TRUNK_WINO || S3 == TRUNK_WINO_F43) && KIND == AFFNET_NET_HARDNET, F43_3 = S3 == TRUNK_WINO_F43 && KIND == AFFNET_NET_HARDNET;
+    static constexpr bool POLY = (S3 == TRUNK_WINO || S3 == TRUNK_WINO_F43 || S3 == TRUNK_WINO_F24) && KIND == AFFNET_NET_HARDNET;
+    static constexpr bool F43_3 = (S3 == TRUNK_WINO_F43 || S3 == TRUNK_WINO_F24) && KIND == AFFNET_NET_HARDNET, F24_1 = S3 == TRUNK_WINO_F24 && KIND == AFFNET_NET_HARDNET;
 };
 
 template <int C, typename L, int NTHR>
@@ -199,7 +200,8 @@
 template <int KIND, int NW, bool STAMPS, int S3 = 0>
 __global__ __launch_bounds__(NW * 64, (KIND == AFFNET_NET_HARDNET) ? NW / 4 : 4) void cnn32_trunk_kernel(CnnArgs a, PyrSrc ps) {
     using F = TrunkTraits<KIND, S3>;
-    constexpr bool EXACT = F::EXACT, WINO13 = F::WINO13, POLY16 = F::POLY16, POLY = F::POLY, F43_3 = F::F43_3;
+    constexpr bool EXACT = F::EXACT, WINO13 = F::WINO13, POLY16 = F::POLY16, POLY = F::POLY, F43_3 = F::F43_3, F24_1 = F::F24_1;
+    using L0 = std::conditional_t<F24_1, LayC0F, LayC0>;
     using S = TrunkShape<KIND, NW>;
     constexpr int CB = S::CB, NTHR = S::NTHR;
     static_assert((CB / 4) * LayC1::PSG <= TrunkLds<CB>::ACT && (CB / 2) * LayC3::PSG <= TrunkLds<CB>::ACT, "LDS layout");
@@ -259,7 +261,7 @@
         const int y = e < 34 ? 0 : (e < 68 ? 33 : 1 + ((e - 68) >> 1)), x = e < 34 ? e : (e < 68 ? e - 34 : ((e - 68) & 1) * 33);
         patch[y * WP32 + x] = 0.0f;
     }
-    if constexpr (EXACT) zero_halo<LayC0, NTHR>(act, CB);
+    if constexpr (EXACT) zero_halo<L0, NTHR>(act, CB);
     else if constexpr (S3 == TRUNK_SPLIT2) zero_halo_q<typename SplitLays<CB>::LR0, NTHR>(act);
     else zero_halo_q<typename SplitLays<CB>::LQH, NTHR>(act);
     float sum = 0.f;
@@ -286,22 +288,41 @@
         f32x4 Up[2][4];
         f32x4 Uw[16];
         f32x4 Uf[18];
+        f32x4 Ug[2][3];
         {
             f32x4 acc[T1M][T1N];
             conv0_mfma<NW, CB, T1M, T1N>(patch, w0, bias0, acc, wave, lane);
             CNN_STAMP(19);
-            store_tiles_lds<CB, LayC0, T1M, T1N, false>(act, bias0, acc, wave, lane);
+            store_tiles_lds<CB, L0, T1M, T1N, false>(act, bias0, acc, wave, lane);
             CNN_STAMP(20);
-            wino_prefetch_u_pair<NW, CB, CB, 32, NB1>(a.packed + a.off.w_wino[0], Up, wave, lane);
-            __syncthreads();
-        }
-        if (STAMPS && a.dbg_layer == 0) { dump_planes<CB, LayC0, NTHR>(act, a.dbg_out); return; }
+            if constexpr (F24_1) f24_prefetch_u<CB, CB>(a.wino_u + F24::BASE + F24::offset(1), Ug, lane);
+            else wino_prefetch_u_pair<NW, CB, CB, 32, NB1>(a.packed + a.off.w_wino[0], Up, wave, lane);
+            __syncthreads();
+        }
+        if (STAMPS && a.dbg_layer == 0) { dump_planes<CB, L0, NTHR>(act, a.dbg_out); return; }
         CNN_STAMP(2);
 
         f32x4 b2[S::G2][T2N];
         f32x4 bias2[T2N];
         f32x4 P2a[2][3], P2b[2][3];
-        {
+        if constexpr (F24_1) {
+            static_assert(CB == 32 && (CB / 4) * LayC0F::PSG <= TrunkLds<CB>::ACT, "conv1: two channel blocks; conv0's output in LayC0F fits the activation buffer");
+            f32x4 y[2][2][4], bw[2];
+            __builtin_amdgcn_s_setprio(0);
+            conv3x3_f24_mfma_pair_rows<NW, CB, CB, LayC0F>(act, a.wino_u + F24::BASE + F24::offset(1), Ug, y, wave, lane);
+            __builtin_amdgcn_s_setprio(3);
+            CNN_STAMP(3);
+            poly_prefetch_u<NW, CB, 2 * CB, 16, NBP2, 2>(a.wino_u + Poly32::offset(2), P2a, P2b, wave, lane);
+#pragma unroll
+            for (int c = 0; c < 2; ++c) bw[c] = *reinterpret_cast<const f32x4*>(&a.packed[a.off.b[1] + c * 16 + 4 * (lane >> 4)]);
+            __syncthreads();
+            CNN_STAMP(21);
+            zero_halo<LayC1, NTHR>(act, CB);
+            f24_store_lds<LayC1>(act, bw, y, wave, lane);
+            CNN_STAMP(22);
+            __syncthreads();
+            CNN_STAMP(4);
+        } else {
             f32x4 y[NB1][4], bw[NB1];
             __builtin_amdgcn_s_setprio(0);
             conv3x3_wino_mfma_pair_rows<NW, CB, CB, LayC0, NB1>(act, a.packed + a.off.w_wino[0], Up, y, wave, lane);
diff --git a/affnet_amd/csrc/cnn_trunk_hardnet_f24.hip b/affnet_amd/csrc/cnn_trunk_hardnet_f24.hip
--- /dev/null
+++ b/affnet_amd/csrc/cnn_trunk_hardnet_f24.hip
@@ -0,0 +1,3 @@
+#include "cnn_trunk.h"
+
+TrunkKernel aff_trunk_hardnet_f24(int form, bool stamps) { return trunk_unit<AFFNET_NET_HARDNET, TRUNK_WINO_F24>(form, stamps); }
diff --git a/affnet_amd/csrc/common.h b/affnet_amd/csrc/common.h
--- a/affnet_amd/csrc/common.h
+++ b/affnet_amd/csrc/common.h
@@ -104,7 +104,7 @@
     hipGraph_t graph = nullptr;
     hipGraphExec_t graph_exec = nullptr;
     float* derived_u = nullptr;
-    int desc_form = AFFNET_DESC_FORM_F43;
+    int desc_form = AFFNET_DESC_FORM_F24;
     ~affnet_ctx() {
         if (derived_u) (void)hipFree(derived_u);
         if (graph_exec) (void)hipGraphExecDestroy(graph_exec);
@@ -224,7 +224,8 @@
 constexpr int TRUNK_SPLIT3 = 3;
 constexpr int TRUNK_WINO_F43 = 4;
 constexpr int TRUNK_WINO_POLY = 5;
-constexpr int TRUNK_FORMS = 6;
+constexpr int TRUNK_WINO_F24 = 6;
+constexpr int TRUNK_FORMS = 7;
 
 __device__ __forceinline__ bool lazy_skip(const int32_t* skip_cnt, int skip_n, int image, int which = CNT_SURVIVED1) {
     if (!skip_cnt) return false;
@@ -296,7 +297,7 @@
 int aff_trunk_launch(affnet_ctx* ctx, const CnnCall& c, const NetLayout& L, dim3 grid, int wino, const int32_t* reeval, int shape_op);
 
 TrunkKernel aff_trunk_affnet(int form, bool stamps), aff_trunk_affnet_poly(int form, bool stamps), aff_trunk_orinet(int form, bool stamps);
-TrunkKernel aff_trunk_hardnet(int form, bool stamps), aff_trunk_hardnet_poly(int form, bool stamps), aff_trunk_hardnet_f43(int form, bool stamps);
+TrunkKernel aff_trunk_hardnet(int form, bool stamps), aff_trunk_hardnet_poly(int form, bool stamps), aff_trunk_hardnet_f43(int form, bool stamps), aff_trunk_hardnet_f24(int form, bool stamps);
 int aff_derived_u_ensure(affnet_ctx* ctx);
 int aff_derive_u(affnet_ctx* ctx, int kind, int form, const float* packed, const NetLayout& L, hipStream_t st, const float** region);
 
diff --git a/affnet_amd/csrc/context.hip b/affnet_amd/csrc/context.hip
--- a/affnet_amd/csrc/context.hip
+++ b/affnet_amd/csrc/context.hip
@@ -226,7 +226,7 @@
 
 extern "C" int affnet_set_desc_form(affnet_ctx* ctx, int form) {
     if (!ctx) return AFFNET_ERR_INVALID;
-    if (form != AFFNET_DESC_FORM_DIRECT && form != AFFNET_DESC_FORM_POLYPHASE && form != AFFNET_DESC_FORM_F43) return aff_fail(ctx, AFFNET_ERR_INVALID, "descriptor form=%d (AFFNET_DESC_FORM_*)", form);
+    if (form != AFFNET_DESC_FORM_DIRECT && form != AFFNET_DESC_FORM_POLYPHASE && form != AFFNET_DESC_FORM_F43 && form != AFFNET_DESC_FORM_F24) return aff_fail(ctx, AFFNET_ERR_INVALID, "descriptor form=%d (AFFNET_DESC_FORM_*)", form);
     ctx->desc_form = form;
     return AFFNET_OK;
 }
diff --git a/affnet_amd/csrc/debug.hip b/affnet_amd/csrc/debug.hip
--- a/affnet_amd/csrc/debug.hip
+++ b/affnet_amd/csrc/debug.hip
@@ -157,3 +157,21 @@
     if (!ctx || !d_packed || !d_out || (layer != 1 && layer != 3)) return aff_fail(ctx, AFFNET_ERR_INVALID, "probe_hardnet_f43_u: layer 1 or 3");
     return probe_derived_u(ctx, AFFNET_NET_HARDNET, TRUNK_WINO_F43, d_packed, F43::BASE + F43::offset(layer), F43::floats(layer), d_out, stream);
 }
+
+extern "C" int affnet_probe_hardnet_f24_layer(affnet_ctx* ctx, const float* d_packed, const float* d_patch, int layer, float* d_out, void* stream) {
+    AFF_DEVICE(ctx);
+    if (!ctx || !d_packed || !d_patch || !d_out || layer < 0 || layer > 5) return aff_fail(ctx, AFFNET_ERR_INVALID, "probe_hardnet_f24_layer: layer 0 .. 5");
+    return aff_hardnet_poly_patches(ctx, d_packed, d_patch, 1, d_out, nullptr, layer, (hipStream_t)stream, AFFNET_DESC_FORM_F24);
+}
+
+extern "C" int affnet_probe_hardnet_f24_forward(affnet_ctx* ctx, const float* d_packed, const float* d_patches, int n, float* d_out, float* d_scratch, void* stream) {
+    AFF_DEVICE(ctx);
+    if (!ctx || !d_packed || !d_patches || !d_out || !d_scratch || n < 1 || n > 65535) return aff_fail(ctx, AFFNET_ERR_INVALID, "probe_hardnet_f24_forward: bad argument");
+    return aff_hardnet_poly_patches(ctx, d_packed, d_patches, n, d_out, d_scratch, -1, (hipStream_t)stream, AFFNET_DESC_FORM_F24);
+}
+
+extern "C" int affnet_probe_hardnet_f24_u(affnet_ctx* ctx, const float* d_packed, int layer, float* d_out, void* stream) {
+    AFF_DEVICE(ctx);
+    if (!ctx || !d_packed || !d_out || layer != 1) return aff_fail(ctx, AFFNET_ERR_INVALID, "probe_hardnet_f24_u: layer 1");
+    return probe_derived_u(ctx, AFFNET_NET_HARDNET, TRUNK_WINO_F24, d_packed, F24::BASE + F24::offset(layer), F24::floats(layer), d_out, stream);
+}
diff --git a/affnet_amd/csrc/derive_u.hip b/affnet_amd/csrc/derive_u.hip
--- a/affnet_amd/csrc/derive_u.hip
+++ b/affnet_amd/csrc/derive_u.hip
@@ -11,7 +11,7 @@
 }
 
 static DerivedTable table_of(int kind, int form) {
-    if (kind == AFFNET_NET_HARDNET) return form == TRUNK_WINO ? derived_hardnet_poly() : (form == TRUNK_WINO_F43 ? derived_hardnet_form2() : DerivedTable{});
+    if (kind == AFFNET_NET_HARDNET) return form == TRUNK_WINO ? derived_hardnet_poly() : (form == TRUNK_WINO_F43 ? derived_hardnet_form2() : (form == TRUNK_WINO_F24 ? derived_hardnet_form3() : DerivedTable{}));
     const bool wino = kind == AFFNET_NET_ORINET ? form == TRUNK_EXACT : (form == TRUNK_WINO || form == TRUNK_WINO_POLY);
     return wino ? derived_trunk16() : DerivedTable{};
 }
diff --git a/affnet_amd/csrc/pack_check.cpp b/affnet_amd/csrc/pack_check.cpp
--- a/affnet_amd/csrc/pack_check.cpp
+++ b/affnet_amd/csrc/pack_check.cpp
@@ -92,6 +92,7 @@
 static_assert(Wino16::offset(1) == 0 && Wino16::offset(3) == 4096 && Wino16::offset(5) == 20480 && Wino16::offset(2) == 86016 && Wino16::offset(4) == 98816 && Wino16::FLOATS == 150016 && Wino16::PAIRS == 7936, "Wino16");
 static_assert(Poly32::offset(2) == 0 && Poly32::offset(4) == 51200 && Poly32::FLOATS == 256000 && Poly32::PAIRS == 10240, "Poly32");
 static_assert(F43::BASE == 256000 && F43::offset(1) == 0 && F43::offset(3) == 36864 && F43::FLOATS == 184320 && F43::PAIRS == 5120, "F43");
+static_assert(F24::BASE == 440320 && F24::offset(1) == 0 && F24::FLOATS == 24576 && F24::PAIRS == 1024, "F24");
 
 static int check_derived(const char* name, int kind, const DerivedTable& t, int want_sections, size_t want_floats) {
     const NetLayout L = net_layout(kind); const NetOffsets off = to_offsets(L);
@@ -103,14 +104,15 @@
     size_t pairs = 0, floats = 0;
     for (int i = 0; i < t.n; ++i) {
         const DerivedSection& s = t.s[i];
-        const int xi = s.family == DERIVED_WINO ? 16 : s.family == DERIVED_POLY ? 25 : 36;
-        CHECK(s.layer >= 1 && s.layer <= 5 && s.cin == L.cin[s.layer] && s.cout == L.cout[s.layer] && (size_t)s.pair0 == pairs && s.family >= 0 && s.family <= DERIVED_F43);
+        const int xi = s.family == DERIVED_WINO ? 16 : s.family == DERIVED_POLY ? 25 : s.family == DERIVED_F43 ? 36 : 24;
+        CHECK(s.layer >= 1 && s.layer <= 5 && s.cin == L.cin[s.layer] && s.cout == L.cout[s.layer] && (size_t)s.pair0 == pairs && s.family >= 0 && s.family <= DERIVED_F24);
         for (int c = 0; c < s.cin; ++c)
             for (int n = 0; n < s.cout; ++n, ++pairs) {
                 float g[9], u[36];
                 for (int tap = 0; tap < 9; ++tap) g[tap] = blob[L.w_off[s.layer] + w_tap_index(tap, c, n, s.cin, s.cout)];
                 if (s.family == DERIVED_WINO) wino_weight_transform(g, u);
                 else if (s.family == DERIVED_POLY) poly_weight_transform(g, u);
+                else if (s.family == DERIVED_F24) f24_weight_transform(g, u);
                 else f43_weight_transform(g, u);
                 const size_t e = s.pair0 + w_tap_index(0, c, n, s.cin, s.cout);
                 CHECK(e < (size_t)t.pairs);
@@ -129,10 +131,11 @@
 }
 
 static int check_regions() {
-    const size_t t16 = derived_trunk16().floats, poly = derived_hardnet_poly().floats, f43 = derived_hardnet_f43().floats;
-    CHECK(DerivedU::AFFNET == 0 && DerivedU::ORINET == t16 && DerivedU::HARDNET == 2 * t16 && DerivedU::HARDNET_F43 == 2 * t16 + poly && DerivedU::FLOATS == 2 * t16 + poly + f43);
+    const size_t t16 = derived_trunk16().floats, poly = derived_hardnet_poly().floats, f43 = derived_hardnet_f43().floats, f24 = derived_hardnet_f24().floats;
+    CHECK(DerivedU::AFFNET == 0 && DerivedU::ORINET == t16 && DerivedU::HARDNET == 2 * t16 && DerivedU::HARDNET_F43 == 2 * t16 + poly && DerivedU::HARDNET_F24 == 2 * t16 + poly + f43 &&
+          DerivedU::FLOATS == 2 * t16 + poly + f43 + f24);
     CHECK(DerivedU::region(AFFNET_NET_AFFNET) == DerivedU::AFFNET && DerivedU::region(AFFNET_NET_ORINET) == DerivedU::ORINET && DerivedU::region(AFFNET_NET_HARDNET) == DerivedU::HARDNET);
-    CHECK(derived_hardnet_form2().floats == poly + f43);
+    CHECK(derived_hardnet_form2().floats == poly + f43 && derived_hardnet_form3().floats == poly + f43 + f24);
     return 0;
 }
 
@@ -141,7 +144,9 @@
         if (check_kind(kind)) return 1;
     if (check_derived("AffNet", AFFNET_NET_AFFNET, derived_trunk16(), 5, 150016) || check_derived("OriNet", AFFNET_NET_ORINET, derived_trunk16(), 5, 150016) ||
         check_derived("HardNet polyphase", AFFNET_NET_HARDNET, derived_hardnet_poly(), 2, 256000) || check_derived("HardNet F(4x4, 3x3)", AFFNET_NET_HARDNET, derived_hardnet_f43(), 2, 184320) ||
-        check_derived("HardNet form 2", AFFNET_NET_HARDNET, derived_hardnet_form2(), 4, 256000 + 184320) || check_regions())
+        check_derived("HardNet form 2", AFFNET_NET_HARDNET, derived_hardnet_form2(), 4, 256000 + 184320) ||
+        check_derived("HardNet F(2x4, 3x3)", AFFNET_NET_HARDNET, derived_hardnet_f24(), 1, 24576) ||
+        check_derived("HardNet form 3", AFFNET_NET_HARDNET, derived_hardnet_form3(), 5, 256000 + 184320 + 24576) || check_regions())
         return 1;
     return 0;
 }
diff --git a/affnet_amd/csrc/weights_layout.h b/affnet_amd/csrc/weights_layout.h
--- a/affnet_amd/csrc/weights_layout.h
+++ b/affnet_amd/csrc/weights_layout.h
@@ -168,8 +168,17 @@
     for (int j = 0; j < 6; ++j) f43_g_axis(t[j], t[6 + j], t[12 + j], U + j, 6);
 }
 
-enum { DERIVED_WINO = 0, DERIVED_POLY = 1, DERIVED_F43 = 2 };
-constexpr int derived_xi(int family) { return family == DERIVED_WINO ? 16 : (family == DERIVED_POLY ? POLY_XI : F43_XI); }
+#define F24_XI 24
+AFF_HOST_DEVICE inline void f24_weight_transform(const float g[9], float U[F24_XI]) {
+    float t[18];
+#pragma unroll
+    for (int ky = 0; ky < 3; ++ky) f43_g_axis(g[3 * ky], g[3 * ky + 1], g[3 * ky + 2], t + 6 * ky, 1);
+#pragma unroll
+    for (int j = 0; j < 6; ++j) wino_g_axis(t[j], t[6 + j], t[12 + j], U + j, 6);
+}
+
+enum { DERIVED_WINO = 0, DERIVED_POLY = 1, DERIVED_F43 = 2, DERIVED_F24 = 3 };
+constexpr int derived_xi(int family) { return family == DERIVED_WINO ? 16 : (family == DERIVED_POLY ? POLY_XI : (family == DERIVED_F43 ? F43_XI : F24_XI)); }
 struct DerivedSection {
     int layer, cin, cout;
     int family;
@@ -193,6 +202,8 @@
 constexpr DerivedTable derived_hardnet_poly() { return derived_add(derived_add(DerivedTable{}, 32, 2, DERIVED_POLY), 32, 4, DERIVED_POLY); }
 constexpr DerivedTable derived_hardnet_f43() { return derived_add(derived_add(DerivedTable{}, 32, 1, DERIVED_F43), 32, 3, DERIVED_F43); }
 constexpr DerivedTable derived_hardnet_form2() { return derived_add(derived_add(derived_hardnet_poly(), 32, 1, DERIVED_F43), 32, 3, DERIVED_F43); }
+constexpr DerivedTable derived_hardnet_f24() { return derived_add(DerivedTable{}, 32, 1, DERIVED_F24); }
+constexpr DerivedTable derived_hardnet_form3() { return derived_add(derived_hardnet_form2(), 32, 1, DERIVED_F24); }
 constexpr DerivedSection derived_layer(const DerivedTable& t, int layer) {
     for (int i = 0; i < t.n; ++i)
         if (t.s[i].layer == layer) return t.s[i];
@@ -208,7 +219,7 @@
     return i == t.n || (t.s[i].pair0 % 256 == 0 && t.s[i].cin * t.s[i].cout % 256 == 0 && derived_by_workgroups(t, i + 1));
 }
 static_assert(derived_by_workgroups(derived_trunk16()) && derived_by_workgroups(derived_hardnet_poly()) && derived_by_workgroups(derived_hardnet_f43()) &&
-              derived_by_workgroups(derived_hardnet_form2()), "a 256-thread workgroup of derive_u_kernel stays within one section");
+              derived_by_workgroups(derived_hardnet_form2()) && derived_by_workgroups(derived_hardnet_f24()) && derived_by_workgroups(derived_hardnet_form3()), "a 256-thread workgroup of derive_u_kernel stays within one section");
 
 template <DerivedTable (*T)()>
 struct DerivedView {
@@ -221,18 +232,22 @@
 struct F43 : DerivedView<derived_hardnet_f43> { static constexpr int BASE = Poly32::FLOATS; };
 static_assert(derived_hardnet_form2().s[2].dst == F43::BASE + F43::offset(1) && derived_hardnet_form2().s[3].dst == F43::BASE + F43::offset(3) &&
               derived_hardnet_form2().floats == F43::BASE + F43::FLOATS, "form 2's table = Poly32 with F43 at F43::BASE");
+struct F24 : DerivedView<derived_hardnet_f24> { static constexpr int BASE = F43::BASE + F43::FLOATS; };
+static_assert(derived_hardnet_form3().n == 5 && derived_hardnet_form3().s[4].dst == F24::BASE + F24::offset(1) && derived_hardnet_form3().floats == F24::BASE + F24::FLOATS,
+              "form 3's table = form 2's with F24 at F24::BASE");
 
 struct DerivedU {
     static constexpr int AFFNET = 0, ORINET = AFFNET + Wino16::FLOATS;
     static constexpr int HARDNET = ORINET + Wino16::FLOATS;
     static constexpr int HARDNET_F43 = HARDNET + F43::BASE;
-    static constexpr int FLOATS = HARDNET_F43 + F43::FLOATS;
+    static constexpr int HARDNET_F24 = HARDNET + F24::BASE;
+    static constexpr int FLOATS = HARDNET_F24 + F24::FLOATS;
     static constexpr int region(int kind) { return kind == AFFNET_NET_AFFNET ? AFFNET : (kind == AFFNET_NET_ORINET ? ORINET : HARDNET); }
 };
 static_assert(DerivedU::AFFNET == 0 && DerivedU::ORINET - DerivedU::AFFNET == derived_trunk16().floats && DerivedU::HARDNET - DerivedU::ORINET == derived_trunk16().floats &&
-              DerivedU::FLOATS - DerivedU::HARDNET == derived_hardnet_form2().floats && DerivedU::FLOATS == 2 * Wino16::FLOATS + Poly32::FLOATS + F43::FLOATS,
+              DerivedU::FLOATS - DerivedU::HARDNET == derived_hardnet_form3().floats && DerivedU::FLOATS == 2 * Wino16::FLOATS + Poly32::FLOATS + F43::FLOATS + F24::FLOATS,
               "the regions are disjoint, in this order, and fill the buffer");
-static_assert(DerivedU::ORINET % 64 == 0 && DerivedU::HARDNET % 64 == 0 && DerivedU::HARDNET_F43 % 64 == 0, "every region starts on a 256-byte boundary, as an allocation of its own would");
+static_assert(DerivedU::ORINET % 64 == 0 && DerivedU::HARDNET % 64 == 0 && DerivedU::HARDNET_F43 % 64 == 0 && DerivedU::HARDNET_F24 % 64 == 0, "every region starts on a 256-byte boundary, as an allocation of its own would");
 static_assert(w_tap_index(7, 21, 13, 32, 64) == 7 * 32 * 64 + w_tap_index(0, 21, 13, 32, 64) && w_tap_index(35, 63, 63, 64, 64) == 35 * 64 * 64 + w_tap_index(0, 63, 63, 64, 64),
               "a position is a plane of cin * cout floats");
 AFF_HOST_DEVICE inline void derive_u_pair(const DerivedTable& t, int e, const float* packed, const int (&w_off)[6], float* U) {
@@ -247,6 +262,7 @@
     float u[F43_XI];
     if (s.family == DERIVED_WINO) wino_weight_transform(g, u);
     else if (s.family == DERIVED_POLY) poly_weight_transform(g, u);
+    else if (s.family == DERIVED_F24) f24_weight_transform(g, u);
     else f43_weight_transform(g, u);
 #pragma unroll
     for (int xi = 0; xi < F43_XI; ++xi)
diff --git a/affnet_amd/engine.py b/affnet_amd/engine.py
--- a/affnet_amd/engine.py
+++ b/affnet_amd/engine.py
@@ -44,7 +44,7 @@
                                          onepass=onepass, lazy_shape_rows=lazy_shape_rows, arith=arith)
         self.arith = _lib.arith_code(arith)
         self.shape_form = _lib.SHAPE_FORM_WINOGRAD
-        self.desc_form = _lib.DESC_FORM_F43
+        self.desc_form = _lib.DESC_FORM_F24
         self.device = device
         self.handle = C.c_void_p()
         idx = device.index if device.index is not None else torch.cuda.current_device()
diff --git a/include/affnet_hip.h b/include/affnet_hip.h
--- a/include/affnet_hip.h
+++ b/include/affnet_hip.h
@@ -77,6 +77,7 @@
 #define AFFNET_DESC_FORM_DIRECT 0
 #define AFFNET_DESC_FORM_POLYPHASE 1
 #define AFFNET_DESC_FORM_F43 2
+#define AFFNET_DESC_FORM_F24 3
 int affnet_set_desc_form(affnet_ctx* ctx, int form);
 int affnet_get_desc_form(const affnet_ctx* ctx);
 
diff --git a/include/affnet_hip_probes.h b/include/affnet_hip_probes.h
--- a/include/affnet_hip_probes.h
+++ b/include/affnet_hip_probes.h
@@ -32,6 +32,10 @@
 int affnet_probe_hardnet_f43_forward(affnet_ctx* ctx, const float* d_packed, const float* d_patches, int n, float* d_out, float* d_scratch, void* stream);
 int affnet_probe_hardnet_f43_u(affnet_ctx* ctx, const float* d_packed, int layer, float* d_out, void* stream);
 
+int affnet_probe_hardnet_f24_layer(affnet_ctx* ctx, const float* d_packed, const float* d_patch, int layer, float* d_out, void* stream);
+int affnet_probe_hardnet_f24_forward(affnet_ctx* ctx, const float* d_packed, const float* d_patches, int n, float* d_out, float* d_scratch, void* stream);
+int affnet_probe_hardnet_f24_u(affnet_ctx* ctx, const float* d_packed, int layer, float* d_out, void* stream);
+
 #ifdef __cplusplus
 }
 #endif
```

Result: no change. 1.694 million, median of 6 (+1.0%).
